# DerEchteKarsten/RayTracer3

Hardware: AMD Instinct MI355X
Metric: Mrays/s (higher is better)
Workload: dtype f32

## Files before the change

### include/rt3.h

```cpp
#ifndef RT3_H
#define RT3_H
#include <stddef.h>
#include <stdint.h>

#ifdef __cplusplus
extern "C" {
#endif

#define RT3_OK 0
#define RT3_E_INVALID (-1)
#define RT3_E_HIP (-2)
#define RT3_E_NO_DEVICE (-3)
#define RT3_E_STATE (-4)
#define RT3_E_UNSUPPORTED (-5)
#define RT3_E_DEPTH (-6)
#define RT3_E_COMM (-7)

#define RT3_INVALID_HANDLE 0xFFFFFFFFu
#define RT3_TAG_BUFFER 0u
#define RT3_TAG_IMAGE 1u
#define RT3_TAG_ACCEL 3u
#define RT3_MISS 0xFFFFFFFFu
#define RT3_BACKGROUND_DEPTH 100000.0f

#define RT3_FORMAT_R32_SFLOAT 100u
#define RT3_FORMAT_R32G32B32A32_SFLOAT 109u
#define RT3_FORMAT_R32G32B32A32_UINT 107u
#define RT3_FORMAT_R8G8B8A8_UNORM 37u
#define RT3_FORMAT_R16_UINT 74u

#define RT3_F_NEE_SKY 1u
#define RT3_F_BLUENOISE 2u
#define RT3_F_SPECULAR 4u
#define RT3_F_FACEFORWARD 8u
#define RT3_F_PROBE_RADIANCE 16u
#define RT3_F_NEE_EMISSIVE 32u

typedef struct rt3_gconst {
    float proj[16];
    float view[16];
    float proj_inverse[16];
    float view_inverse[16];
    float window_size[2];
    uint32_t frame;
    float blendfactor;
    uint32_t bounces;
    uint32_t samples;
    uint32_t proberng;
    float cell_size;
    uint32_t mouse[2];
    uint32_t pad[2];
} rt3_gconst;

typedef struct rt3_geometry_info {
    float base_color[4];
    int32_t base_color_texture_index;
    float metallic_factor;
    uint32_t index_offset;
    uint32_t vertex_offset;
    float emission[4];
    float roughness;
    uint32_t _pad[3];
} rt3_geometry_info;

typedef struct rt3_instance {
    uint32_t geometry_first, geometry_count;
    float transform[16];
} rt3_instance;

typedef struct rt3_stats {
    uint64_t extension_rays;
    uint64_t shadow_rays;
    uint64_t nodes_visited;
    uint64_t tris_tested;
    uint64_t shadow_nodes_visited;
    uint64_t shadow_tris_tested;
    uint64_t extend_launches;
    double extend_ms;
    uint64_t shadow_launches;
    double shadow_ms;
    double shade_ms;
    double other_ms;
    uint64_t trace_launches;
    double trace_ms;
    uint64_t trace_rays[2];
    uint64_t trace_nodes[2];
    uint64_t trace_tris[2];
    double gather_ms;
    uint64_t nodes_visited_lds;
    uint64_t shadow_nodes_visited_lds;
    double accel_build_ms;
    uint64_t accel_bulk_copies;
    uint64_t accel_arena_serial;
} rt3_stats;

typedef struct rt3_ctx rt3_ctx;

int rt3_create(int device, rt3_ctx **out);
void rt3_destroy(rt3_ctx *ctx);
const char *rt3_last_error(rt3_ctx *ctx);
int rt3_device_name(rt3_ctx *ctx, char *buf, size_t buf_size);

#define RT3_OPT_BATCH_SPP 1
#define RT3_OPT_PROFILE 2
#define RT3_OPT_COUNT_TRAVERSAL 3
#define RT3_OPT_EXTEND_VARIANT 4
#define RT3_OPT_LEAF_SIZE 5
#define RT3_OPT_NODE_WIDTH 6
#define RT3_OPT_NODE_QUANT 7
#define RT3_OPT_WIDE_COLLAPSE 8
#define RT3_OPT_POOL_CHUNK 9
#define RT3_OPT_SAH_TOP 11
#define RT3_OPT_TRACE_BLOCKS 12
#define RT3_OPT_INSTANCE_MODE 14
int rt3_set_option(rt3_ctx *ctx, int option, int64_t value);

int rt3_scene_set_vertices(rt3_ctx *ctx, const float *interleaved_p_n_t, uint32_t n_vertices);
int rt3_scene_set_indices(rt3_ctx *ctx, const uint32_t *indices, uint32_t n_indices);
int rt3_scene_set_geometry(rt3_ctx *ctx, const rt3_geometry_info *infos, const uint32_t *prim_counts, uint32_t n);
int rt3_scene_set_sky(rt3_ctx *ctx, const float *rgb, uint32_t width, uint32_t height);
int rt3_scene_set_bluenoise(rt3_ctx *ctx, const uint8_t *rgba, uint32_t width, uint32_t height);
int rt3_scene_set_texture(rt3_ctx *ctx, uint32_t index, const uint8_t *rgba_srgb, uint32_t width, uint32_t height);
int rt3_scene_set_alpha_cutoffs(rt3_ctx *ctx, const float *cutoffs, uint32_t n);
typedef struct rt3_material_textures {
    int32_t metallic_roughness_texture;
    int32_t normal_texture;
    int32_t emissive_texture;
    float   normal_scale;
} rt3_material_textures;
int rt3_scene_set_material_textures(rt3_ctx *ctx, const rt3_material_textures *m, uint32_t n);

int rt3_scene_set_instances(rt3_ctx *ctx, const rt3_instance *instances, uint32_t n);
int rt3_scene_set_prev_transforms(rt3_ctx *ctx, const float *transforms , uint32_t n);
int rt3_scene_snapshot_vertices(rt3_ctx *ctx);
int rt3_scene_forget_prev_vertices(rt3_ctx *ctx);
int rt3_scene_deformed_geometries(rt3_ctx *ctx, uint8_t *flags, uint32_t n);

int rt3_accel_build(rt3_ctx *ctx, uint32_t *out_handle);
int rt3_accel_info(rt3_ctx *ctx, uint32_t *n_nodes, uint32_t *n_tris, uint32_t *max_depth, uint32_t *node_bytes);
int rt3_accel_download(rt3_ctx *ctx, void *nodes, size_t nodes_bytes, void *tris, size_t tris_bytes);
int rt3_accel_levels(rt3_ctx *ctx, uint32_t *n_meshes, uint32_t *n_meshes_built, uint32_t *n_top_nodes, uint64_t *accel_bytes);
int rt3_accel_import(rt3_ctx *ctx, const void *nodes, size_t nodes_bytes, const void *tris, size_t tris_bytes);
int rt3_scene_update_vertices(rt3_ctx *ctx, const float *interleaved_p_n_t, uint32_t first, uint32_t n);
int rt3_accel_refit(rt3_ctx *ctx, uint32_t *out_handle);
int rt3_light_info(rt3_ctx *ctx, uint32_t *n_emitters, uint64_t *cdf_total);
int rt3_light_download(rt3_ctx *ctx, uint32_t *prim, float *area, uint32_t *mass );
int rt3_sky_download(rt3_ctx *ctx, uint32_t *alias, uint32_t *texels_rgb9e5, float *cdf_marg, float *pdf_uv);

int rt3_buffer_create(rt3_ctx *ctx, size_t bytes, uint32_t *out_handle);
int rt3_image_create(rt3_ctx *ctx, uint32_t width, uint32_t height, uint32_t format, uint32_t *out_handle);
int rt3_image_import(rt3_ctx *ctx, void *device_ptr, uint32_t width, uint32_t height, uint32_t format, uint32_t *out_handle);
int rt3_resource_upload(rt3_ctx *ctx, uint32_t handle, const void *src, size_t bytes);
int rt3_resource_download(rt3_ctx *ctx, uint32_t handle, void *dst, size_t bytes);
int rt3_resource_device_ptr(rt3_ctx *ctx, uint32_t handle, void **out_ptr, size_t *out_bytes);

int rt3_set_tile_partition(rt3_ctx *ctx, uint32_t width, uint32_t height, uint32_t rank, uint32_t n_ranks);
int rt3_tile_pixel_count(rt3_ctx *ctx, uint32_t rank, uint32_t n_ranks, uint32_t *out_count);
int rt3_image_pack_tiles(rt3_ctx *ctx, uint32_t image, uint32_t rank, uint32_t n_ranks, void *dst_device);
int rt3_image_unpack_tiles(rt3_ctx *ctx, uint32_t image, uint32_t rank, uint32_t n_ranks, const void *src_device);

#define RT3_COMM_ID_BYTES 128
int rt3_comm_version(int *out);
int rt3_comm_unique_id(void *id_out );
int rt3_comm_init(rt3_ctx *ctx, const void *id , uint32_t rank, uint32_t n_ranks);
int rt3_comm_destroy(rt3_ctx *ctx);
int rt3_gather_tiles(rt3_ctx *ctx, uint32_t image, uint32_t root);
int rt3_gather_layout(rt3_ctx *ctx, uint32_t image, uint32_t root, uint32_t n_ranks, uint64_t *offsets );
int rt3_gather_unpack(rt3_ctx *ctx, uint32_t image, uint32_t root, uint32_t n_ranks, const void *recv_device);

int rt3_pass_launch(rt3_ctx *ctx, const char *pass_name, const char *entry, uint32_t x, uint32_t y, uint32_t z,
                    const void *constants, size_t constants_size, const uint32_t *bindings, uint32_t n_bindings);
#define RT3_DENOISE_NO_DEMODULATION 1u
typedef struct rt3_denoise_params {
    uint32_t iterations;
    uint32_t normal_squarings;
    float sigma_z;
    float sigma_l;
    uint32_t flags;
} rt3_denoise_params;
int rt3_denoise_set_params(rt3_ctx *ctx, const rt3_denoise_params *params);
int rt3_denoise_set_variance_input(rt3_ctx *ctx, uint32_t moments_image);

#define RT3_TEMPORAL_NO_DEMODULATION 1u
typedef struct rt3_temporal_params {
    float alpha;
    float alpha_moments;
    uint32_t max_history;
    float normal_cos;
    float plane_tolerance;
    uint32_t flags;
} rt3_temporal_params;
int rt3_temporal_set_prev_view(rt3_ctx *ctx, const void *prev_gconst, size_t size);
int rt3_temporal_set_params(rt3_ctx *ctx, const rt3_temporal_params *params);
int rt3_temporal_set_motion_input(rt3_ctx *ctx, uint32_t motion_image);

int rt3_frame_wait(rt3_ctx *ctx);

int rt3_trace_rays(rt3_ctx *ctx, const float *rays, uint32_t n, int any_hit, float *t, float *u, float *v, uint32_t *prim,
                   uint32_t *n_nodes, uint32_t *n_tris, int repeat, double *kernel_ms);

int rt3_selftest_eval(rt3_ctx *ctx, int op, const void *in, uint32_t n, void *out);

int rt3_stats_reset(rt3_ctx *ctx);
int rt3_stats_get(rt3_ctx *ctx, rt3_stats *out);

void rt3_camera_gconst(const float position[3], const float direction[3], float fov_y_radians, float aspect,
                       float z_near, float z_far, float width, float height, rt3_gconst *out);

#ifdef __cplusplus
}
#endif
#endif
```

### raytracer3_amd/_lib.py

```python
from __future__ import annotations

import ctypes as C
import os
from pathlib import Path

PKG = Path(__file__).resolve().parent
LIB_PATH = Path(os.environ.get("RT3_LIBRARY", PKG / "librt3.so"))

RT3_OK = 0
E_INVALID, E_HIP, E_NO_DEVICE, E_STATE, E_UNSUPPORTED, E_DEPTH, E_COMM = -1, -2, -3, -4, -5, -6, -7
COMM_ID_BYTES = 128
TAG_BUFFER, TAG_IMAGE, TAG_ACCEL = 0, 1, 3
MISS = 0xFFFFFFFF
BACKGROUND_DEPTH = 100000.0
FORMAT_R32_SFLOAT, FORMAT_R32G32B32A32_SFLOAT, FORMAT_R32G32B32A32_UINT, FORMAT_R8G8B8A8_UNORM, FORMAT_R16_UINT = 100, 109, 107, 37, 74
F_NEE_SKY, F_BLUENOISE, F_SPECULAR, F_FACEFORWARD, F_PROBE_RADIANCE = 1, 2, 4, 8, 16
F_NEE_EMISSIVE = 32
OPT_BATCH_SPP, OPT_PROFILE, OPT_COUNT_TRAVERSAL, OPT_EXTEND_VARIANT, OPT_LEAF_SIZE, OPT_NODE_WIDTH, OPT_NODE_QUANT = 1, 2, 3, 4, 5, 6, 7
OPT_WIDE_COLLAPSE, OPT_POOL_CHUNK, OPT_SAH_TOP, OPT_TRACE_BLOCKS = 8, 9, 11, 12
OPT_FUSED_TRACE = 10
OPT_INSTANCE_MODE = 14
DENOISE_NO_DEMODULATION = 1
TEMPORAL_NO_DEMODULATION = 1
SELFTEST_EXPN = 28
SELFTEST_HIT_INFO = 29

EXPORTS = [
    "rt3_create", "rt3_destroy", "rt3_last_error", "rt3_device_name", "rt3_set_option",
    "rt3_scene_set_vertices", "rt3_scene_set_indices", "rt3_scene_set_geometry", "rt3_scene_set_sky", "rt3_scene_set_bluenoise", "rt3_scene_set_texture",
    "rt3_scene_set_alpha_cutoffs",
    "rt3_scene_set_material_textures",
    "rt3_scene_set_instances",
    "rt3_accel_build", "rt3_accel_info", "rt3_accel_levels", "rt3_accel_download", "rt3_accel_import", "rt3_sky_download",
    "rt3_scene_update_vertices", "rt3_accel_refit", "rt3_light_info", "rt3_light_download",
    "rt3_buffer_create", "rt3_image_create", "rt3_image_import", "rt3_resource_upload", "rt3_resource_download", "rt3_resource_device_ptr",
    "rt3_set_tile_partition", "rt3_tile_pixel_count", "rt3_image_pack_tiles", "rt3_image_unpack_tiles",
    "rt3_comm_version", "rt3_comm_unique_id", "rt3_comm_init", "rt3_comm_destroy", "rt3_gather_tiles", "rt3_gather_layout", "rt3_gather_unpack",
    "rt3_pass_launch", "rt3_denoise_set_params", "rt3_denoise_set_variance_input", "rt3_temporal_set_prev_view", "rt3_temporal_set_params",
    "rt3_scene_set_prev_transforms", "rt3_temporal_set_motion_input",
    "rt3_scene_snapshot_vertices", "rt3_scene_forget_prev_vertices", "rt3_scene_deformed_geometries",
    "rt3_frame_wait", "rt3_trace_rays", "rt3_selftest_eval", "rt3_stats_reset", "rt3_stats_get", "rt3_camera_gconst",
]


class GConst(C.Structure):

    _fields_ = [("proj", C.c_float * 16), ("view", C.c_float * 16), ("proj_inverse", C.c_float * 16), ("view_inverse", C.c_float * 16),
                ("window_size", C.c_float * 2), ("frame", C.c_uint32), ("blendfactor", C.c_float), ("bounces", C.c_uint32),
                ("samples", C.c_uint32), ("proberng", C.c_uint32), ("cell_size", C.c_float), ("mouse", C.c_uint32 * 2), ("pad", C.c_uint32 * 2)]


class Stats(C.Structure):
    _fields_ = [("extension_rays", C.c_uint64), ("shadow_rays", C.c_uint64), ("nodes_visited", C.c_uint64), ("tris_tested", C.c_uint64),
                ("shadow_nodes_visited", C.c_uint64), ("shadow_tris_tested", C.c_uint64),
                ("extend_launches", C.c_uint64), ("extend_ms", C.c_double), ("shadow_launches", C.c_uint64), ("shadow_ms", C.c_double),
                ("shade_ms", C.c_double), ("other_ms", C.c_double),
                ("trace_launches", C.c_uint64), ("trace_ms", C.c_double), ("trace_rays", C.c_uint64 * 2), ("trace_nodes", C.c_uint64 * 2),
                ("trace_tris", C.c_uint64 * 2), ("gather_ms", C.c_double), ("nodes_visited_lds", C.c_uint64), ("shadow_nodes_visited_lds", C.c_uint64), ("accel_build_ms", C.c_double), ("accel_bulk_copies", C.c_uint64),
                ("accel_arena_serial", C.c_uint64)]


class Instance(C.Structure):

    _fields_ = [("geometry_first", C.c_uint32), ("geometry_count", C.c_uint32), ("transform", C.c_float * 16)]


class DenoiseParams(C.Structure):

    _fields_ = [("iterations", C.c_uint32), ("normal_squarings", C.c_uint32), ("sigma_z", C.c_float), ("sigma_l", C.c_float), ("flags", C.c_uint32)]

    def __init__(self, iterations=5, normal_squarings=7, sigma_z=0.05, sigma_l=4.0, flags=0):
        super().__init__(iterations, normal_squarings, sigma_z, sigma_l, flags)


class TemporalParams(C.Structure):

    _fields_ = [("alpha", C.c_float), ("alpha_moments", C.c_float), ("max_history", C.c_uint32), ("normal_cos", C.c_float),
                ("plane_tolerance", C.c_float), ("flags", C.c_uint32)]

    def __init__(self, alpha=0.2, alpha_moments=0.2, max_history=32, normal_cos=0.9, plane_tolerance=0.01, flags=0):
        super().__init__(alpha, alpha_moments, max_history, normal_cos, plane_tolerance, flags)


assert C.sizeof(GConst) == 304


def kernel_source_hash() -> str:
    import hashlib

    h = hashlib.sha256()
    files = sorted((PKG / "csrc").glob("*.hip")) + sorted((PKG / "csrc").glob("*.hpp")) + [PKG / "csrc" / "Makefile", PKG.parent / "include" / "rt3.h"]
    for f in files:
        h.update(f.name.encode())
        h.update(f.read_bytes())
    return h.hexdigest()[:16]


class Rt3Error(RuntimeError):
    def __init__(self, code, msg):
        super().__init__(f"rt3 error {code}: {msg}")
        self.code = code


_lib = None


def load():
    global _lib
    if _lib is not None:
        return _lib
    try:
        import torch
    except ImportError:
        pass
    if not LIB_PATH.exists():
        raise ImportError(f"{LIB_PATH} is missing: build it with `make -C {PKG / 'csrc'}` (hipcc, gfx950). There is no CPU fallback.")
    L = C.CDLL(str(LIB_PATH))
    vp, u32, i32, f32, sz = C.c_void_p, C.c_uint32, C.c_int, C.c_float, C.c_size_t
    pu32 = C.POINTER(C.c_uint32)
    sig = {
        "rt3_create": (i32, [i32, C.POINTER(vp)]),
        "rt3_destroy": (None, [vp]),
        "rt3_last_error": (C.c_char_p, [vp]),
        "rt3_device_name": (i32, [vp, C.c_char_p, sz]),
        "rt3_set_option": (i32, [vp, i32, C.c_int64]),
        "rt3_scene_set_vertices": (i32, [vp, vp, u32]),
        "rt3_scene_set_indices": (i32, [vp, vp, u32]),
        "rt3_scene_set_geometry": (i32, [vp, vp, vp, u32]),
        "rt3_scene_set_sky": (i32, [vp, vp, u32, u32]),
        "rt3_scene_set_bluenoise": (i32, [vp, vp, u32, u32]),
        "rt3_scene_set_texture": (i32, [vp, u32, vp, u32, u32]),
        "rt3_scene_set_alpha_cutoffs": (i32, [vp, vp, u32]),
        "rt3_scene_set_material_textures": (i32, [vp, vp, u32]),
        "rt3_scene_set_instances": (i32, [vp, vp, u32]),
        "rt3_accel_build": (i32, [vp, pu32]),
        "rt3_accel_info": (i32, [vp, pu32, pu32, pu32, pu32]),
        "rt3_accel_levels": (i32, [vp, pu32, pu32, pu32, C.POINTER(C.c_uint64)]),
        "rt3_accel_download": (i32, [vp, vp, sz, vp, sz]),
        "rt3_accel_import": (i32, [vp, vp, sz, vp, sz]),
        "rt3_sky_download": (i32, [vp, vp, vp, vp, vp]),
        "rt3_scene_update_vertices": (i32, [vp, vp, u32, u32]),
        "rt3_accel_refit": (i32, [vp, pu32]),
        "rt3_light_info": (i32, [vp, pu32, C.POINTER(C.c_uint64)]),
        "rt3_light_download": (i32, [vp, vp, vp, vp]),
        "rt3_buffer_create": (i32, [vp, sz, pu32]),
        "rt3_image_create": (i32, [vp, u32, u32, u32, pu32]),
        "rt3_image_import": (i32, [vp, vp, u32, u32, u32, pu32]),
        "rt3_resource_upload": (i32, [vp, u32, vp, sz]),
        "rt3_resource_download": (i32, [vp, u32, vp, sz]),
        "rt3_resource_device_ptr": (i32, [vp, u32, C.POINTER(vp), C.POINTER(sz)]),
        "rt3_set_tile_partition": (i32, [vp, u32, u32, u32, u32]),
        "rt3_tile_pixel_count": (i32, [vp, u32, u32, pu32]),
        "rt3_image_pack_tiles": (i32, [vp, u32, u32, u32, vp]),
        "rt3_image_unpack_tiles": (i32, [vp, u32, u32, u32, vp]),
        "rt3_comm_version": (i32, [C.POINTER(i32)]),
        "rt3_comm_unique_id": (i32, [vp]),
        "rt3_comm_init": (i32, [vp, vp, u32, u32]),
        "rt3_comm_destroy": (i32, [vp]),
        "rt3_gather_tiles": (i32, [vp, u32, u32]),
        "rt3_gather_layout": (i32, [vp, u32, u32, u32, C.POINTER(C.c_uint64)]),
        "rt3_gather_unpack": (i32, [vp, u32, u32, u32, vp]),
        "rt3_pass_launch": (i32, [vp, C.c_char_p, C.c_char_p, u32, u32, u32, vp, sz, pu32, u32]),
        "rt3_denoise_set_params": (i32, [vp, C.POINTER(DenoiseParams)]),
        "rt3_denoise_set_variance_input": (i32, [vp, u32]),
        "rt3_temporal_set_prev_view": (i32, [vp, vp, sz]),
        "rt3_temporal_set_params": (i32, [vp, C.POINTER(TemporalParams)]),
        "rt3_scene_set_prev_transforms": (i32, [vp, vp, u32]),
        "rt3_temporal_set_motion_input": (i32, [vp, u32]),
        "rt3_scene_snapshot_vertices": (i32, [vp]),
        "rt3_scene_forget_prev_vertices": (i32, [vp]),
        "rt3_scene_deformed_geometries": (i32, [vp, vp, u32]),
        "rt3_frame_wait": (i32, [vp]),
        "rt3_trace_rays": (i32, [vp, vp, u32, i32, vp, vp, vp, vp, vp, vp, i32, C.POINTER(C.c_double)]),
        "rt3_selftest_eval": (i32, [vp, i32, vp, u32, vp]),
        "rt3_stats_reset": (i32, [vp]),
        "rt3_stats_get": (i32, [vp, C.POINTER(Stats)]),
        "rt3_camera_gconst": (None, [C.POINTER(f32), C.POINTER(f32), f32, f32, f32, f32, f32, f32, C.POINTER(GConst)]),
    }
    for name, (res, args) in sig.items():
        fn = getattr(L, name)
        fn.restype = res
        fn.argtypes = args
    _lib = L
    return L
```

### raytracer3_amd/csrc/rt3_accel.hip

```cpp
#include <hip/hip_runtime.h>

#include <cmath>
#include <cstring>
#include <algorithm>
#include <chrono>
#include <string>
#include <vector>

#include "rt3_ctx.hpp"

using namespace rt3;

namespace rt3 {

void invalidate_accel(rt3_ctx* c) { c->accel.built = false; }
void mark_accel_stale(rt3_ctx* c) {
    if (c->accel.built) c->accel.stale = true;
}
int check_accel_current(rt3_ctx* c, const char* unbuilt) {
    if (!c || !c->accel.built) return fail(c, RT3_E_STATE, unbuilt);
    if (c->accel.stale) return fail(c, RT3_E_STATE, "vertices were updated since the acceleration structure was built: rt3_accel_refit or rt3_accel_build first");
    return RT3_OK;
}
std::pair<const rt3_instance*, size_t> placements(const rt3_ctx* c, rt3_instance& whole) {
// ... 392 lines not shown
    uint32_t total = 0;
    for (size_t i = 0; i < n_inst; i++) {
        const float* m = inst[i].transform;
        double M[3][3];
        for (int r = 0; r < 3; r++)
            for (int k = 0; k < 3; k++) M[r][k] = m[4 * k + r];
        const double det = M[0][0] * (M[1][1] * M[2][2] - M[1][2] * M[2][1]) - M[0][1] * (M[1][0] * M[2][2] - M[1][2] * M[2][0]) +
                           M[0][2] * (M[1][0] * M[2][1] - M[1][1] * M[2][0]);
        TlInstance& in = ii[i];
        memcpy(in.m, m, sizeof(in.m));
        in.identity = memcmp(m, kIdentity, sizeof(kIdentity)) == 0;
        if (!(std::fabs(det) > 0.0) || !std::isfinite(1.0 / det))
            return fail(c, RT3_E_UNSUPPORTED, "instance " + std::to_string(i) + ": the upper 3 x 3 of the transform is singular (instance mode 1 needs its inverse)");
        const double id = 1.0 / det;
        in.A[0][0] = (M[1][1] * M[2][2] - M[1][2] * M[2][1]) * id;
        in.A[0][1] = (M[0][2] * M[2][1] - M[0][1] * M[2][2]) * id;
        in.A[0][2] = (M[0][1] * M[1][2] - M[0][2] * M[1][1]) * id;
        in.A[1][0] = (M[1][2] * M[2][0] - M[1][0] * M[2][2]) * id;
        in.A[1][1] = (M[0][0] * M[2][2] - M[0][2] * M[2][0]) * id;
        in.A[1][2] = (M[0][2] * M[1][0] - M[0][0] * M[1][2]) * id;
        in.A[2][0] = (M[1][0] * M[2][1] - M[1][1] * M[2][0]) * id;
        in.A[2][1] = (M[0][1] * M[2][0] - M[0][0] * M[2][1]) * id;
        in.A[2][2] = (M[0][0] * M[1][1] - M[0][1] * M[1][0]) * id;
        for (int r = 0; r < 3; r++) {
            for (int k = 0; k < 3; k++) in.A[r][k] = (double)(float)in.A[r][k];
            in.b[r] = (double)(float)-(in.A[r][0] * m[12] + in.A[r][1] * m[13] + in.A[r][2] * m[14]);
        }
        in.nA = in.nM = 0.0;
        for (int r = 0; r < 3; r++) {
            in.nA = std::fmax(in.nA, std::fabs(in.A[r][0]) + std::fabs(in.A[r][1]) + std::fabs(in.A[r][2]));
            in.nM = std::fmax(in.nM, std::fabs(M[r][0]) + std::fabs(M[r][1]) + std::fabs(M[r][2]));
        }
        if (!std::isfinite(in.nA) || in.nA * in.nM > kTlMaxCondition)
            return fail(c, RT3_E_UNSUPPORTED, "instance " + std::to_string(i) + ": the transform is too badly conditioned for instance mode 1 (||M|| ||M^-1|| > 2^20)");
        in.prim_base = total;
        uint32_t cnt = 0;
        for (; at < placed.size() && placed[at].instance == i; at++) cnt += placed[at].n_prims;
        total += cnt;
        in.mesh = ~0u;
        if (cnt == 0) continue;
        for (size_t q = 0; q < meshes.size(); q++)
            if (meshes[q].first == inst[i].geometry_first && meshes[q].count == inst[i].geometry_count) in.mesh = (uint32_t)q;
        if (in.mesh == ~0u) {
            TlMesh nm;
            memset(&nm, 0, sizeof(nm));
            nm.first = inst[i].geometry_first;
            nm.count = inst[i].geometry_count;
            nm.n_tris = cnt;
            in.mesh = (uint32_t)meshes.size();
            meshes.push_back(nm);
        }
    }
    uint32_t n_ne = 0;
    for (auto& in : ii) n_ne += in.mesh != ~0u ? 1u : 0u;
    if (n_ne >= (1u << 26)) return fail(c, RT3_E_UNSUPPORTED, "instance mode 1: too many instances");
    const uint32_t top_cap = n_ne ? n_ne : 1u;
    const uint32_t head = top_cap + 2u * n_ne;

    bool same = tl.valid && tl.gen == c->scene.content_gen && tl.head == head && tl.meshes.size() == meshes.size();
    for (size_t q = 0; same && q < meshes.size(); q++) same = tl.meshes[q].first == meshes[q].first && tl.meshes[q].count == meshes[q].count;
    tl.n_built = 0;
    if (same) {
        meshes = tl.meshes;
    } else {
        const bool reuse = tl.valid && tl.gen == c->scene.content_gen;
        std::vector<LbvhResult> built(meshes.size());
        std::vector<int> from(meshes.size(), -1);
        int rc = RT3_OK;
        for (size_t q = 0; q < meshes.size() && rc == RT3_OK; q++) {
            for (size_t o = 0; reuse && o < tl.meshes.size(); o++)
                if (tl.meshes[o].first == meshes[q].first && tl.meshes[o].count == meshes[q].count) from[q] = (int)o;
            if (from[q] >= 0) {
                const TlMesh& om = tl.meshes[from[q]];
                meshes[q].n_nodes = om.n_nodes;
                meshes[q].depth = om.depth;
                memcpy(meshes[q].box, om.box, sizeof(om.box));
            } else {
                rc = tl_build_mesh(c, meshes[q], &built[q]);
                tl.n_built++;
            }
        }
        uint64_t nodes_total = head, tris_total = 0;
        for (auto& m : meshes) {
            m.node_off = (uint32_t)nodes_total;
            m.tri_off = (uint32_t)tris_total;
            nodes_total += m.n_nodes;
            tris_total += m.n_tris;
        }
        if (rc == RT3_OK && (nodes_total >= (1ull << 29) || tris_total > (1ull << 28)))
            rc = fail(c, RT3_E_UNSUPPORTED, "instance mode 1: the bottom trees exceed the 28-bit references");
        LbvhResult fresh;
        hipError_t e = hipSuccess;
        if (rc == RT3_OK) {
            e = fresh.alloc_arena((size_t)nodes_total * 64, (size_t)tris_total, c->stream);
            if (fresh.arena_need > kArenaMaxBytes) rc = fail_arena(c, "two-level: bottom trees", fresh.arena_need);
        }
        if (rc == RT3_OK) {
            for (size_t q = 0; e == hipSuccess && q < meshes.size(); q++) {
                const TlMesh& m = meshes[q];
                if (from[q] >= 0) {
                    const TlMesh& om = tl.meshes[from[q]];
                    tlas_rebase_nodes(c->stream, c->accel.bvh.nodes.get() + 4 * (size_t)om.node_off, fresh.nodes.get() + 4 * (size_t)m.node_off, m.n_nodes, om.node_off,
                                      m.node_off, om.tri_off, m.tri_off);
                    e = hipMemcpyAsync(fresh.tris.get() + 3 * (size_t)m.tri_off, c->accel.bvh.tris.get() + 3 * (size_t)om.tri_off, (size_t)m.n_tris * 48, hipMemcpyDeviceToDevice,
                                       c->stream);
                } else {
                    tlas_rebase_nodes(c->stream, built[q].nodes.get(), fresh.nodes.get() + 4 * (size_t)m.node_off, m.n_nodes, 0u, m.node_off, 0u, m.tri_off);
                    e = hipMemcpyAsync(fresh.tris.get() + 3 * (size_t)m.tri_off, built[q].tris.get(), (size_t)m.n_tris * 48, hipMemcpyDeviceToDevice, c->stream);
                }
            }
            if (e == hipSuccess) e = hipGetLastError();
            if (e == hipSuccess) e = hipStreamSynchronize(c->stream);
            if (e != hipSuccess) rc = fail(c, RT3_E_HIP, std::string("two-level: bottom trees: ") + hipGetErrorString(e));
        }
        if (rc != RT3_OK) {
            free_accel(c);
            return rc;
        }
        c->accel.bvh.take_arena(fresh);
        tl.meshes = meshes;
        tl.head = head;
        tl.gen = c->scene.content_gen;
        tl.n_alloc_nodes = (uint32_t)nodes_total;
        tl.valid = true;
    }
    tl.inst = std::move(ii);
    tl.n_placed = n_ne;
    tl.top_cap = top_cap;
    return tl_records_and_top(c);
}

static int make_alpha_tables(rt3_ctx* c) {
    c->accel.masked = false;
    if (!any_cutoff(c)) return RT3_OK;
    if (c->opt.node_width != 4 || c->opt.node_quant != 1)
        return fail(c, RT3_E_UNSUPPORTED, "alpha-masked geometry needs the default node layout (RT3_OPT_NODE_WIDTH 4, RT3_OPT_NODE_QUANT 1)");
    std::vector<uint2> mask(c->scene.n_geoms, make_uint2(0u, 0u)), table;
    for (uint32_t g = 0; g < c->scene.n_geoms; g++) {
        if (!(c->scene.h_cutoffs[g] > 0.0f)) continue;
        uint32_t cb, ab;
        memcpy(&cb, &c->scene.h_cutoffs[g], 4);
        memcpy(&ab, &c->scene.h_geoms[g].base_color[3], 4);
        mask[g] = make_uint2(cb, (uint32_t)table.size());
        table.push_back(make_uint2((uint32_t)c->scene.h_geoms[g].base_color_texture_index, ab));
    }
    for (const Placed& p : c->accel.placed)
        if (mask[p.geom].x != 0u && p.n_prims > 0) c->accel.masked = true;
    if (int r = dev_alloc(c, c->accel.d_geom_mask, mask.size())) return r;
    if (int r = dev_alloc(c, c->accel.d_alpha, table.size())) return r;
    HIPC(c, hipMemcpy(c->accel.d_geom_mask.get(), mask.data(), mask.size() * sizeof(uint2), hipMemcpyHostToDevice));
    HIPC(c, hipMemcpy(c->accel.d_alpha.get(), table.data(), table.size() * sizeof(uint2), hipMemcpyHostToDevice));
    return RT3_OK;
}
static void bump_stamp(rt3_ctx* c) { c->accel.stamp++; }
static int accel_finish(rt3_ctx* c, uint32_t* out_handle) {
    if (int r = make_shade_records(c)) return r;
    HIPC(c, hipStreamSynchronize(c->stream));
    c->prof.stats.accel_bulk_copies += c->accel.bulk_copies;
    c->accel.bulk_copies = 0;
    c->accel.built = true;
    c->accel.stale = false;
    bump_stamp(c);
    c->accel.topo_gen = c->scene.topo_gen;
    if (out_handle) *out_handle = (RT3_TAG_ACCEL << 30) | 0u;
    return RT3_OK;
}
int rt3_accel_build(rt3_ctx* c, uint32_t* out_handle) {
    if (!c) return RT3_E_INVALID;
    HIPC(c, hipSetDevice(c->device));
    if (c->scene.n_prims && (!c->scene.d_verts || !c->scene.d_indices)) return fail(c, RT3_E_STATE, "set vertices, indices and geometry before rt3_accel_build");
    if (int r = revalidate_geometry(c)) return r;
    HIPC(c, hipStreamSynchronize(c->stream));
    const auto t_build0 = std::chrono::steady_clock::now();
    invalidate_accel(c);
    c->accel.refit_planned = false;
    if (int r = flatten_world(c)) return r;
    if (int r = make_alpha_tables(c)) return r;
    if (c->opt.instance_mode == 1) {
        if (int r = build_two_level(c)) return r;
    } else {
        free_accel(c);
        hipError_t e = lbvh_build(c->stream, world_tables(c), c->accel.n_flat_prims, c->opt.leaf_size, c->opt.node_width, c->opt.node_quant, c->opt.collapse,
                                  c->opt.sah_top, c->accel.build_scratch, &c->accel.bvh, c->accel.masked ? c->accel.d_geom_mask.get() : nullptr);
        if (c->accel.build_scratch.capacity_bytes() > ((size_t)1 << 30)) c->accel.build_scratch.reset();
        if (e != hipSuccess) {
            const uint64_t need = c->accel.bvh.arena_need;
            free_accel(c);
            if (need > kArenaMaxBytes) return fail_arena(c, "lbvh_build", need);
            return fail(c, RT3_E_HIP, std::string("lbvh_build: ") + hipGetErrorString(e));
        }
        const uint32_t stack_need = stack_entries(c->opt.node_width, c->accel.bvh.max_depth);
        if (stack_need > kMaxStack) {
            const int rc = fail(c, RT3_E_DEPTH, "LBVH with " + std::to_string(c->accel.bvh.max_depth) + " levels needs " + std::to_string(stack_need) +
                                                    " stack entries, the traversal kernels hold " + std::to_string(kMaxStack));
            free_accel(c);
            return rc;
        }
    }
    if (int r = accel_finish(c, out_handle)) return r;
    c->prof.stats.accel_build_ms = std::chrono::duration<double, std::milli>(std::chrono::steady_clock::now() - t_build0).count();
    return RT3_OK;
}
int rt3_accel_info(rt3_ctx* c, uint32_t* n_nodes, uint32_t* n_tris, uint32_t* max_depth, uint32_t* node_bytes) {
    if (!c || !c->accel.built) return fail(c, RT3_E_STATE, "no acceleration structure built");
    if (n_nodes) *n_nodes = c->accel.bvh.n_nodes;
    if (n_tris) *n_tris = c->accel.bvh.n_tris;
    if (max_depth) *max_depth = c->accel.bvh.max_depth;
    if (node_bytes) *node_bytes = c->accel.bvh.node_bytes;
    return RT3_OK;
}
int rt3_accel_levels(rt3_ctx* c, uint32_t* n_meshes, uint32_t* n_meshes_built, uint32_t* n_top_nodes, uint64_t* accel_bytes) {
    if (!c || !c->accel.built) return fail(c, RT3_E_STATE, "no acceleration structure built");
    const bool two = c->accel.bvh.layout == kLayoutTwoLevel;
    if (n_meshes) *n_meshes = two ? c->accel.tl.n_meshes : 0u;
    if (n_meshes_built) *n_meshes_built = two ? c->accel.tl.n_built : 0u;
    if (n_top_nodes) *n_top_nodes = two ? c->accel.tl.n_top : 0u;
    if (accel_bytes) {
        const uint64_t nodes = !c->accel.bvh.nodes ? 0u : (two ? (uint64_t)c->accel.tl.n_alloc_nodes * 64u : (uint64_t)c->accel.bvh.n_nodes * c->accel.bvh.node_bytes);
        *accel_bytes = nodes + (!c->accel.bvh.tris ? 0u : (uint64_t)c->accel.bvh.n_tris * 48u) + (uint64_t)c->accel.bvh.n_top * 64u;
    }
    return RT3_OK;
}
int rt3_accel_download(rt3_ctx* c, void* nodes, size_t nodes_bytes, void* tris, size_t tris_bytes) {
    if (int r = check_accel_current(c, "no acceleration structure built")) return r;
    if (c->accel.bvh.layout == kLayoutTwoLevel) return fail(c, RT3_E_UNSUPPORTED, "accel_download: not for the two-level structure (RT3_OPT_INSTANCE_MODE 1)");
    if (nodes) {
        if (nodes_bytes != (size_t)c->accel.bvh.n_nodes * c->accel.bvh.node_bytes) return fail(c, RT3_E_INVALID, "nodes_bytes mismatch");
        if (nodes_bytes) HIPC(c, hipMemcpy(nodes, c->accel.bvh.nodes.get(), nodes_bytes, hipMemcpyDeviceToHost));
    }
    if (tris) {
        if (tris_bytes != (size_t)c->accel.bvh.n_tris * 48) return fail(c, RT3_E_INVALID, "tris_bytes mismatch");
        if (tris_bytes) HIPC(c, hipMemcpy(tris, c->accel.bvh.tris.get(), tris_bytes, hipMemcpyDeviceToHost));
    }
    return RT3_OK;
}
int rt3_accel_import(rt3_ctx* c, const void* nodes, size_t nodes_bytes, const void* tris, size_t tris_bytes) {
    if (!c || !nodes || !tris) return fail(c, RT3_E_INVALID, "accel_import: NULL argument");
    if (!c->accel.built) return fail(c, RT3_E_STATE, "accel_import: build the scene's own structure first (rt3_accel_build makes the shading records)");
    if (c->accel.bvh.layout == kLayoutTwoLevel) return fail(c, RT3_E_UNSUPPORTED, "accel_import: not for the two-level structure (RT3_OPT_INSTANCE_MODE 1)");
    if (c->accel.bvh.layout != kLayoutWide64Q) return fail(c, RT3_E_UNSUPPORTED, "accel_import: default node layout only");
    if (any_cutoff(c)) return fail(c, RT3_E_UNSUPPORTED, "accel_import: not for a scene with alpha-masked geometry (rt3_scene_set_alpha_cutoffs)");
    if (nodes_bytes == 0 || nodes_bytes % 64 || tris_bytes % 48 || nodes_bytes / 64 > 0x3FFFFFFFull) return fail(c, RT3_E_INVALID, "accel_import: sizes must be multiples of 64 / 48 bytes");
    const uint32_t nn = (uint32_t)(nodes_bytes / 64), nt = (uint32_t)(tris_bytes / 48);
    const uint32_t* w = static_cast<const uint32_t*>(nodes);
    const uint32_t* tw = static_cast<const uint32_t*>(tris);
    for (uint32_t k = 0; k < nt; k++)
        if (tw[12 * (size_t)k + 9] >= c->accel.n_flat_prims) return fail(c, RT3_E_INVALID, "accel_import: triangle record " + std::to_string(k) + " names a primitive the scene does not have");
    std::vector<uint8_t> seen(nn, 0);
    std::vector<std::pair<uint32_t, uint32_t>> st;
    st.emplace_back(0u, 1u);
    seen[0] = 1;
    uint32_t max_level = 1;
    while (!st.empty()) {
        const auto [node, level] = st.back();
        st.pop_back();
        max_level = level > max_level ? level : max_level;
        for (int k = 0; k < 4; k++) {
            const uint32_t ref = w[16 * (size_t)node + 10 + k];
            if (ref == 0xFFFFFFFFu) continue;
            if (ref & 0x80000000u) {
                const uint64_t first = ref & 0x0FFFFFFFu, cnt = ((ref >> 28) & 7u) + 1u;
                if (first + cnt > nt) return fail(c, RT3_E_INVALID, "accel_import: node " + std::to_string(node) + " references triangles beyond the array");
            } else {
                if (ref >= nn || seen[ref]) return fail(c, RT3_E_INVALID, "accel_import: node " + std::to_string(node) + " references a node out of range or reachable twice");
                seen[ref] = 1;
                st.emplace_back(ref, level + 1);
            }
        }
    }
    const uint32_t depth = max_level + 1;
    if (stack_entries(4, depth) > kMaxStack) return fail(c, RT3_E_DEPTH, "accel_import: the tree is deeper than the traversal stack supports");
    HIPC(c, hipSetDevice(c->device));
    HIPC(c, hipStreamSynchronize(c->stream));
    LbvhResult fresh;
    hipError_t e = fresh.alloc_arena(nodes_bytes, nt, c->stream);
    if (fresh.arena_need > kArenaMaxBytes) return fail_arena(c, "accel_import", fresh.arena_need);
    if (e == hipSuccess) e = hipStreamSynchronize(c->stream);
    if (e == hipSuccess) e = hipMemcpy(fresh.nodes.get(), nodes, nodes_bytes, hipMemcpyHostToDevice);
    if (e == hipSuccess && tris_bytes) e = hipMemcpy(fresh.tris.get(), tris, tris_bytes, hipMemcpyHostToDevice);
    if (e != hipSuccess) return fail(c, RT3_E_HIP, std::string("accel_import: ") + hipGetErrorString(e));
    c->accel.bvh.take_arena(fresh);
    c->accel.bvh.n_nodes = nn;
    c->accel.bvh.n_tris = nt;
    c->accel.bvh.max_depth = depth;
    c->accel.refit_planned = false;
    bump_stamp(c);
    e = lbvh_make_top(c->stream, c->accel.bvh.nodes.get(), nn, c->accel.bvh.top, &c->accel.bvh.n_top);
    if (e != hipSuccess) {
        invalidate_accel(c);
        return fail(c, RT3_E_HIP, std::string("accel_import: top-of-tree copy: ") + hipGetErrorString(e));
    }
    return RT3_OK;
}

struct RefitScratch {
    uint32_t* bounds;
    float *nbox, *tbox;
};
static int refit_scratch(rt3_ctx* c, size_t n_nodes, size_t n_tris, RefitScratch* s) {
    BufLayout plan;
    plan.add(&s->bounds, 6).add(&s->nbox, 6 * n_nodes).add(&s->tbox, 6 * n_tris);
    HIPC(c, c->accel.refit_scratch.grow_bytes(plan.bytes()));
    HIPC(c, plan.carve(c->accel.refit_scratch));
    return RT3_OK;
}
static int refit_flat(rt3_ctx* c) {
    LbvhResult& b = c->accel.bvh;
    if (!b.n_nodes) return RT3_OK;
    if (!c->accel.refit_planned) {
        c->accel.refit_trees.clear();
        c->accel.refit_trees.resize(1);
        const hipError_t e = refit_plan(c->stream, b.nodes.get(), 0u, b.n_nodes, b.max_depth, &c->accel.refit_trees[0]);
        if (e != hipSuccess) return fail(c, RT3_E_HIP, std::string("accel_refit: plan: ") + hipGetErrorString(e));
        c->accel.refit_planned = true;
    }
    RefitScratch s;
    if (int r = refit_scratch(c, b.n_nodes, b.n_tris, &s)) return r;
    hipError_t e = refit_tree(c->stream, c->accel.refit_trees[0], world_tables(c), c->accel.n_flat_prims, 0u, b.n_tris, b.nodes.get(), b.tris.get(), s.bounds, s.nbox,
                              s.tbox);
    if (e == hipSuccess) e = lbvh_make_top(c->stream, b.nodes.get(), b.n_nodes, b.top, &b.n_top);
    if (e != hipSuccess) return fail(c, RT3_E_HIP, std::string("accel_refit: ") + hipGetErrorString(e));
    return RT3_OK;
}
static int refit_two_level(rt3_ctx* c) {
    TwoLevelState& tl = c->accel.tl;
    tl.n_built = 0;
    if (!tl.valid) return RT3_OK;
    const std::vector<TlMesh>& meshes = tl.meshes;
    const size_t nm = meshes.size();
    if (!c->accel.refit_planned) {
        c->accel.refit_trees.clear();
        c->accel.refit_trees.resize(nm);
        c->accel.refit_tables.clear();
        c->accel.refit_tables.resize(nm);
        for (size_t q = 0; q < nm; q++) {
            const TlMesh& m = meshes[q];
            hipError_t e = make_mesh_tables(c, m, &c->accel.refit_tables[q]);
            if (e == hipSuccess && m.count * sizeof(FlatGeomDev) > (64u << 10)) c->accel.bulk_copies += 1;
            if (e == hipSuccess) e = refit_plan(c->stream, c->accel.bvh.nodes.get(), m.node_off, m.n_nodes, m.depth, &c->accel.refit_trees[q]);
            if (e != hipSuccess) return fail(c, RT3_E_HIP, std::string("accel_refit: plan: ") + hipGetErrorString(e));
        }
        c->accel.refit_planned = true;
    }
    RefitScratch s;
    if (int r = refit_scratch(c, tl.n_alloc_nodes, c->accel.bvh.n_tris, &s)) return r;
    std::vector<uint32_t> roots(16 * nm);
    hipError_t e = hipSuccess;
    for (size_t q = 0; e == hipSuccess && q < nm; q++) {
        const TlMesh& m = meshes[q];
        e = refit_tree(c->stream, c->accel.refit_trees[q], mesh_tables(c, c->accel.refit_tables[q]), m.n_tris, m.tri_off, m.n_tris, c->accel.bvh.nodes.get(), c->accel.bvh.tris.get(),
                       s.bounds, s.nbox, s.tbox);
        if (e == hipSuccess) e = hipMemcpyAsync(&roots[16 * q], c->accel.bvh.nodes.get() + 4 * (size_t)m.node_off, 64, hipMemcpyDeviceToHost, c->stream);
    }
    if (e == hipSuccess) e = hipStreamSynchronize(c->stream);
    if (e != hipSuccess) return fail(c, RT3_E_HIP, std::string("accel_refit: bottom trees: ") + hipGetErrorString(e));
    for (size_t q = 0; q < nm; q++) quantised_node_box(&roots[16 * q], tl.meshes[q].box);
    tl.gen = c->scene.content_gen;
    return tl_records_and_top(c);
}
int rt3_accel_refit(rt3_ctx* c, uint32_t* out_handle) {
    if (!c) return RT3_E_INVALID;
    if (c->opt.node_width != 4 || c->opt.node_quant != 1)
        return fail(c, RT3_E_UNSUPPORTED, "accel_refit: default node layout only (RT3_OPT_NODE_WIDTH 4, RT3_OPT_NODE_QUANT 1)");
    if (!c->accel.built || c->accel.topo_gen != c->scene.topo_gen)
        return fail(c, RT3_E_STATE, "accel_refit: no acceleration structure for the current scene (only rt3_scene_update_vertices may come between rt3_accel_build and a refit)");
    const bool two = c->accel.bvh.layout == kLayoutTwoLevel;
    if (!two && c->accel.bvh.layout != kLayoutWide64Q) return fail(c, RT3_E_UNSUPPORTED, "accel_refit: default node layout only");
    HIPC(c, hipSetDevice(c->device));
    HIPC(c, hipStreamSynchronize(c->stream));
    invalidate_accel(c);
    if (int r = two ? refit_two_level(c) : refit_flat(c)) return r;
    return accel_finish(c, out_handle);
}

int rt3_light_info(rt3_ctx* c, uint32_t* n_emitters, uint64_t* cdf_total) {
    if (!c) return RT3_E_INVALID;
    if (int r = ensure_lights(c)) return r;
    if (n_emitters) *n_emitters = c->accel.lights.n;
    if (cdf_total) *cdf_total = c->accel.lights.total;
    return RT3_OK;
}
int rt3_light_download(rt3_ctx* c, uint32_t* prim, float* area, uint32_t* mass) {
    if (!c) return RT3_E_INVALID;
    if (int r = ensure_lights(c)) return r;
    const LightTable& t = c->accel.lights;
    if (!t.n) return RT3_OK;
    if (prim) HIPC(c, hipMemcpy(prim, t.prim.get(), (size_t)t.n * 4, hipMemcpyDeviceToHost));
    if (area) HIPC(c, hipMemcpy(area, t.area.get(), (size_t)t.n * 4, hipMemcpyDeviceToHost));
    if (mass) {
        HIPC(c, hipMemcpy(mass, t.cdf.get(), (size_t)t.n * 4, hipMemcpyDeviceToHost));
        for (uint32_t k = t.n - 1; k > 0; k--) mass[k] -= mass[k - 1];
    }
    return RT3_OK;
}

}
```

### raytracer3_amd/csrc/rt3_api.hip

```cpp
#include <hip/hip_runtime.h>

#include <cmath>
#include <cstdio>
#include <cstring>
#include <string>
#include <vector>

#include "rt3_ctx.hpp"

using namespace rt3;

static_assert(sizeof(rt3_gconst) == 304 && sizeof(GConstDev) == 304, "GConst is 304 bytes (renderer/mod.rs:47-63)");
static_assert(sizeof(rt3_geometry_info) == 64, "geometry info is 64 bytes");
static_assert(RT3_F_NEE_SKY == RT3_FLAG_NEE_SKY && RT3_F_BLUENOISE == RT3_FLAG_BLUENOISE && RT3_F_FACEFORWARD == RT3_FLAG_FACEFORWARD && RT3_F_SPECULAR == RT3_FLAG_SPECULAR && RT3_F_PROBE_RADIANCE == RT3_FLAG_PROBE_RADIANCE && RT3_F_NEE_EMISSIVE == RT3_FLAG_NEE_EMISSIVE, "flags");

static thread_local std::string g_create_error;

namespace rt3 {

int fail(rt3_ctx* c, int code, const std::string& msg) {
    if (c) c->err = msg;
    else g_create_error = msg;
    return code;
}
// ... 5 lines not shown
    return r->tag == want_tag && r->ptr ? r : nullptr;
}
size_t format_bytes(uint32_t f) {
    switch (f) {
        case RT3_FORMAT_R32_SFLOAT: return 4;
        case RT3_FORMAT_R32G32B32A32_SFLOAT: return 16;
        case RT3_FORMAT_R32G32B32A32_UINT: return 16;
        case RT3_FORMAT_R8G8B8A8_UNORM: return 4;
        case RT3_FORMAT_R16_UINT: return 2;
        default: return 0;
    }
}

int harvest(rt3_ctx* c) {
    if (!c->work.pending_counters.empty()) {
        std::vector<uint32_t> h(c->work.counters_next);
        HIPC(c, hipMemcpy(h.data(), c->work.d_counters.get(), (size_t)c->work.counters_next * 4, hipMemcpyDeviceToHost));
        for (auto& b : c->work.pending_counters) {
            for (uint32_t k = 0; k < b.n_pairs; k++) {
                c->prof.stats.extension_rays += h[b.first + 2 * k];
                c->prof.stats.shadow_rays += h[b.first + 2 * k + 1];
            }
            for (uint32_t k = 0; k < b.n_emit; k++) c->prof.stats.shadow_rays += h[b.emit_first + k];
        }
        c->work.pending_counters.clear();
    }
    c->work.counters_next = 0;
    c->prof.stats.extension_rays += c->work.primary_rays_pending;
    c->work.primary_rays_pending = 0;
    if (c->opt.count) {
        unsigned long long t[kTotWords] = {};
        HIPC(c, hipMemcpy(t, c->work.d_totals.get(), sizeof(t), hipMemcpyDeviceToHost));
        c->prof.stats.nodes_visited += t[kTotExtendNodes];
        c->prof.stats.tris_tested += t[kTotExtendTris];
        c->prof.stats.shadow_nodes_visited += t[kTotShadowNodes];
        c->prof.stats.shadow_tris_tested += t[kTotShadowTris];
        c->prof.stats.nodes_visited_lds += t[kTotExtendLds];
        c->prof.stats.shadow_nodes_visited_lds += t[kTotShadowLds];
        HIPC(c, hipMemset(c->work.d_totals.get(), 0, sizeof(t)));
    }
    for (auto& t : c->prof.pending_events) {
        float ms = 0.0f;
        HIPC(c, hipEventElapsedTime(&ms, t.a, t.b));
        switch (t.cat) {
            case CAT_EXTEND: c->prof.stats.extend_ms += ms; c->prof.stats.extend_launches++; break;
            case CAT_SHADOW: c->prof.stats.shadow_ms += ms; c->prof.stats.shadow_launches++; break;
            case CAT_SHADE: c->prof.stats.shade_ms += ms; break;
            case CAT_GATHER: c->prof.stats.gather_ms += ms; break;
            default: c->prof.stats.other_ms += ms; break;
        }
        c->prof.free_events.push_back(t);
    }
    c->prof.pending_events.clear();
    return RT3_OK;
}

}

extern "C" {

int rt3_create(int device, rt3_ctx** out) {
    if (!out) return fail(nullptr, RT3_E_INVALID, "out is NULL");
    *out = nullptr;
    int n = 0;
    if (hipGetDeviceCount(&n) != hipSuccess || n <= 0) return fail(nullptr, RT3_E_NO_DEVICE, "no HIP device visible (librt3 has no CPU fallback)");
    if (device < 0 || device >= n) return fail(nullptr, RT3_E_INVALID, "device index out of range");
    hipDeviceProp_t prop;
    if (hipSetDevice(device) != hipSuccess || hipGetDeviceProperties(&prop, device) != hipSuccess) return fail(nullptr, RT3_E_HIP, "hipSetDevice failed");
    if (std::string(prop.gcnArchName).rfind("gfx950", 0) != 0)
        return fail(nullptr, RT3_E_NO_DEVICE, std::string("device is ") + prop.gcnArchName + ", librt3 is built for gfx950 only");
    rt3_ctx* c = new rt3_ctx();
    c->device = device;
    snprintf(c->name, sizeof(c->name), "%s (%s)", prop.name, prop.gcnArchName);
    memset(&c->prof.stats, 0, sizeof(c->prof.stats));
    if (hipStreamCreateWithFlags(&c->stream, hipStreamNonBlocking) != hipSuccess || c->work.d_counters.alloc_bytes((size_t)c->work.counters_cap * 4) != hipSuccess ||
        c->work.d_totals.alloc_bytes(kTotWords * 8) != hipSuccess || hipMemset(c->work.d_totals.get(), 0, kTotWords * 8) != hipSuccess) {
        rt3_destroy(c);
        return fail(nullptr, RT3_E_HIP, "stream / counter allocation failed");
    }
    *out = c;
    return RT3_OK;
}

void rt3_destroy(rt3_ctx* c) {
    if (!c) return;
    (void)hipSetDevice(c->device);
    if (c->stream) (void)hipStreamSynchronize(c->stream);
    comm_release(c);
    for (auto& t : c->prof.pending_events) { (void)hipEventDestroy(t.a); (void)hipEventDestroy(t.b); }
    for (auto& t : c->prof.free_events) { (void)hipEventDestroy(t.a); (void)hipEventDestroy(t.b); }
    hipStream_t stream = c->stream;
    delete c;
    if (stream) (void)hipStreamDestroy(stream);
}

const char* rt3_last_error(rt3_ctx* c) { return c ? c->err.c_str() : g_create_error.c_str(); }

int rt3_device_name(rt3_ctx* c, char* buf, size_t n) {
    if (!c || !buf || !n) return RT3_E_INVALID;
    snprintf(buf, n, "%s", c->name);
    return RT3_OK;
}

int rt3_set_option(rt3_ctx* c, int option, int64_t value) {
    if (!c) return RT3_E_INVALID;
    switch (option) {
        case RT3_OPT_BATCH_SPP: c->opt.batch_spp = value; return RT3_OK;
        case RT3_OPT_PROFILE: c->opt.profile = value != 0; return RT3_OK;
        case RT3_OPT_COUNT_TRAVERSAL: c->opt.count = value != 0; return RT3_OK;
        case RT3_OPT_EXTEND_VARIANT:
            c->opt.variant = (int)value;
            HIPC(c, hipSetDevice(c->device));
            set_refill_lanes((uint32_t)value);
            return RT3_OK;
        case RT3_OPT_LEAF_SIZE:
            if (value < 1 || value > 8) return fail(c, RT3_E_INVALID, "leaf size must be 1..8");
            c->opt.leaf_size = (uint32_t)value;
            invalidate_topology(c);
            return RT3_OK;
        case RT3_OPT_NODE_QUANT:
            if (value < 0 || value > 2) return fail(c, RT3_E_INVALID, "node quantisation must be 0 (fp32), 1 (64 B) or 2 (compact 48 B)");
            c->opt.node_quant = (uint32_t)value;
            invalidate_topology(c);
            return RT3_OK;
        case RT3_OPT_SAH_TOP:
            if (value < 0 || value > 65536) return fail(c, RT3_E_INVALID, "SAH-top cluster size must be 0 (off) .. 65536");
            c->opt.sah_top = (uint32_t)value;
            invalidate_topology(c);
            return RT3_OK;
        case RT3_OPT_POOL_CHUNK:
            if (value < 64 || value > 65536 || (value & 63)) return fail(c, RT3_E_INVALID, "pool chunk must be a multiple of 64 in [64, 65536]");
            HIPC(c, hipSetDevice(c->device));
            set_pool_chunk((uint32_t)value);
            return RT3_OK;
        case RT3_OPT_TRACE_BLOCKS:
            if (value < 1 || value > 65535) return fail(c, RT3_E_INVALID, "trace blocks must be in [1, 65535]");
            set_trace_blocks((uint32_t)value);
            return RT3_OK;
        case RT3_OPT_WIDE_COLLAPSE:
            if (value < 0 || value > 2) return fail(c, RT3_E_INVALID, "wide collapse must be 0 (even depth), 1 (surface area) or 2 (cost-driven)");
            c->opt.collapse = (uint32_t)value;
            invalidate_topology(c);
            return RT3_OK;
        case RT3_OPT_NODE_WIDTH:
            if (value != 2 && value != 4) return fail(c, RT3_E_INVALID, "node width must be 2 or 4");
            c->opt.node_width = (uint32_t)value;
            invalidate_topology(c);
            return RT3_OK;
        case RT3_OPT_INSTANCE_MODE:
            if (value != 0 && value != 1) return fail(c, RT3_E_INVALID, "instance mode must be 0 (flatten) or 1 (two-level)");
            c->opt.instance_mode = (int)value;
            invalidate_accel(c);
            return RT3_OK;
        default: return fail(c, RT3_E_INVALID, "unknown option");
    }
}

int rt3_buffer_create(rt3_ctx* c, size_t bytes, uint32_t* out) {
    if (!c || !out || !bytes) return fail(c, RT3_E_INVALID, "bad buffer size");
    HIPC(c, hipSetDevice(c->device));
    Resource r;
    r.tag = RT3_TAG_BUFFER;
    r.bytes = bytes;
    HIPC(c, r.mem.alloc_bytes(bytes));
    r.ptr = r.mem.get();
    HIPC(c, hipMemset(r.ptr, 0, bytes));
    c->resources.push_back(std::move(r));
    *out = (RT3_TAG_BUFFER << 30) | (uint32_t)(c->resources.size() - 1);
    return RT3_OK;
}
int rt3_image_create(rt3_ctx* c, uint32_t w, uint32_t h, uint32_t format, uint32_t* out) {
    size_t px = format_bytes(format);
    if (!c || !out || !w || !h || !px) return fail(c, RT3_E_INVALID, "bad image size / format");
    HIPC(c, hipSetDevice(c->device));
    Resource r;
    r.tag = RT3_TAG_IMAGE;
    r.w = w; r.h = h; r.format = format;
    r.bytes = (size_t)w * h * px;
    HIPC(c, r.mem.alloc_bytes(r.bytes));
    r.ptr = r.mem.get();
    HIPC(c, hipMemset(r.ptr, 0, r.bytes));
    c->resources.push_back(std::move(r));
    *out = (RT3_TAG_IMAGE << 30) | (uint32_t)(c->resources.size() - 1);
    return RT3_OK;
}
int rt3_image_import(rt3_ctx* c, void* device_ptr, uint32_t w, uint32_t h, uint32_t format, uint32_t* out) {
    size_t px = format_bytes(format);
    if (!c || !out || !device_ptr || !w || !h || !px) return fail(c, RT3_E_INVALID, "bad import");
    Resource r;
    r.tag = RT3_TAG_IMAGE;
    r.w = w; r.h = h; r.format = format;
    r.bytes = (size_t)w * h * px;
    r.ptr = device_ptr;
    c->resources.push_back(std::move(r));
    *out = (RT3_TAG_IMAGE << 30) | (uint32_t)(c->resources.size() - 1);
    return RT3_OK;
}
static Resource* any_res(rt3_ctx* c, uint32_t handle) {
    Resource* r = get_res(c, handle, RT3_TAG_IMAGE);
    return r ? r : get_res(c, handle, RT3_TAG_BUFFER);
}
int rt3_resource_upload(rt3_ctx* c, uint32_t handle, const void* src, size_t bytes) {
    if (!c || !src) return RT3_E_INVALID;
    Resource* r = any_res(c, handle);
    if (!r || bytes != r->bytes) return fail(c, RT3_E_INVALID, "upload: bad handle or size");
    HIPC(c, hipSetDevice(c->device));
    HIPC(c, hipStreamSynchronize(c->stream));
    HIPC(c, hipMemcpy(r->ptr, src, bytes, hipMemcpyHostToDevice));
    return RT3_OK;
}
int rt3_resource_download(rt3_ctx* c, uint32_t handle, void* dst, size_t bytes) {
    if (!c || !dst) return RT3_E_INVALID;
    Resource* r = any_res(c, handle);
    if (!r || bytes != r->bytes) return fail(c, RT3_E_INVALID, "download: bad handle or size");
    HIPC(c, hipSetDevice(c->device));
    HIPC(c, hipStreamSynchronize(c->stream));
    HIPC(c, hipMemcpy(dst, r->ptr, bytes, hipMemcpyDeviceToHost));
    return RT3_OK;
}
int rt3_resource_device_ptr(rt3_ctx* c, uint32_t handle, void** out_ptr, size_t* out_bytes) {
    if (!c || !out_ptr) return RT3_E_INVALID;
    Resource* r = any_res(c, handle);
    if (!r) return fail(c, RT3_E_INVALID, "bad handle");
    *out_ptr = r->ptr;
    if (out_bytes) *out_bytes = r->bytes;
    return RT3_OK;
}

int rt3_frame_wait(rt3_ctx* c) {
    if (!c) return RT3_E_INVALID;
    HIPC(c, hipSetDevice(c->device));
    HIPC(c, hipStreamSynchronize(c->stream));
    return RT3_OK;
}

int rt3_trace_rays(rt3_ctx* c, const float* rays, uint32_t n, int any_hit, float* t, float* u, float* v, uint32_t* prim, uint32_t* n_nodes,
                   uint32_t* n_tris, int repeat, double* kernel_ms) {
    if (!c || !rays || !prim || (!any_hit && (!t || !u || !v))) return fail(c, RT3_E_INVALID, "trace_rays: NULL argument");
    if (int r = check_accel_current(c)) return r;
    if (n == 0) return RT3_OK;
    HIPC(c, hipSetDevice(c->device));
    DevBuf<float> d_rays, d_hits;
    DevBuf<uint32_t> d_cn, d_ct, d_occ, d_cur;
    const bool count = n_nodes || n_tris;
    struct Events {
        hipEvent_t e0 = nullptr, e1 = nullptr;
        ~Events() {
            if (e0) (void)hipEventDestroy(e0);
            if (e1) (void)hipEventDestroy(e1);
        }
    } ev;
    HIPC(c, d_rays.alloc_bytes((size_t)n * 32));
    HIPC(c, d_hits.alloc_bytes((size_t)n * 16));
    HIPC(c, d_occ.alloc_bytes((size_t)n * 4));
    HIPC(c, d_cur.alloc_bytes(4));
    if (count) {
        HIPC(c, d_cn.alloc_bytes((size_t)n * 4));
        HIPC(c, d_ct.alloc_bytes((size_t)n * 4));
    }
    {
        std::vector<float> rec((size_t)n * 8);
        for (uint32_t i = 0; i < n; i++) {
            float* a = &rec[4 * (size_t)i];
            float* b = &rec[4 * ((size_t)n + i)];
            a[0] = rays[i]; a[1] = rays[(size_t)n + i]; a[2] = rays[2 * (size_t)n + i]; a[3] = rays[6 * (size_t)n + i];
            b[0] = rays[3 * (size_t)n + i]; b[1] = rays[4 * (size_t)n + i]; b[2] = rays[5 * (size_t)n + i]; b[3] = rays[7 * (size_t)n + i];
        }
        HIPC(c, hipMemcpy(d_rays.get(), rec.data(), (size_t)n * 32, hipMemcpyHostToDevice));
    }
    HIPC(c, hipEventCreate(&ev.e0));
    HIPC(c, hipEventCreate(&ev.e1));
    if (repeat < 1) repeat = 1;
    TraceLaunch L;
    L.rays = d_rays.get(); L.stride = n; L.n = n; L.work_counter = d_cur.get();
    L.hits = d_hits.get(); L.occluded = d_occ.get();
    L.count = count; L.cnt_nodes = d_cn.get(); L.cnt_tris = d_ct.get();
    if (c->accel.masked) {
        if (int r = sync_textures(c)) return r;
        L.alpha = alpha_dev(c);
    }
    auto launch = [&]() {
        (void)hipMemsetAsync(d_cur.get(), 0, 4, c->stream);
        if (any_hit) launch_shadow(c->stream, c->accel.bvh, L);
        else launch_extend(c->stream, c->accel.bvh, L);
    };
    launch();
    HIPC(c, hipEventRecord(ev.e0, c->stream));
    for (int k = 0; k < repeat; k++) launch();
    HIPC(c, hipEventRecord(ev.e1, c->stream));
    HIPC(c, hipGetLastError());
    HIPC(c, hipStreamSynchronize(c->stream));
    float ms = 0.0f;
    HIPC(c, hipEventElapsedTime(&ms, ev.e0, ev.e1));
    if (kernel_ms) *kernel_ms = (double)ms / repeat;
    if (any_hit) {
        HIPC(c, hipMemcpy(prim, d_occ.get(), (size_t)n * 4, hipMemcpyDeviceToHost));
    } else {
        std::vector<float> rec((size_t)n * 4);
        HIPC(c, hipMemcpy(rec.data(), d_hits.get(), (size_t)n * 16, hipMemcpyDeviceToHost));
        for (uint32_t i = 0; i < n; i++) {
            t[i] = rec[4 * (size_t)i];
            u[i] = rec[4 * (size_t)i + 1];
            v[i] = rec[4 * (size_t)i + 2];
            memcpy(&prim[i], &rec[4 * (size_t)i + 3], 4);
        }
    }
// ... 110 lines not shown
```

### raytracer3_amd/csrc/rt3_ctx.hpp

```cpp
#pragma once
#include <hip/hip_runtime.h>

#include <cstring>
#include <string>
#include <utility>
#include <vector>

#include "../../include/rt3.h"
#include "rt3_internal.hpp"

struct ncclComm;

namespace rt3 {

inline const rt3_denoise_params kDenoiseDefaults = {5u, 7u, 0.05f, 4.0f, 0u};
inline const rt3_temporal_params kTemporalDefaults = {0.2f, 0.2f, 32u, 0.9f, 0.01f, 0u};
inline constexpr float kIdentity[16] = {1, 0, 0, 0, 0, 1, 0, 0, 0, 0, 1, 0, 0, 0, 0, 1};
inline void pack3x4(const float* m16, float* m12) {
    for (int col = 0; col < 4; col++)
        for (int row = 0; row < 3; row++) m12[3 * col + row] = m16[4 * col + row];
}

struct Resource {
    uint32_t tag = 0;
    void* ptr = nullptr;
    DevBuf<char> mem;
    size_t bytes = 0;
    uint32_t w = 0, h = 0, format = 0;
};
struct PixelList {
    uint32_t w, h, rank, n_ranks, count;
    DevBuf<uint32_t> dev;
    DevBuf<uint2> dev_bn;
    uint64_t bn_stamp = ~0ull;
};
struct GatherLayout {
    uint32_t w, h, root, n_ranks;
    std::vector<uint64_t> off;
    DevBuf<uint32_t> dev;
};
enum Cat { CAT_EXTEND = 0, CAT_SHADOW = 1, CAT_SHADE = 2, CAT_OTHER = 3, CAT_GATHER = 4 };
struct Timed {
    hipEvent_t a, b;
    int cat;
};
struct CounterBlock {
    uint32_t first, n_pairs;
    uint32_t emit_first = 0, n_emit = 0;
};

struct TlMesh {
    uint32_t first, count;
    uint32_t node_off, tri_off;
    uint32_t n_nodes, n_tris, depth;
    double box[6];
};
struct TlInstance {
    double A[3][3], b[3];
    double nA, nM;
    float m[16];
    uint32_t mesh, prim_base;
    bool identity;
};
struct TwoLevelState {
    bool valid = false;
    uint64_t gen = 0;
    uint32_t head = 0;
    uint32_t n_alloc_nodes = 0;
    std::vector<TlMesh> meshes;
    std::vector<TlInstance> inst;
    uint32_t n_placed = 0, top_cap = 0;
    uint32_t n_meshes = 0, n_built = 0, n_top = 0;
    DevBuf<char> scratch;
};
struct MeshTables {
    DevBuf<char> mem;
    FlatGeomDev* geoms = nullptr;
    uint32_t *first_prim = nullptr, *prim_geom = nullptr;
};
struct ShadeRecords {
    DevBuf<uint4> rec;
    DevBuf<float2> uv;
    DevBuf<uint32_t> tan;
    bool has_tan = false;
    uint32_t n = 0;
    std::vector<uint64_t> key;
};
struct Placed {
    uint32_t instance, geom;
    uint32_t first_prim, n_prims;
    bool identity;
};

}

struct rt3_ctx {
    int device = 0;
    hipStream_t stream = nullptr;
    std::string err;
    char name[256] = {0};
    std::vector<rt3::Resource> resources;

    struct Scene {
        rt3::DevBuf<float> d_verts;
        uint32_t n_verts = 0;
        rt3::DevBuf<uint32_t> d_indices;
        uint32_t n_indices = 0;
        uint32_t n_geoms = 0, n_prims = 0;
        std::vector<uint32_t> h_indices;
        std::vector<rt3_geometry_info> h_geoms;
        std::vector<uint32_t> h_prim_counts;
        std::vector<std::pair<uint32_t, uint32_t>> h_geom_span;
        int64_t max_tex_index = -1;
        std::vector<float> h_cutoffs;
        std::vector<rt3_material_textures> h_mat_tex;
        std::vector<rt3_instance> h_instances;
        std::vector<float> prev_transforms;
        rt3::DevBuf<uint2> d_sky;
        rt3::DevBuf<float> d_cdf_marg;
        rt3::DevBuf<uint32_t> d_sky_alias, d_guide_marg;
        uint32_t sky_w = 0, sky_h = 0, sky_wt = 0;
        rt3::DevBuf<uint8_t> d_bn;
        uint32_t bn_w = 0, bn_h = 0;
        uint64_t bn_stamp = 0;
        std::vector<std::vector<uint8_t>> h_tex;
        std::vector<uint32_t> tex_w, tex_h;
        rt3::DevBuf<uint8_t> d_tex_pixels;
        rt3::DevBuf<uint4> d_tex_table;
        rt3::DevBuf<float> d_srgb_lut;
        bool tex_dirty = false;
        uint64_t topo_gen = 1, content_gen = 1;
    } scene;

    struct Accel {
        rt3::DevBuf<rt3::FlatGeomDev> d_geoms;
        rt3::DevBuf<rt3::ShadeGeomDev> d_shade_geoms;
        rt3::DevBuf<rt3::MatTexDev> d_mat_tex;
        bool has_mat_tex = false, has_normal_tex = false;
        rt3::DevBuf<uint32_t> d_prim_geom, d_first_prim;
        uint32_t n_flat_geoms = 0, n_flat_prims = 0;
        std::vector<rt3::Placed> placed;
        uint64_t bulk_copies = 0;
        rt3::DevBuf<uint2> d_geom_mask, d_alpha;
        bool masked = false;
        rt3::LbvhResult bvh;
        rt3::ShadeRecords shade;
        rt3::DevBuf<char> build_scratch;
        bool built = false;
        bool stale = false;
        uint64_t topo_gen = 0;
        uint64_t stamp = 0;
        rt3::LightTable lights;
        bool refit_planned = false;
        std::vector<rt3::RefitTree> refit_trees;
        std::vector<rt3::MeshTables> refit_tables;
        rt3::DevBuf<char> refit_scratch;
        rt3::TwoLevelState tl;
    } accel;

    struct Work {
        size_t cap = 0, cap_pix = 0;
        rt3::DevBuf<float> rays[2], hits, T[2];
        rt3::DevBuf<float> sh_rays, sh_contrib, lacc, radsum;
        rt3::DevBuf<float> sh2_rays, sh2_contrib, sh2_tmax;
        size_t cap_emit = 0;
        rt3::DevBuf<uint32_t> d_counters;
        uint32_t counters_cap = 1 << 16, counters_next = 0;
        rt3::DevBuf<unsigned long long> d_totals;
        std::vector<rt3::CounterBlock> pending_counters;
        uint64_t primary_rays_pending = 0;
    } work;

    struct Tiles {
        std::vector<rt3::PixelList> pixlists;
        std::vector<rt3::GatherLayout> gather_layouts;
        uint32_t rank = 0, n_ranks = 1, part_w = 0, part_h = 0;
        ncclComm* comm = nullptr;
        uint32_t comm_rank = 0, comm_size = 0;
        rt3::DevBuf<char> gather_buf;
    } tiles;

    struct Denoise {
        rt3_denoise_params params = rt3::kDenoiseDefaults;
        rt3::DevBuf<char> scratch;
        uint32_t variance_image = 0;
    } denoise;
    struct Temporal {
        rt3_temporal_params params = rt3::kTemporalDefaults;
        rt3_gconst prev;
        bool has_prev = false;
        uint32_t motion_image = 0;
    } temporal;
    struct Motion {
        bool dirty = false, any_moved = false, any_deformed = false;
        uint64_t stamp = 0;
        rt3::DevBuf<rt3::MotionPrevDev> d_prev;
        rt3::DevBuf<uint32_t> d_slot;
    } motion;
    struct Deform {
        rt3::DevBuf<float4> d_prev_pos;
        bool snapshot = false, dirty = false;
        std::vector<std::pair<uint32_t, uint32_t>> ranges;
        std::vector<uint32_t> h_deformed;
        rt3::DevBuf<uint32_t> d_deformed;
        rt3::DevBuf<uint4> d_chunks;
    } deform;

    struct Opt {
        int64_t batch_spp = 0;
        bool profile = false, count = false;
        int variant = 0;
        uint32_t leaf_size = 2, node_width = 4, node_quant = 1, collapse = 2, sah_top = 1;
        int instance_mode = 0;
    } opt;
    struct Prof {
        rt3_stats stats;
        std::vector<rt3::Timed> pending_events;
        std::vector<rt3::Timed> free_events;
    } prof;
};

namespace rt3 {

int fail(rt3_ctx* c, int code, const std::string& msg);
#define HIPC(ctx, call)                                                                                              \
    do {                                                                                                             \
        hipError_t e_ = (call);                                                                                      \
        if (e_ != hipSuccess) return fail(ctx, RT3_E_HIP, std::string(#call) + ": " + hipGetErrorString(e_));        \
    } while (0)

template <typename T>
int dev_alloc(rt3_ctx* c, DevBuf<T>& b, size_t count) {
    HIPC(c, b.alloc_bytes((count ? count : 1) * sizeof(T)));
    return RT3_OK;
}
struct ScopedTimer {
    rt3_ctx* c;
    Timed t;
    bool on;
    ScopedTimer(rt3_ctx* ctx, int cat) : c(ctx), on(ctx->opt.profile) {
        if (!on) return;
        if (!c->prof.free_events.empty()) {
            t = c->prof.free_events.back();
            c->prof.free_events.pop_back();
        } else if (hipEventCreate(&t.a) != hipSuccess || hipEventCreate(&t.b) != hipSuccess) {
            on = false;
            return;
        }
        t.cat = cat;
        (void)hipEventRecord(t.a, c->stream);
    }
    ~ScopedTimer() {
        if (!on) return;
        (void)hipEventRecord(t.b, c->stream);
        c->prof.pending_events.push_back(t);
    }
};
Resource* get_res(rt3_ctx* c, uint32_t handle, uint32_t want_tag);
size_t format_bytes(uint32_t f);
int harvest(rt3_ctx* c);

void invalidate_topology(rt3_ctx* c);
int sync_textures(rt3_ctx* c);
int revalidate_geometry(rt3_ctx* c);
int deform_flags(rt3_ctx* c);
inline bool any_cutoff(const rt3_ctx* c) { return !c->scene.h_cutoffs.empty(); }
inline bool any_mat_tex(const rt3_ctx* c) { return !c->scene.h_mat_tex.empty(); }

void invalidate_accel(rt3_ctx* c);
void mark_accel_stale(rt3_ctx* c);
int check_accel_current(rt3_ctx* c, const char* unbuilt = "rt3_accel_build has not been called for the current scene");
std::pair<const rt3_instance*, size_t> placements(const rt3_ctx* c, rt3_instance& whole);
SceneDev scene_dev(const rt3_ctx* c);
GeomTables world_tables(const rt3_ctx* c);
AlphaDev alpha_dev(const rt3_ctx* c);
int ensure_lights(rt3_ctx* c);

void motion_tables_stale(rt3_ctx* c);

int get_pixlist(rt3_ctx* c, uint32_t w, uint32_t h, uint32_t rank, uint32_t n_ranks, PixelList** out);
int pixlist_bluenoise(rt3_ctx* c, PixelList* pl);
void comm_release(rt3_ctx* c);

}
```

### raytracer3_amd/csrc/rt3_internal.hpp

```cpp
#pragma once
#include <hip/hip_runtime.h>
#include <stddef.h>
#include <stdint.h>

#include <utility>
#include <vector>

#include "rt3_camera.hpp"
#include "rt3_math.hpp"
#include "rt3_surface.hpp"

#define RT3_FLAG_NEE_SKY 1u
#define RT3_FLAG_BLUENOISE 2u
#define RT3_FLAG_SPECULAR 4u
#define RT3_FLAG_FACEFORWARD 8u
#define RT3_FLAG_PROBE_RADIANCE 16u
#define RT3_FLAG_NEE_EMISSIVE 32u

namespace rt3 {

constexpr int kExtendBlock = 256;
constexpr unsigned kExtendMaxBlocks = 2048;
constexpr int kLayoutBinary64 = 0;
constexpr int kLayoutWide128 = 1;
// ... 31 lines not shown
    uint32_t n_first;
    float* out_rays;
    float* out_T;
    uint32_t* out_count;
    float* sh_rays;
    float* sh_contrib;
    uint32_t* sh_count;
    float* lacc;
    size_t stride;
    LightsDev lights;
    float* sh2_rays;
    float* sh2_contrib;
    float* sh2_tmax;
    uint32_t* sh2_count;
};
struct GeomTables {
    const float* verts;
    const uint32_t* indices;
    const FlatGeomDev* geoms;
    const uint32_t *prim_geom, *first_prim;
};

inline unsigned grid_for(uint64_t n, unsigned block, unsigned max_blocks) {
    uint64_t b = (n + block - 1) / block;
    if (b < 1) b = 1;
    return (unsigned)(b > max_blocks ? max_blocks : b);
}

void launch_raygen(hipStream_t st, const GConstDev& g, const uint32_t* pixels, uint32_t npix, float* rays, size_t stride);
void launch_gbuffer(hipStream_t st, const SceneDev& sc, const uint32_t* pixels, uint32_t npix, uint32_t width, const float* hits,
                    size_t stride, void* gbuffer, float* depth);
void launch_shade(hipStream_t st, bool first, ShadeLaunch L);
void launch_pixbn(hipStream_t st, const uint32_t* pixels, uint32_t npix, const uint8_t* bluenoise, uint32_t bn_w, uint32_t bn_h, uint2* out);
void launch_accumulate(hipStream_t st, const GConstDev& g, const uint32_t* pixels, uint32_t npix, uint32_t width, const float* depth,
                       const float* lacc, size_t stride, uint32_t sb, int first_batch, int last_batch, float* radsum, void* light,
                       const void* prev);
void launch_postprocess(hipStream_t st, const GConstDev& g, const SceneDev& sc, const uint32_t* pixels, uint32_t npix, uint32_t width,
                        const float* depth, const void* in, void* out);
void launch_pack_tiles(hipStream_t st, const uint32_t* pixels, uint32_t npix, uint32_t width, const void* img, void* dst);
void launch_unpack_tiles(hipStream_t st, const uint32_t* pixels, uint32_t npix, uint32_t width, const void* src, void* img);

void launch_sis(hipStream_t st, uint32_t W, uint32_t probes_x, uint32_t probes_y, const void* gbuffer, void* out, float* debug);
void launch_probe_raygen(hipStream_t st, const GConstDev& g, uint32_t W, uint32_t probes_x, uint32_t probes_y, const float* depth, const void* directions,
                         void* atlas, float* rays, size_t stride, void* d2);
void launch_probe_store(hipStream_t st, const SceneDev& sc, uint32_t flags, float blend, uint32_t probes_x, uint32_t probes_y, const float* hits,
                        const void* d2, const void* prev, void* atlas);
void launch_sh_conversion(hipStream_t st, uint32_t probes_x, uint32_t probes_y, const void* atlas, void* out);
void launch_interpolate(hipStream_t st, const GConstDev& g, uint32_t W, uint32_t H, const void* gbuffer, const float* depth, const void* sh, void* light);
void launch_selftest_probes(hipStream_t st, int op, const uint32_t* in, uint32_t n, uint32_t* out);

void launch_prim_geom(hipStream_t st, const uint32_t* first_prim, uint32_t n_geoms, uint32_t n, uint32_t* prim_geom);
void set_refill_lanes(uint32_t v);
void set_pool_chunk(uint32_t v);
void set_trace_blocks(uint32_t v);
bool selftest_widths(int op, uint32_t* in_w, uint32_t* out_w);
void launch_selftest(hipStream_t st, int op, const SceneDev& sc, const uint32_t* in, uint32_t n, uint32_t* out);

#define RT3_TRY(x)                           \
    do {                                     \
        const hipError_t e_ = (x);           \
        if (e_ != hipSuccess) return e_;     \
    } while (0)

template <typename T>
class DevBuf {
public:
    DevBuf() = default;
    DevBuf(const DevBuf&) = delete;
    DevBuf& operator=(const DevBuf&) = delete;
    DevBuf(DevBuf&& o) noexcept : p_(o.p_), cap_(o.cap_) {
        o.p_ = nullptr;
        o.cap_ = 0;
    }
    DevBuf& operator=(DevBuf&& o) noexcept {
        if (this != &o) {
            reset();
            p_ = o.p_;
            cap_ = o.cap_;
            o.p_ = nullptr;
            o.cap_ = 0;
        }
        return *this;
    }
    ~DevBuf() { reset(); }
    T* get() const { return p_; }
    size_t capacity_bytes() const { return cap_; }
    explicit operator bool() const { return p_ != nullptr; }
    void reset() {
        if (p_) (void)hipFree(p_);
        p_ = nullptr;
        cap_ = 0;
    }
    hipError_t alloc_bytes(size_t bytes) {
        reset();
        void* p = nullptr;
        const hipError_t e = hipMalloc(&p, bytes);
        if (e == hipSuccess) {
            p_ = static_cast<T*>(p);
            cap_ = bytes;
        }
        return e;
    }
    hipError_t grow_bytes(size_t bytes) { return bytes <= cap_ ? hipSuccess : alloc_bytes(bytes); }

private:
    T* p_ = nullptr;
    size_t cap_ = 0;
};

class BufLayout {
public:
    template <typename T>
    BufLayout& add(T** dst, size_t count) {
        const size_t at = (end_ + 255) & ~(size_t)255;
        pieces_.push_back({dst, at, &set_ptr<T>});
        end_ = at + count * sizeof(T);
        return *this;
    }
    size_t bytes() const { return end_; }
    hipError_t carve(const DevBuf<char>& buf) const {
        if (buf.capacity_bytes() < end_) return hipErrorOutOfMemory;
        for (const Piece& p : pieces_) p.set(p.dst, buf.get() + p.at);
        return hipSuccess;
    }

private:
    struct Piece {
        void* dst;
        size_t at;
        void (*set)(void* dst, char* p);
    };
    template <typename T>
    static void set_ptr(void* dst, char* p) { *static_cast<T**>(dst) = reinterpret_cast<T*>(p); }
    std::vector<Piece> pieces_;
    size_t end_ = 0;
};

template <typename T>
class DevView {
public:
    DevView() = default;
    explicit DevView(T* p) : p_(p) {}
    T* get() const { return p_; }
    explicit operator bool() const { return p_ != nullptr; }

private:
    T* p_ = nullptr;
};

constexpr uint64_t kArenaMaxBytes = (4ull << 30) - 128;
uint64_t next_arena_serial();
constexpr size_t kArenaSlack = 128;

struct LbvhResult {
    DevBuf<float4> arena;
    DevView<float4> nodes;
    uint32_t node_bytes = 128;
    int layout = kLayoutWide128;
    DevView<float4> tris;
    uint32_t tri_off = 0;
    uint64_t arena_need = 0;
    uint64_t arena_serial = 0;
    DevBuf<float4> top;
    uint32_t n_top = 0;
    uint32_t n_nodes = 0, n_tris = 0, max_depth = 0;

    hipError_t alloc_arena(size_t nodes_bytes, size_t n_records, hipStream_t st) {
        free_arena();
        const size_t off = (nodes_bytes + 127) & ~(size_t)127, rec_end = off + n_records * 48;
        arena_need = rec_end + kArenaSlack;
        if (arena_need > kArenaMaxBytes) return hipErrorInvalidValue;
        RT3_TRY(arena.alloc_bytes(rec_end + kArenaSlack));
        arena_serial = next_arena_serial();
        tri_off = (uint32_t)off;
        nodes = DevView<float4>(arena.get());
        tris = DevView<float4>(reinterpret_cast<float4*>(reinterpret_cast<char*>(arena.get()) + off));
        return hipMemsetAsync(reinterpret_cast<char*>(arena.get()) + rec_end, 0, kArenaSlack, st);
    }
    void free_arena() {
        arena.reset();
        nodes = tris = DevView<float4>();
        tri_off = 0;
        arena_serial = 0;
    }
    void take_arena(LbvhResult& from) {
        arena = std::move(from.arena);
        nodes = from.nodes;
        tris = from.tris;
        tri_off = from.tri_off;
        arena_serial = from.arena_serial;
        from.nodes = from.tris = DevView<float4>();
        from.tri_off = 0;
        from.arena_serial = 0;
    }
};
struct TraceLaunch {
    const float* rays = nullptr;
    size_t stride = 0;
    const uint32_t* count_ptr = nullptr;
    uint32_t n = 0;
    uint32_t* work_counter = nullptr;
    float* hits = nullptr;
    bool payload = false;
    const float* contrib = nullptr;
    float* lacc = nullptr;
    const float* tmax = nullptr;
    uint32_t* occluded = nullptr;
    bool count = false;
    uint32_t *cnt_nodes = nullptr, *cnt_tris = nullptr;
    unsigned long long* totals = nullptr;
    AlphaDev alpha = {};
};
void launch_extend(hipStream_t st, const LbvhResult& bvh, const TraceLaunch& L);
void launch_shadow(hipStream_t st, const LbvhResult& bvh, const TraceLaunch& L);
hipError_t lbvh_build(hipStream_t st, GeomTables t, uint32_t n_prims, uint32_t leaf_max, uint32_t node_width, uint32_t node_quant, uint32_t collapse_mode,
                      uint32_t sah_top, DevBuf<char>& scratch, LbvhResult* out, const uint2* geom_mask = nullptr);
struct SahTopScratch {
    uint32_t *top, *ncl, *pool_pos, *cl_pos, *pool, *cl_ref, *cl_cnt, *idx, *tmp, *counters, *tile_left, *tile_woff, *tile_roff;
    float *cl_mn, *cl_mx;
    char *seg_a, *seg_b, *seg_small, *huge, *tiles;
    char* scan_tmp;
    size_t scan_bytes;
};
hipError_t sah_top_plan(hipStream_t st, uint32_t n, BufLayout& plan, SahTopScratch* s);
hipError_t sah_top_relink_gpu(hipStream_t st, uint32_t nn, uint32_t* left, uint32_t* right, uint32_t* rcnt, uint32_t* pint, uint32_t* pleaf,
                              const float* lmin, const float* lmax, float* nbox, uint32_t T, const SahTopScratch& s, bool* relinked);

void launch_tri_shade(hipStream_t st, GeomTables t, uint32_t n, uint4* tri_shade, float2* tri_uv);
void launch_tri_tangent(hipStream_t st, GeomTables t, uint32_t n, uint32_t* tri_tan);

void tlas_rebase_nodes(hipStream_t st, const float4* src, float4* dst, uint32_t n, uint32_t node_from, uint32_t node_to, uint32_t tri_from, uint32_t tri_to);
void tlas_box_tris(hipStream_t st, const float* boxes, uint32_t n, float* verts, uint32_t* indices);
void tlas_emit_top(hipStream_t st, const float4* top_nodes, uint32_t n_nodes, const float4* top_tris, uint32_t rec_base, float4* dst);

struct RefitTree {
    DevBuf<uint32_t> order;
    std::vector<uint32_t> level_count;
};
hipError_t refit_plan(hipStream_t st, const float4* nodes, uint32_t root, uint32_t n_nodes, uint32_t max_depth, RefitTree* plan);
hipError_t refit_tree(hipStream_t st, const RefitTree& plan, GeomTables t, uint32_t n_prims, uint32_t tri_first, uint32_t n_tris, float4* nodes,
                      float4* tris, uint32_t* bounds, float* nbox, float* tbox);

struct LightTable {
    DevBuf<float4> rec;
    DevBuf<uint32_t> cdf, guide, prim, geom_base;
    DevBuf<float> area;
    DevBuf<char> scratch;
    uint32_t n = 0, n_guide = 0, guide_shift = 0, total = 0;
    uint64_t stamp = 0;
    LightsDev dev() const {
        LightsDev d;
        d.rec = rec.get(); d.cdf = cdf.get(); d.guide = guide.get(); d.geom_base = geom_base.get();
        d.n = total ? n : 0u; d.guide_shift = guide_shift;
        return d;
    }
};
hipError_t lights_build(hipStream_t st, GeomTables t, const std::vector<uint32_t>& geom_base, const std::vector<uint32_t>& eg_geom,
                        const std::vector<uint32_t>& eg_first, uint32_t n, LightTable* out);

struct DenoiseScratch {
    float4 *gP, *gN;
    float4* sig[2];
};
struct DenoiseLaunch {
    GConstDev g;
    uint32_t W, H, squarings, flags;
    float sigma_z, sigma_l;
    const void* gbuffer;
    const float* depth;
    const void* in;
    void* out;
    const void* moments = nullptr;
    DenoiseScratch s;
};
void denoise_plan(uint32_t W, uint32_t H, BufLayout& plan, DenoiseScratch* s);
void launch_denoise_prepare(hipStream_t st, const DenoiseLaunch& L);
void launch_denoise_variance(hipStream_t st, const DenoiseLaunch& L);
void launch_denoise_atrous(hipStream_t st, const DenoiseLaunch& L, uint32_t iteration);
void launch_denoise_finish(hipStream_t st, const DenoiseLaunch& L, uint32_t iterations);
void launch_selftest_denoise(hipStream_t st, const uint32_t* in, uint32_t n, uint32_t* out);

struct TemporalLaunch {
    GConstDev g, prev;
    uint32_t W, H, flags;
    float alpha, alpha_moments, max_history, normal_cos, plane_tolerance;
    const void *gbuffer, *in, *prev_gbuffer, *prev_history, *prev_moments;
    const float *depth, *prev_depth;
    void *out, *history, *moments;
    const void* motion = nullptr;
};
void launch_temporal(hipStream_t st, const TemporalLaunch& L);

constexpr uint32_t kMotionUnmoved = 0xFFFFFFFFu;
constexpr uint32_t kMotionDeformed = 0x80000000u;
struct MotionPrevDev {
    float m[12];
    uint32_t identity;
    uint32_t pad[3];
};
static_assert(sizeof(MotionPrevDev) == 64, "MotionPrev layout");
struct MotionDev {
    const float* verts;
    const uint32_t *indices, *prim_geom, *first_prim, *geom_slot;
    const FlatGeomDev* geoms;
    const MotionPrevDev* prev;
};
struct MotionLaunch {
    GConstDev g;
    MotionDev m;
    const uint32_t* pixels;
    uint32_t npix, width;
    const float* hits;
    void* out;
    const float4* prev_pos = nullptr;
};
void launch_motion(hipStream_t st, const MotionLaunch& L);
void launch_snapshot_positions(hipStream_t st, const float* verts, uint32_t first, uint32_t n, float4* prev_pos);
constexpr uint32_t kDeformChunk = 1024;
void launch_compare_positions(hipStream_t st, const float* verts, const float4* prev_pos, const uint4* chunks, uint32_t n_chunks, uint32_t* flags);

hipError_t lbvh_make_top(hipStream_t st, const float4* nodes, uint32_t n_nodes, DevBuf<float4>& top, uint32_t* n_top);

}
```

### raytracer3_amd/csrc/rt3_lbvh.hip

```cpp
#include <hip/hip_runtime.h>
#include <hipcub/hipcub.hpp>

#include <atomic>
#include <chrono>
#include <cstdio>
#include <cstdlib>
#include <vector>

#include "rt3_bvh_device.hpp"
#include "rt3_internal.hpp"
#include "rt3_math.hpp"
#include "rt3_surface.hpp"

namespace rt3 {

__global__ void k_prim_geom(const uint32_t* first_prim, uint32_t n_geoms, uint32_t n, uint32_t* prim_geom) {
    for (uint32_t p = blockIdx.x * blockDim.x + threadIdx.x; p < n; p += gridDim.x * blockDim.x) {
        uint32_t lo = 0, hi = n_geoms;
        while (hi - lo > 1u) {
            uint32_t mid = (lo + hi) >> 1;
            if (first_prim[mid] <= p) lo = mid;
            else hi = mid;
        }
        prim_geom[p] = lo;
// ... 548 lines not shown
                        meta[k] = 8u | (cnt - 1u);
                        for (uint32_t t = 0; t < 3u * cnt; t++) tris_out[3 * (size_t)tcur + t] = tris_morton[3 * (size_t)first + t];
                        tcur += cnt;
                    } else {
                        meta[k] = 0u;
                    }
                }
                compact_node(qmn, qmx, meta, ns, 1u + cbase[i], tbase[i], nodes + kC48Stride * (size_t)o);
            } else {
                quantize_node(qmn, qmx, qref, ns, nodes + 4 * (size_t)o);
            }
        } else if (wide) {
            const float inf = INFINITY;
            const uint32_t sl[4] = {s0, s1, s2, s3};
            const bool vl[4] = {true, true, v2, v3};
#pragma unroll
            for (int k = 0; k < 4; k++) {
                if (vl[k]) {
                    slot_of(sl[k], lmin, lmax, nbox, range_lo, range_cnt, newidx, live, mn, mx, ref);
                } else {
                    mn[0] = mn[1] = mn[2] = inf;
                    mx[0] = mx[1] = mx[2] = -inf;
                    ref = 0xFFFFFFFFu;
                }
                nodes[8 * (size_t)o + 2 * k] = make_float4(mn[0], mn[1], mn[2], mx[0]);
                nodes[8 * (size_t)o + 2 * k + 1] = make_float4(mx[1], mx[2], __uint_as_float(ref), 0.0f);
            }
        } else {
            float mn1[3], mx1[3];
            uint32_t ref1;
            slot_of(s0, lmin, lmax, nbox, range_lo, range_cnt, newidx, live, mn, mx, ref);
            slot_of(s1, lmin, lmax, nbox, range_lo, range_cnt, newidx, live, mn1, mx1, ref1);
            nodes[4 * (size_t)o + 0] = make_float4(mn[0], mn[1], mn[2], mx[0]);
            nodes[4 * (size_t)o + 1] = make_float4(mx[1], mx[2], mn1[0], mn1[1]);
            nodes[4 * (size_t)o + 2] = make_float4(mn1[2], mx1[0], mx1[1], mx1[2]);
            nodes[4 * (size_t)o + 3] = make_float4(__uint_as_float(ref), __uint_as_float(ref1), 0.0f, 0.0f);
        }
    }
}

__global__ void k_top_cache(const float4* __restrict__ nodes, uint32_t n_nodes, uint32_t* __restrict__ top_words , uint32_t* __restrict__ n_top_out) {
    if (blockIdx.x != 0 || threadIdx.x != 0) return;
    uint32_t queue[kTopCacheNodes];
    uint32_t head = 0, tail = 0;
    if (n_nodes) queue[tail++] = 0u;
    while (head < tail) {
        const uint32_t node = queue[head];
        const uint32_t* src = reinterpret_cast<const uint32_t*>(nodes + 4 * (size_t)node);
        uint32_t* dst = top_words + 16 * (size_t)head;
        for (int k = 0; k < 16; k++) dst[k] = src[k];
        for (int k = 0; k < 4; k++) {
            const uint32_t ref = src[10 + k];
            if (ref == 0xFFFFFFFFu || (ref & 0x80000000u)) continue;
            if (tail < kTopCacheNodes) {
                dst[10 + k] = 0x40000000u | tail;
                queue[tail++] = ref;
            }
        }
        head++;
    }
    *n_top_out = tail;
}

hipError_t lbvh_make_top(hipStream_t st, const float4* nodes, uint32_t n_nodes, DevBuf<float4>& top, uint32_t* n_top) {
    *n_top = 0;
    if (!top) {
        hipError_t e = top.alloc_bytes((size_t)kTopCacheNodes * 64);
        if (e != hipSuccess) return e;
    }
    DevBuf<uint32_t> d_ntop;
    hipError_t e = d_ntop.alloc_bytes(4);
    if (e != hipSuccess) return e;
    hipLaunchKernelGGL(k_top_cache, dim3(1), dim3(1), 0, st, nodes, n_nodes, (uint32_t*)top.get(), d_ntop.get());
    e = hipMemcpyAsync(n_top, d_ntop.get(), 4, hipMemcpyDeviceToHost, st);
    if (e == hipSuccess) e = hipStreamSynchronize(st);
    return e;
}

__global__ void k_single(const float* lmin, const float* lmax, int wide, int quant, float4* nodes) {
    const float inf = INFINITY;
    if (wide && quant) {
        float qmn[4][3], qmx[4][3];
        uint32_t qref[4] = {0x80000000u, 0, 0, 0};
        for (int j = 0; j < 3; j++) {
            qmn[0][j] = lmin[j];
            qmx[0][j] = lmax[j];
        }
        const uint32_t qmeta[4] = {8u, 7u, 7u, 7u};
        if (quant == 2) compact_node(qmn, qmx, qmeta, 1, 1u, 0u, nodes);
        else quantize_node(qmn, qmx, qref, 1, nodes);
    } else if (wide) {
        nodes[0] = make_float4(lmin[0], lmin[1], lmin[2], lmax[0]);
        nodes[1] = make_float4(lmax[1], lmax[2], __uint_as_float(0x80000000u), 0.0f);
        for (int k = 1; k < 4; k++) {
            nodes[2 * k] = make_float4(inf, inf, inf, -inf);
            nodes[2 * k + 1] = make_float4(-inf, -inf, __uint_as_float(0xFFFFFFFFu), 0.0f);
        }
    } else {
        nodes[0] = make_float4(lmin[0], lmin[1], lmin[2], lmax[0]);
        nodes[1] = make_float4(lmax[1], lmax[2], inf, inf);
        nodes[2] = make_float4(inf, -inf, -inf, -inf);
        nodes[3] = make_float4(__uint_as_float(0x80000000u), __uint_as_float(0xFFFFFFFFu), 0.0f, 0.0f);
    }
}

namespace {
struct LbvhScratch {
    float *bmin, *bmax, *lmin, *lmax, *nbox;
    uint32_t *bounds, *vals_in, *vals_out, *left, *right, *pint, *pleaf, *arrive, *rlo, *rcnt, *keep, *newidx, *levels, *live;
    uint64_t *keys_in, *keys_out;
    char *sort_tmp, *scan_tmp;
    size_t sort_bytes, scan_bytes;
    uint32_t *dk, *newpos;
    float *dc, *lmin2, *lmax2;
    float4* tris_dp;
    float4* tris_morton;
    uint32_t *n_int, *n_ltri, *cbase, *tbase;
    float4* tris_stage;
    SahTopScratch sah;
    uint32_t *fr_a, *fr_b, *fr_n;
    uint32_t* n_top;
};
hipError_t plan_scratch(hipStream_t st, uint32_t n, int quant, int collapse, bool sah_top, bool top_cache, BufLayout& plan, LbvhScratch* s) {
    const size_t nn = n > 1 ? n - 1 : 1;
    plan.add(&s->bmin, 3 * (size_t)n).add(&s->bmax, 3 * (size_t)n).add(&s->lmin, 3 * (size_t)n).add(&s->lmax, 3 * (size_t)n).add(&s->nbox, 6 * nn);
    plan.add(&s->bounds, 12).add(&s->keys_in, n).add(&s->keys_out, n).add(&s->vals_in, n).add(&s->vals_out, n);
    plan.add(&s->left, nn).add(&s->right, nn).add(&s->pint, nn).add(&s->pleaf, n).add(&s->arrive, nn).add(&s->rlo, nn).add(&s->rcnt, nn);
    plan.add(&s->keep, nn).add(&s->newidx, nn).add(&s->levels, 1).add(&s->live, nn);
    if (collapse == 2 && n > 1) {
        plan.add(&s->dk, nn).add(&s->dc, 3 * nn).add(&s->newpos, n).add(&s->lmin2, 3 * (size_t)n).add(&s->lmax2, 3 * (size_t)n);
        plan.add(&s->tris_dp, 3 * (size_t)n);
    }
    if (quant != 2 || n == 1) plan.add(&s->tris_stage, 3 * (size_t)n);
    if (quant == 2 && n > 1)
        plan.add(&s->tris_morton, 3 * (size_t)n).add(&s->n_int, nn).add(&s->n_ltri, nn).add(&s->cbase, nn).add(&s->tbase, nn);
    RT3_TRY(hipcub::DeviceRadixSort::SortPairs(nullptr, s->sort_bytes, s->keys_in, s->keys_out, s->vals_in, s->vals_out, (int)n, 0, 63, st));
    plan.add(&s->sort_tmp, s->sort_bytes);
    if (n == 1) return hipSuccess;
    if (sah_top) RT3_TRY(sah_top_plan(st, n, plan, &s->sah));
    if (collapse) plan.add(&s->fr_a, nn).add(&s->fr_b, nn).add(&s->fr_n, nn + 18);
    RT3_TRY(hipcub::DeviceScan::ExclusiveSum(nullptr, s->scan_bytes, s->keep, s->newidx, (int)nn, st));
    plan.add(&s->scan_tmp, s->scan_bytes);
    if (top_cache) plan.add(&s->n_top, 1);
    return hipSuccess;
}
}

uint64_t next_arena_serial() {
    static std::atomic<uint64_t> serial{0};
    return ++serial;
}

hipError_t lbvh_build(hipStream_t st, GeomTables t, uint32_t n, uint32_t leaf_max, uint32_t node_width, uint32_t node_quant, uint32_t collapse_mode,
                      uint32_t sah_top, DevBuf<char>& scratch, LbvhResult* out, const uint2* geom_mask) {
    *out = LbvhResult{};
    out->n_tris = n;
    const int wide = node_width == 4, quant = wide ? (node_quant > 2 ? 2 : (int)node_quant) : 0, collapse = wide ? (collapse_mode > 2 ? 2 : (int)collapse_mode) : 0;
    const bool dp = collapse == 2;
    out->node_bytes = (wide && !quant) ? 128u : (quant == 2 ? 16u * kC48Stride : 64u);
    out->layout = !wide ? kLayoutBinary64 : (quant == 2 ? kLayoutWide48Q : (quant ? kLayoutWide64Q : kLayoutWide128));
    if (n == 0) return hipSuccess;
    const uint32_t nn = n > 1 ? n - 1 : 1;
    LbvhScratch s = {};
    {
        BufLayout plan;
        RT3_TRY(plan_scratch(st, n, quant, collapse, sah_top != 0, wide && quant == 1, plan, &s));
        RT3_TRY(scratch.grow_bytes(plan.bytes()));
        RT3_TRY(plan.carve(scratch));
        if (getenv("RT3_TRACE_BUILD"))
            fprintf(stderr, "rt3 build: %u triangles, scratch %zu bytes (radix sort %zu, scan %zu)\n", n, plan.bytes(), s.sort_bytes, s.scan_bytes);
    }
    const unsigned grid = (unsigned)(((uint64_t)n + 255) / 256 > 4096 ? 4096 : ((uint64_t)n + 255) / 256);
    uint32_t init_bounds[12];
    uint32_t tail[2] = {0, 0};
    for (int k = 0; k < 3; k++) {
        init_bounds[k] = 0xFFFFFFFFu;
        init_bounds[3 + k] = 0u;
        init_bounds[6 + k] = 0xFFFFFFFFu;
        init_bounds[9 + k] = 0u;
    }
    RT3_TRY(hipMemcpyAsync(s.bounds, init_bounds, sizeof(init_bounds), hipMemcpyHostToDevice, st));
    RT3_TRY(hipMemsetAsync(s.arrive, 0, (size_t)nn * 4, st));
    RT3_TRY(hipMemsetAsync(s.levels, 0, 4, st));
    hipLaunchKernelGGL(k_prim_bounds, dim3(grid > 512 ? 512 : grid), dim3(256), 0, st, t.verts, t.indices, t.geoms, t.prim_geom, t.first_prim, n, s.bmin, s.bmax, s.bounds);
    hipLaunchKernelGGL(k_morton, dim3(grid), dim3(256), 0, st, s.bmin, s.bmax, s.bounds, n, s.keys_in, s.vals_in);
    RT3_TRY(hipcub::DeviceRadixSort::SortPairs(s.sort_tmp, s.sort_bytes, s.keys_in, s.keys_out, s.vals_in, s.vals_out, (int)n, 0, 63, st));
    hipLaunchKernelGGL(k_leaves, dim3(grid), dim3(256), 0, st, t.verts, t.indices, t.geoms, t.prim_geom, t.first_prim, s.vals_out, s.bmin, s.bmax, s.bounds, n,
                       s.tris_dp ? s.tris_dp : (s.tris_morton ? s.tris_morton : s.tris_stage), s.lmin, s.lmax, geom_mask);
    if (n == 1) {
        RT3_TRY(out->alloc_arena(out->node_bytes, 1, st));
        hipLaunchKernelGGL(k_single, dim3(1), dim3(1), 0, st, s.lmin, s.lmax, wide, quant, out->nodes.get());
        RT3_TRY(hipMemcpyAsync(out->tris.get(), s.tris_stage, 48, hipMemcpyDeviceToDevice, st));
        out->n_nodes = 1;
        out->max_depth = 2;
        RT3_TRY(hipGetLastError());
        RT3_TRY(hipStreamSynchronize(st));
    } else {
        hipLaunchKernelGGL(k_hierarchy, dim3(grid), dim3(256), 0, st, s.keys_out, (int)n, s.left, s.right, s.pint, s.pleaf, s.rlo, s.rcnt);
        const uint32_t T_sah = dp ? sah_top : (sah_top > leaf_max ? sah_top : leaf_max);
        const bool lite = sah_top && T_sah <= 64;
        if (lite) hipLaunchKernelGGL(k_refit_clusters, dim3(grid), dim3(256), 0, st, s.rlo, s.rcnt, s.lmin, s.lmax, nn, T_sah, s.nbox);
        else hipLaunchKernelGGL(k_refit, dim3(grid), dim3(256), 0, st, s.left, s.right, s.pint, s.pleaf, s.lmin, s.lmax, n, s.nbox, s.arrive);
        if (sah_top) {
            bool relinked = false;
            const auto t0 = std::chrono::steady_clock::now();
            RT3_TRY(sah_top_relink_gpu(st, nn, s.left, s.right, s.rcnt, s.pint, s.pleaf, s.lmin, s.lmax, s.nbox, T_sah, s.sah, &relinked));
            if (!relinked && lite) {
                RT3_TRY(hipMemsetAsync(s.arrive, 0, (size_t)nn * 4, st));
                hipLaunchKernelGGL(k_refit, dim3(grid), dim3(256), 0, st, s.left, s.right, s.pint, s.pleaf, s.lmin, s.lmax, n, s.nbox, s.arrive);
            }
            if (getenv("RT3_TRACE_BUILD")) {
                RT3_TRY(hipStreamSynchronize(st));
                fprintf(stderr, "rt3 build: device SAH top (incl. GPU LBVH drain) %.2f ms\n",
                        std::chrono::duration<double, std::milli>(std::chrono::steady_clock::now() - t0).count());
            }
        }
        const auto t3 = std::chrono::steady_clock::now();
        if (dp) {
            RT3_TRY(hipMemsetAsync(s.arrive, 0, (size_t)nn * 4, st));
            hipLaunchKernelGGL(k_dp_up, dim3(grid), dim3(256), 0, st, s.left, s.right, s.pint, s.pleaf, s.lmin, s.lmax, s.nbox, n, leaf_max, s.rcnt, s.dc, s.dk,
                               s.live, s.arrive);
            const unsigned g3 = (unsigned)(((uint64_t)n + nn + 255) / 256 > 4096 ? 4096 : ((uint64_t)n + nn + 255) / 256);
            hipLaunchKernelGGL(k_tree_order, dim3(g3), dim3(256), 0, st, s.left, s.right, s.pint, s.pleaf, s.rcnt, n, nn, s.newpos, s.rlo);
            float4* tris_to = quant == 2 ? s.tris_morton : s.tris_stage;
            hipLaunchKernelGGL(k_tree_reorder, dim3(g3), dim3(256), 0, st, s.newpos, n, nn, s.tris_dp, tris_to, s.lmin, s.lmax, s.lmin2, s.lmax2, s.left, s.right);
            s.lmin = s.lmin2;
            s.lmax = s.lmax2;
        } else {
            hipLaunchKernelGGL(k_live_flags, dim3(grid), dim3(256), 0, st, s.rcnt, nn, leaf_max, s.live);
        }
        if (collapse) {
            const uint32_t root = 0, one = 1;
            const size_t n_cnt = (size_t)nn + 18;
            RT3_TRY(hipMemsetAsync(s.keep, 0, (size_t)nn * 4, st));
            RT3_TRY(hipMemsetAsync(s.fr_n, 0, n_cnt * 4, st));
            RT3_TRY(hipMemcpyAsync(s.fr_a, &root, 4, hipMemcpyHostToDevice, st));
            RT3_TRY(hipMemcpyAsync(s.fr_n, &one, 4, hipMemcpyHostToDevice, st));
            const unsigned g2 = (unsigned)((nn + 255) / 256 > 1024 ? 1024 : (nn + 255) / 256);
            uint32_t level = 0, last = 1, wide_levels = 0;
            while (last > 0 && level + 16 < n_cnt) {
                for (int burst = 0; burst < 16; burst++, level++) {
                    hipLaunchKernelGGL(k_wide_level, dim3(g2), dim3(256), 0, st, s.left, s.right, s.live, s.nbox, s.dk, collapse, s.fr_a, s.fr_n + level, s.keep,
                                       s.fr_b, s.fr_n + level + 1);
                    std::swap(s.fr_a, s.fr_b);
                }
                RT3_TRY(hipMemcpyAsync(&last, s.fr_n + level, 4, hipMemcpyDeviceToHost, st));
                RT3_TRY(hipStreamSynchronize(st));
            }
            std::vector<uint32_t> h_cnt(level + 1);
            RT3_TRY(hipMemcpyAsync(h_cnt.data(), s.fr_n, (size_t)(level + 1) * 4, hipMemcpyDeviceToHost, st));
            RT3_TRY(hipStreamSynchronize(st));
            while (wide_levels <= level && h_cnt[wide_levels] > 0) wide_levels++;
            const uint32_t lv = wide_levels + 1;
            RT3_TRY(hipMemcpyAsync(s.levels, &lv, 4, hipMemcpyHostToDevice, st));
            RT3_TRY(hipStreamSynchronize(st));
        } else {
            hipLaunchKernelGGL(k_keep_flags, dim3(grid), dim3(256), 0, st, s.pint, s.live, nn, wide, s.keep, s.levels);
        }
        RT3_TRY(hipcub::DeviceScan::ExclusiveSum(s.scan_tmp, s.scan_bytes, s.keep, s.newidx, (int)nn, st));
        RT3_TRY(hipMemcpyAsync(&tail[0], s.newidx + (nn - 1), 4, hipMemcpyDeviceToHost, st));
        RT3_TRY(hipMemcpyAsync(&tail[1], s.keep + (nn - 1), 4, hipMemcpyDeviceToHost, st));
        RT3_TRY(hipMemcpyAsync(&out->max_depth, s.levels, 4, hipMemcpyDeviceToHost, st));
        RT3_TRY(hipStreamSynchronize(st));
        out->n_nodes = tail[0] + tail[1];
        RT3_TRY(out->alloc_arena((size_t)out->n_nodes * out->node_bytes, n, st));
        if (quant != 2) RT3_TRY(hipMemcpyAsync(out->tris.get(), s.tris_stage, (size_t)n * 48, hipMemcpyDeviceToDevice, st));
        if (quant == 2) {
            hipLaunchKernelGGL(k_child_counts, dim3(grid), dim3(256), 0, st, s.left, s.right, s.rcnt, s.nbox, s.keep, nn, s.live, s.dk, collapse, s.n_int, s.n_ltri);
            RT3_TRY(hipcub::DeviceScan::ExclusiveSum(s.scan_tmp, s.scan_bytes, s.n_int, s.cbase, (int)nn, st));
            RT3_TRY(hipcub::DeviceScan::ExclusiveSum(s.scan_tmp, s.scan_bytes, s.n_ltri, s.tbase, (int)nn, st));
            hipLaunchKernelGGL(k_assign_index, dim3(grid), dim3(256), 0, st, s.left, s.right, s.live, s.nbox, s.keep, nn, s.dk, collapse, s.cbase, s.newidx);
        }
        hipLaunchKernelGGL(k_emit_nodes, dim3(grid), dim3(256), 0, st, s.left, s.right, s.rlo, s.rcnt, s.keep, s.newidx, s.lmin, s.lmax, s.nbox, nn, s.live, s.dk,
                           wide, quant, collapse, out->nodes.get(), s.cbase, s.tbase, s.tris_morton, out->tris.get());
        if (wide && quant == 1) {
            RT3_TRY(out->top.alloc_bytes((size_t)kTopCacheNodes * 64));
            hipLaunchKernelGGL(k_top_cache, dim3(1), dim3(1), 0, st, out->nodes.get(), out->n_nodes, (uint32_t*)out->top.get(), s.n_top);
            RT3_TRY(hipMemcpyAsync(&out->n_top, s.n_top, 4, hipMemcpyDeviceToHost, st));
            RT3_TRY(hipStreamSynchronize(st));
        }
        RT3_TRY(hipGetLastError());
        RT3_TRY(hipStreamSynchronize(st));
        if (getenv("RT3_TRACE_BUILD"))
            fprintf(stderr, "rt3 build: collapse + emit %.2f ms\n", std::chrono::duration<double, std::milli>(std::chrono::steady_clock::now() - t3).count());
    }
    return hipSuccess;
}

}
```

### raytracer3_amd/csrc/rt3_scene.hip

```cpp
#include <hip/hip_runtime.h>

#include <cmath>
#include <cstring>
#include <algorithm>
#include <string>
#include <vector>

#include "rt3_ctx.hpp"

using namespace rt3;

static int validate_geometry(rt3_ctx* c, const rt3_geometry_info* g, const uint32_t* prim_counts, uint32_t n,
                             std::vector<std::pair<uint32_t, uint32_t>>* spans = nullptr) {
    for (uint32_t i = 0; i < n; i++) {
        if ((uint64_t)g[i].index_offset + 3ull * prim_counts[i] > c->scene.n_indices)
            return fail(c, RT3_E_INVALID, "geometry " + std::to_string(i) + ": index range exceeds the index buffer");
        uint32_t mx = 0, mn = 0xFFFFFFFFu;
        for (uint64_t k = 0; k < 3ull * prim_counts[i]; k++) {
            uint32_t v = c->scene.h_indices[g[i].index_offset + k];
            mx = v > mx ? v : mx;
            mn = v < mn ? v : mn;
        }
        if (prim_counts[i] && (uint64_t)g[i].vertex_offset + mx >= (uint64_t)c->scene.n_verts)
            return fail(c, RT3_E_INVALID, "geometry " + std::to_string(i) + ": vertex range exceeds the vertex buffer (set vertices and indices before geometry)");
// ... 204 lines not shown
    forget_snapshot(c);
    return RT3_OK;
}
int rt3_scene_set_alpha_cutoffs(rt3_ctx* c, const float* cutoffs, uint32_t n) {
    if (!c || (!cutoffs && n)) return fail(c, RT3_E_INVALID, "alpha cutoffs NULL");
    if (n != 0 && n != c->scene.n_geoms)
        return fail(c, RT3_E_INVALID, "alpha cutoffs: n must be 0 or the geometry count of rt3_scene_set_geometry (" + std::to_string(c->scene.n_geoms) + ")");
    for (uint32_t i = 0; i < n; i++)
        if (!(cutoffs[i] >= 0.0f && cutoffs[i] <= 1.0f)) return fail(c, RT3_E_INVALID, "alpha cutoff " + std::to_string(i) + " is not in [0, 1]");
    c->scene.h_cutoffs.clear();
    if (std::any_of(cutoffs, cutoffs + n, [](float v) { return v > 0.0f; })) c->scene.h_cutoffs.assign(cutoffs, cutoffs + n);
    invalidate_topology(c);
    return RT3_OK;
}
int rt3_scene_set_material_textures(rt3_ctx* c, const rt3_material_textures* m, uint32_t n) {
    if (!c || (!m && n)) return fail(c, RT3_E_INVALID, "material textures NULL");
    if (n != 0 && n != c->scene.n_geoms)
        return fail(c, RT3_E_INVALID, "material textures: n must be 0 or the geometry count of rt3_scene_set_geometry (" + std::to_string(c->scene.n_geoms) + ")");
    for (uint32_t i = 0; i < n; i++) {
        if (m[i].metallic_roughness_texture < -1 || m[i].normal_texture < -1 || m[i].emissive_texture < -1)
            return fail(c, RT3_E_INVALID, "material textures: entry " + std::to_string(i) + " has a texture index below -1");
        if (!(std::fabs(m[i].normal_scale) <= kFloatMax)) return fail(c, RT3_E_INVALID, "material textures: normal_scale " + std::to_string(i) + " is not finite");
    }
    c->scene.h_mat_tex.clear();
    if (std::any_of(m, m + n, [](const rt3_material_textures& e) { return e.metallic_roughness_texture >= 0 || e.normal_texture >= 0 || e.emissive_texture >= 0; }))
        c->scene.h_mat_tex.assign(m, m + n);
    invalidate_topology(c);
    return RT3_OK;
}
static uint32_t host_rgb9e5(const float* c) {
    auto bits = [](float f) { uint32_t u; memcpy(&u, &f, 4); return u; };
    auto from_bits = [](uint32_t u) { float f; memcpy(&f, &u, 4); return f; };
    const float mx = (511.0f / 512.0f) * 65536.0f;
    auto clampf = [&](float v) { v = v > 0.0f ? v : 0.0f; return v < mx ? v : mx; };
    const float rc = clampf(c[0]), gc = clampf(c[1]), bc = clampf(c[2]);
    const float m1 = gc > bc ? gc : bc, maxrgb = rc > m1 ? rc : m1;
    const int fl2 = (int)((bits(maxrgb) & 0x7F800000u) >> 23) - 127;
    int exp_shared = (fl2 > -16 ? fl2 : -16) + 1 + 15;
    float denom = from_bits((uint32_t)(exp_shared - 15 - 9 + 127) << 23);
    const int maxm = (int)std::floor(maxrgb / denom + 0.5f);
    if (maxm == 512) {
        denom *= 2.0f;
        exp_shared += 1;
    }
    const int rm = (int)std::floor(rc / denom + 0.5f), gm = (int)std::floor(gc / denom + 0.5f), bm = (int)std::floor(bc / denom + 0.5f);
    return ((uint32_t)rm << 23) | ((uint32_t)gm << 14) | ((uint32_t)bm << 5) | (uint32_t)exp_shared;
}
static void host_rgb9e5_decode(uint32_t v, float* c) {
    const uint32_t sb = (uint32_t)((int)(v & 31u) - 24 + 127) << 23;
    float scale;
    memcpy(&scale, &sb, 4);
    c[0] = (float)((v >> 23) & 511u) * scale;
    c[1] = (float)((v >> 14) & 511u) * scale;
    c[2] = (float)((v >> 5) & 511u) * scale;
}
int rt3_scene_set_sky(rt3_ctx* c, const float* rgb, uint32_t w, uint32_t h) {
    if (!c || !rgb || !w || !h) return fail(c, RT3_E_INVALID, "sky NULL / empty");
    if (w > 65535 || h > 65535) return fail(c, RT3_E_INVALID, "sky larger than 65535 texels per side");
    HIPC(c, hipSetDevice(c->device));
    const size_t n = (size_t)w * h;
    for (size_t i = 0; i < 3 * n; i++)
        if (!(rgb[i] >= 0.0f && rgb[i] <= kFloatMax))
            return fail(c, RT3_E_INVALID, "sky texel " + std::to_string(i / 3) + " is negative or not finite (clamp the image before uploading it)");
    std::vector<uint32_t> texq(n), alias(n);
    std::vector<float> pdf(n), marg(h);
    std::vector<double> rows(h), f(w), sc(w), real(w);
    std::vector<uint32_t> small(w), large(w);
    double total = 0.0;
    for (uint32_t y = 0; y < h; y++) {
        const double st = std::sin(3.14159265358979323846 * ((double)y + 0.5) / (double)h);
        double acc = 0.0;
        for (uint32_t x = 0; x < w; x++) {
            const size_t i = (size_t)y * w + x;
            texq[i] = host_rgb9e5(rgb + 3 * i);
            float p[3];
            host_rgb9e5_decode(texq[i], p);
            const float lum = p[0] * 0.299f + p[1] * 0.587f + p[2] * 0.114f;
            f[x] = ((double)lum + 1e-6) * st;
            acc += f[x];
        }
        rows[y] = acc;
        total += acc;
        uint32_t ns = 0, nl = 0;
        uint32_t* al = alias.data() + (size_t)y * w;
        for (uint32_t x = 0; x < w; x++) {
            sc[x] = f[x] * (double)w / acc;
            if (sc[x] < 1.0) small[ns++] = x;
            else large[nl++] = x;
        }
        for (uint32_t x = 0; x < w; x++) al[x] = 65535u | (x << 16);
        while (ns && nl) {
            const uint32_t a = small[--ns], g = large[--nl];
            const double q = sc[a] * 65536.0;
            int64_t q16 = (int64_t)std::floor(q + 0.5) - 1;
            q16 = q16 < 0 ? 0 : (q16 > 65535 ? 65535 : q16);
            al[a] = (uint32_t)q16 | (g << 16);
            sc[g] = (sc[g] + sc[a]) - 1.0;
            if (sc[g] < 1.0) small[ns++] = g;
            else large[nl++] = g;
        }
        for (uint32_t x = 0; x < w; x++) real[x] = 0.0;
        for (uint32_t x = 0; x < w; x++) {
            const double Q = (double)((al[x] & 0xFFFFu) + 1u) / 65536.0;
            real[x] += Q;
            real[al[x] >> 16] += 1.0 - Q;
        }
        for (uint32_t x = 0; x < w; x++) pdf[(size_t)y * w + x] = (float)real[x];
    }
    double run = 0.0;
    for (uint32_t y = 0; y < h; y++) {
        run += rows[y];
        marg[y] = (float)(run / total);
        const double rowp = rows[y] / total * (double)h;
        for (uint32_t x = 0; x < w; x++) pdf[(size_t)y * w + x] = (float)((double)pdf[(size_t)y * w + x] * rowp);
    }
    marg[h - 1] = 1.0f;
    std::vector<uint32_t> gmarg(h);
    {
        std::vector<uint32_t> g(h + 1);
        uint32_t i = 0;
        for (uint32_t k = 0; k <= h; k++) {
            const float thr = (float)k / (float)h;
            while (i < h - 1 && !(marg[i] > thr)) i++;
            g[k] = i;
        }
        for (uint32_t k = 0; k < h; k++) {
            const uint32_t lo = g[k > 0 ? k - 1 : 0], hi = g[k + 1] > h - 1 ? h - 1 : g[k + 1];
            gmarg[k] = lo | (hi << 16);
        }
    }
    std::vector<float> margp((size_t)h + 4);
    margp[0] = 0.0f;
    std::memcpy(margp.data() + 1, marg.data(), (size_t)h * 4);
    margp[h + 1] = margp[h + 2] = margp[h + 3] = 2.0f;
    const uint32_t wt = (w + 3) / 4, ht = (h + 3) / 4;
    std::vector<uint2> tiled((size_t)wt * ht * 16, make_uint2(0u, 0u));
    for (uint32_t y = 0; y < h; y++)
        for (uint32_t x = 0; x < w; x++) {
            uint32_t pb;
            memcpy(&pb, &pdf[(size_t)y * w + x], 4);
            tiled[((size_t)(y >> 2) * wt + (x >> 2)) * 16 + (((y & 3u) << 2) | (x & 3u))] = make_uint2(texq[(size_t)y * w + x], pb);
        }
    if (int r = dev_alloc(c, c->scene.d_guide_marg, gmarg.size())) return r;
    if (int r = dev_alloc(c, c->scene.d_sky_alias, alias.size())) return r;
    if (int r = dev_alloc(c, c->scene.d_sky, tiled.size())) return r;
    if (int r = dev_alloc(c, c->scene.d_cdf_marg, margp.size())) return r;
    HIPC(c, hipMemcpy(c->scene.d_guide_marg.get(), gmarg.data(), gmarg.size() * 4, hipMemcpyHostToDevice));
    HIPC(c, hipMemcpy(c->scene.d_sky_alias.get(), alias.data(), alias.size() * 4, hipMemcpyHostToDevice));
    HIPC(c, hipMemcpy(c->scene.d_sky.get(), tiled.data(), tiled.size() * 8, hipMemcpyHostToDevice));
    HIPC(c, hipMemcpy(c->scene.d_cdf_marg.get(), margp.data(), margp.size() * 4, hipMemcpyHostToDevice));
    c->scene.sky_w = w;
    c->scene.sky_h = h;
    c->scene.sky_wt = wt;
    return RT3_OK;
}
int rt3_scene_set_bluenoise(rt3_ctx* c, const uint8_t* rgba, uint32_t w, uint32_t h) {
    if (!c || !rgba || !w || !h) return fail(c, RT3_E_INVALID, "bluenoise NULL / empty");
    HIPC(c, hipSetDevice(c->device));
    if (int r = dev_alloc(c, c->scene.d_bn, (size_t)w * h * 4)) return r;
    HIPC(c, hipMemcpy(c->scene.d_bn.get(), rgba, (size_t)w * h * 4, hipMemcpyHostToDevice));
    c->scene.bn_w = w;
    c->scene.bn_h = h;
    c->scene.bn_stamp++;
    return RT3_OK;
}
int rt3_scene_set_texture(rt3_ctx* c, uint32_t index, const uint8_t* rgba, uint32_t w, uint32_t h) {
    if (!c || !rgba || !w || !h || w > 16384 || h > 16384 || index > 4096) return fail(c, RT3_E_INVALID, "texture: NULL / bad size / index");
    if (index >= c->scene.h_tex.size()) {
        c->scene.h_tex.resize(index + 1);
        c->scene.tex_w.resize(index + 1, 0);
        c->scene.tex_h.resize(index + 1, 0);
    }
    c->scene.h_tex[index].assign(rgba, rgba + (size_t)w * h * 4);
    c->scene.tex_w[index] = w;
    c->scene.tex_h[index] = h;
    c->scene.tex_dirty = true;
    return RT3_OK;
}
int rt3_sky_download(rt3_ctx* c, uint32_t* alias, uint32_t* texels, float* marg, float* pdf) {
    if (!c || !c->scene.d_sky) return fail(c, RT3_E_STATE, "no sky set");
    const uint32_t w = c->scene.sky_w, h = c->scene.sky_h, wt = c->scene.sky_wt, ht = (h + 3) / 4;
    if (alias) HIPC(c, hipMemcpy(alias, c->scene.d_sky_alias.get(), (size_t)w * h * 4, hipMemcpyDeviceToHost));
    if (marg) HIPC(c, hipMemcpy(marg, c->scene.d_cdf_marg.get() + 1, (size_t)h * 4, hipMemcpyDeviceToHost));
    if (texels || pdf) {
        std::vector<uint2> tiled((size_t)wt * ht * 16);
        HIPC(c, hipMemcpy(tiled.data(), c->scene.d_sky.get(), tiled.size() * 8, hipMemcpyDeviceToHost));
        for (uint32_t y = 0; y < h; y++)
            for (uint32_t x = 0; x < w; x++) {
                const uint2 t = tiled[((size_t)(y >> 2) * wt + (x >> 2)) * 16 + (((y & 3u) << 2) | (x & 3u))];
                if (texels) texels[(size_t)y * w + x] = t.x;
                if (pdf) memcpy(&pdf[(size_t)y * w + x], &t.y, 4);
            }
    }
    return RT3_OK;
}

static int check_matrix(rt3_ctx* c, const float* m, uint32_t i, const char* what, const char* not_finite, const char* bad_row) {
    for (int k = 0; k < 16; k++)
        if (!(std::fabs(m[k]) <= 1.0e18f)) return fail(c, RT3_E_INVALID, what + std::to_string(i) + not_finite);
    if (m[3] != 0.0f || m[7] != 0.0f || m[11] != 0.0f || m[15] != 1.0f) return fail(c, RT3_E_INVALID, what + std::to_string(i) + bad_row);
    return RT3_OK;
}
int rt3_scene_set_instances(rt3_ctx* c, const rt3_instance* inst, uint32_t n) {
    if (!c || (!inst && n)) return fail(c, RT3_E_INVALID, "instances NULL");
    for (uint32_t i = 0; i < n; i++)
        if (int r = check_matrix(c, inst[i].transform, i, "instance ", ": transform is not finite (or beyond 1e18)",
                                 ": the last row of the transform must be (0, 0, 0, 1) (VkTransformMatrixKHR is 3 x 4 too)"))
            return r;
    c->scene.h_instances.assign(inst, inst + n);
    invalidate_accel(c);
    return RT3_OK;
}
int rt3_scene_set_prev_transforms(rt3_ctx* c, const float* transforms, uint32_t n) {
    if (!c || (!transforms && n)) return fail(c, RT3_E_INVALID, "previous transforms NULL");
    for (uint32_t i = 0; i < n; i++)
        if (int r = check_matrix(c, transforms + 16 * (size_t)i, i, "previous transform ", " is not finite (or beyond 1e18)",
                                 ": the last row must be (0, 0, 0, 1), as for an instance's matrix"))
            return r;
    c->scene.prev_transforms.assign(transforms, transforms + 16 * (size_t)n);
    motion_tables_stale(c);
    return RT3_OK;
}

}
```

### raytracer3_amd/csrc/rt3_trace.hip

```cpp
#include <hip/hip_fp16.h>
#include <hip/hip_runtime.h>

#include <type_traits>

#include "rt3_hit.hpp"
#include "rt3_internal.hpp"
#include "rt3_math.hpp"
#include "rt3_surface.hpp"

namespace rt3 {

constexpr int kLdsStack = 12;
constexpr uint32_t kTopFlag = 0x40000000u;
constexpr int kSpill = 64 - kLdsStack;
constexpr uint32_t kMaxSteps = 1u << 20;

constexpr uint32_t kEmptySlot = 0xFFFFFFFFu;
constexpr float kTopPadRel = 2.44140625e-4f;

struct Cand {
    float tn;
    uint32_t ref;
};
__device__ __forceinline__ void cswap(Cand& a, Cand& b) {
    bool sw = b.tn < a.tn;
    float ta = a.tn;
    uint32_t ra = a.ref;
    a.tn = sw ? b.tn : a.tn;
    a.ref = sw ? b.ref : a.ref;
    b.tn = sw ? ta : b.tn;
    b.ref = sw ? ra : b.ref;
}
__device__ __forceinline__ void pin(float4& q) { asm volatile("" : "+v"(q.x), "+v"(q.y), "+v"(q.z), "+v"(q.w)); }
__device__ __forceinline__ V3 cross_exact(V3 a, V3 b) { return V3{(a.y * b.z) - (a.z * b.y), (a.z * b.x) - (a.x * b.z), (a.x * b.y) - (a.y * b.x)}; }
template <bool MASK = false>
__device__ __forceinline__ void tri_test_nb(float4 q0, float4 q1, float4 q2, V3 o, V3 d, float inv_dd, float tmin, Hit& best, const AlphaDev& alpha = AlphaDev{}) {
    const V3 A = v3(q0.x, q0.y, q0.z) - o, B = v3(q0.w, q1.x, q1.y) - o, C = v3(q1.z, q1.w, q2.x) - o;
    const float U = dot_fma(d, cross_exact(B, C)), V = dot_fma(d, cross_exact(C, A)), W = dot_fma(d, cross_exact(A, B));
    const float det = U + (V + W);
    const float inv = 1.0f / det;
    const float w = U * inv, u = V * inv, v = W * inv;
    const float T = __builtin_fmaf(U, dot_fma(A, d), __builtin_fmaf(V, dot_fma(B, d), W * dot_fma(C, d)));
    const float t = (T * inv) * inv_dd;
    const uint32_t prim = __float_as_uint(q2.y);
    constexpr float kEdgeEps = 9.5367431640625e-07f;
    const bool inside = (w >= -kEdgeEps) & (u >= -kEdgeEps) & (v >= -kEdgeEps);
    bool ok = (det != 0.0f) & inside & (t > tmin) & ((t < best.t) | ((t == best.t) & (prim < best.prim)));
    if (MASK && ok && q2.z != 0.0f) ok = alpha_counts(alpha, __float_as_uint(q2.w), q2.z, prim, u, v);
    best.t = ok ? t : best.t;
    best.u = ok ? u : best.u;
    best.v = ok ? v : best.v;
    best.prim = ok ? prim : best.prim;
}

__constant__ uint32_t g_pool_chunk = 256;
__constant__ uint32_t g_refill_lanes = 12;
void set_refill_lanes(uint32_t v) { (void)hipMemcpyToSymbol(HIP_SYMBOL(g_refill_lanes), &v, 4); }
void set_pool_chunk(uint32_t v) { (void)hipMemcpyToSymbol(HIP_SYMBOL(g_pool_chunk), &v, 4); }
static unsigned g_trace_max_blocks = kExtendMaxBlocks;
void set_trace_blocks(uint32_t v) { g_trace_max_blocks = v; }

constexpr uint32_t kTopNodes = kTopCacheNodes;
__device__ __forceinline__ bool load_top(float4* s_top, const float4* __restrict__ top, uint32_t n_top) {
    if (top == nullptr || n_top == 0u) return false;
    n_top = n_top < kTopNodes ? n_top : kTopNodes;
    for (uint32_t i = threadIdx.x; i < 4u * n_top; i += kExtendBlock) s_top[i] = top[i];
    __syncthreads();
    return true;
}

__device__ __forceinline__ bool slab_test_sorted(uint32_t p, uint32_t q, V3 A, V3 B, float tmin, float tbest, float& tn_out) {
    const float nx = __builtin_fmaf((float)(p & 0xFFu), A.x, B.x), ny = __builtin_fmaf((float)((p >> 8) & 0xFFu), A.y, B.y),
                nz = __builtin_fmaf((float)((p >> 16) & 0xFFu), A.z, B.z), fx = __builtin_fmaf((float)(p >> 24), A.x, B.x),
                fy = __builtin_fmaf((float)(q & 0xFFu), A.y, B.y), fz = __builtin_fmaf((float)((q >> 8) & 0xFFu), A.z, B.z);
    const float tn = __builtin_fmaxf(__builtin_fmaxf(nx, ny), __builtin_fmaxf(nz, tmin));
    const float tf = __builtin_fminf(__builtin_fminf(fx, fy), __builtin_fminf(fz, tbest));
    tn_out = tn;
    return tn <= tf;
}

__device__ __forceinline__ bool slab_test_sorted_pad(uint32_t p, uint32_t q, V3 A, V3 B, V3 pad, float tmin, float tbest, float& tn_out) {
    const float nx = __builtin_fmaf((float)(p & 0xFFu), A.x, B.x) - pad.x, ny = __builtin_fmaf((float)((p >> 8) & 0xFFu), A.y, B.y) - pad.y,
                nz = __builtin_fmaf((float)((p >> 16) & 0xFFu), A.z, B.z) - pad.z, fx = __builtin_fmaf((float)(p >> 24), A.x, B.x) + pad.x,
                fy = __builtin_fmaf((float)(q & 0xFFu), A.y, B.y) + pad.y, fz = __builtin_fmaf((float)((q >> 8) & 0xFFu), A.z, B.z) + pad.z;
    const float tn = __builtin_fmaxf(__builtin_fmaxf(nx, ny), __builtin_fmaxf(nz, tmin));
    const float tf = __builtin_fminf(__builtin_fminf(fx, fy), __builtin_fminf(fz, tbest));
    tn_out = tn;
    return tn <= tf;
}

struct LaneRay {
    V3 o, d, inv;
    float tmin, inv_dd;
    Hit best;
    uint32_t cur, leaf_k, index, steps, cn, ct, cl;
    int sp;
    float pay0, pay1;
    float pay2, pay3;
    uint32_t sel_p0, sel_q0, sel_p1, sel_q1;
};

template <int MODE, bool COUNT, int LAYOUT, bool TWO = false, bool RANGE = false, bool MASK = false, typename Finish>
__device__ __forceinline__ void trace_stream(const float4* __restrict__ nodes, uint32_t tri_off,
                                             const float* __restrict__ rays, size_t stride, uint32_t n, uint32_t* __restrict__ work_counter,
                                             uint32_t* __restrict__ lds, Finish finish, bool any_payload = false, bool ext_payload = false, const float4* top_lds = nullptr, bool use_top = false,
                                             const float2* __restrict__ any_contrib = nullptr, const float* __restrict__ any_tmax = nullptr,
                                             const AlphaDev& alpha = AlphaDev{}) {
    constexpr bool ANY = MODE == 1;
    constexpr bool WIDE = LAYOUT == kLayoutWide128;
    constexpr bool WIDEQ = LAYOUT == kLayoutWide64Q || LAYOUT == kLayoutWide48Q;
    constexpr bool C48 = LAYOUT == kLayoutWide48Q;
    uint32_t pool_next = 0, pool_end = 0;
    bool queue_empty = false;
    const uint32_t lane = __lane_id();
    const unsigned long long lanes_below = (1ull << lane) - 1ull;
    const uint32_t n_waves = gridDim.x * (blockDim.x >> 6);
    const uint32_t kRefillLanes = g_refill_lanes,
                   kPoolChunk = (n < 2u * n_waves * g_pool_chunk && g_pool_chunk >= 128u) ? ((g_pool_chunk >> 1) & ~63u) : g_pool_chunk;
    const uint32_t wave_id = blockIdx.x * (blockDim.x >> 6) + (uint32_t)__builtin_amdgcn_readfirstlane((int)(threadIdx.x >> 6));
    bool first_chunk = true;
    uint32_t spill[kSpill];
    LaneRay r;
    r.o = r.d = r.inv = v3(0.0f, 0.0f, 0.0f);
    r.tmin = 0.0f;
    r.inv_dd = 1.0f;
    r.best = Hit{0.0f, 0.0f, 0.0f, kMiss};
    r.cur = r.leaf_k = r.index = r.steps = r.cn = r.ct = r.cl = 0u;
    r.sp = 0;
    r.pay0 = r.pay1 = r.pay2 = r.pay3 = 0.0f;
    r.sel_p0 = r.sel_q0 = r.sel_p1 = r.sel_q1 = 0u;
    bool busy = false;
    V3 tl_o = v3(0.0f, 0.0f, 0.0f), tl_pad = v3(0.0f, 0.0f, 0.0f);
    uint32_t tl_mark = 0u, tl_rec = 0u, tl_base = 0u;
    bool tl_bottom = false;
    auto tl_world = [&]() {
        r.inv = v3(guarded_inverse(r.d.x), guarded_inverse(r.d.y), guarded_inverse(r.d.z));
        tl_o = r.o;
        const float pw = kTopPadRel * __builtin_fmaxf(__builtin_fmaxf(fabsf(r.o.x), fabsf(r.o.y)), fabsf(r.o.z));
        tl_pad = v3(pw * fabsf(r.inv.x), pw * fabsf(r.inv.y), pw * fabsf(r.inv.z));
        tl_bottom = false;
    };
    auto tl_sels = [&]() {
        const uint32_t sx = r.inv.x < 0.0f ? 1u : 0u, sy = r.inv.y < 0.0f ? 1u : 0u, sz = r.inv.z < 0.0f ? 1u : 0u;
        const uint32_t nx = 3u * sx, ny = 1u + 3u * sy, nz = 2u + 3u * sz, fx = 3u - 3u * sx, fy = 4u - 3u * sy, fz = 5u - 3u * sz;
        r.sel_p0 = nx | (ny << 8) | (nz << 16) | (fx << 24);
        r.sel_q0 = fy | (fz << 8);
        r.sel_p1 = r.sel_p0 + 0x02020202u;
        r.sel_q1 = r.sel_q0 + 0x00000202u;
    };
    for (;;) {
        const unsigned long long m_idle = __ballot(!busy);
        if (pool_next >= pool_end && !queue_empty && m_idle != 0ull) {
            uint32_t base = 0;
            if (first_chunk) {
                base = wave_id * kPoolChunk;
                first_chunk = false;
            } else {
                if (lane == 0) base = atomicAdd(work_counter, kPoolChunk);
                base = __builtin_amdgcn_readfirstlane(base);
                const unsigned long long b64 = (unsigned long long)n_waves * kPoolChunk + base;
                base = b64 > 0xFFFFFFFFull ? 0xFFFFFFFFu : (uint32_t)b64;
            }
            queue_empty = base >= n;
            pool_next = base < n ? base : n;
            pool_end = (n - pool_next) > kPoolChunk ? pool_next + kPoolChunk : n;
        }
        if (m_idle != 0ull && pool_next < pool_end && ((uint32_t)__popcll(m_idle) >= kRefillLanes || m_idle == ~0ull)) {
            const uint32_t idx = pool_next + (uint32_t)__popcll(m_idle & lanes_below);
            if (!busy && idx < pool_end) {
                const float4 ro = reinterpret_cast<const float4*>(rays)[idx], rd = reinterpret_cast<const float4*>(rays)[stride + idx];
                r.o = v3(ro.x, ro.y, ro.z);
                r.d = v3(rd.x, rd.y, rd.z);
                const bool payload = ANY ? any_payload : ext_payload;
                r.tmin = payload ? kRayTMin : ro.w;
                r.best = Hit{payload ? kBackgroundDepth : rd.w, 0.0f, 0.0f, kMiss};
                if (RANGE) r.best.t = any_tmax[idx];
                r.pay0 = ro.w;
                r.pay1 = rd.w;
                if (ANY && any_contrib != nullptr) {
                    const float2 c2 = any_contrib[idx];
                    r.pay2 = c2.x;
                    r.pay3 = c2.y;
                }
                r.inv = v3(guarded_inverse(r.d.x), guarded_inverse(r.d.y), guarded_inverse(r.d.z));
                r.inv_dd = 1.0f / dot_fma(r.d, r.d);
                if (LAYOUT == kLayoutWide64Q) {
                    const uint32_t sx = r.inv.x < 0.0f ? 1u : 0u, sy = r.inv.y < 0.0f ? 1u : 0u, sz = r.inv.z < 0.0f ? 1u : 0u;
                    const uint32_t nx = 3u * sx, ny = 1u + 3u * sy, nz = 2u + 3u * sz, fx = 3u - 3u * sx, fy = 4u - 3u * sy, fz = 5u - 3u * sz;
                    r.sel_p0 = nx | (ny << 8) | (nz << 16) | (fx << 24);
                    r.sel_q0 = fy | (fz << 8);
                    r.sel_p1 = r.sel_p0 + 0x02020202u;
                    r.sel_q1 = r.sel_q0 + 0x00000202u;
                }
                r.cur = (LAYOUT == kLayoutWide64Q && use_top) ? kTopFlag : 0u;
                if (TWO) tl_world();
                r.leaf_k = 0u;
                r.sp = 0;
                r.index = idx;
                r.steps = 0u;
                r.cn = r.ct = r.cl = 0u;
                busy = true;
                const bool finite_ray = fabsf(r.o.x) <= kFloatMax && fabsf(r.o.y) <= kFloatMax && fabsf(r.o.z) <= kFloatMax && fabsf(r.d.x) <= kFloatMax &&
                                        fabsf(r.d.y) <= kFloatMax && fabsf(r.d.z) <= kFloatMax;
                if (nodes == nullptr || !finite_ray) {
                    finish(r.index, r.best, 0u, 0u, 0u, r.pay0, r.pay1, r.pay2, r.pay3);
                    busy = false;
                }
            }
            const uint32_t taken = (uint32_t)__popcll(m_idle);
            pool_next = pool_next + taken < pool_end ? pool_next + taken : pool_end;
        }
        if (__ballot(busy) == 0ull && pool_next >= pool_end && queue_empty) break;
        if (busy) {
        const bool is_leaf = (r.cur & 0x80000000u) != 0u;
        const uint32_t first = r.cur & 0x0FFFFFFFu, cnt = ((r.cur >> 28) & 7u) + 1u;
        const bool cached = LAYOUT == kLayoutWide64Q && !is_leaf && (r.cur & kTopFlag) != 0u;
        const bool is_inst = TWO && is_leaf && !tl_bottom;
        const bool is_tri = is_leaf && !is_inst;
        constexpr uint32_t kNodeBytes = 16u * (WIDE ? 8 : (C48 ? kC48Stride : 4));
        uint32_t off_tri = tri_off + 48u * (first + r.leaf_k), off_node = kNodeBytes * (cached ? 0u : (is_inst ? first : r.cur));
        asm volatile("" : "+v"(off_tri), "+v"(off_node));
        const uint32_t off = is_tri ? off_tri : off_node;
        const float4* p = reinterpret_cast<const float4*>(reinterpret_cast<const char*>(nodes) + off);
        float4 q0, q1, q2, q3, q4, q5, q6, q7;
        if (TWO && is_tri) {
            const float4* pm = reinterpret_cast<const float4*>(reinterpret_cast<const char*>(nodes) + 64u * (tl_rec + 1u));
            q4 = pm[0];
            q5 = pm[1];
            q6 = pm[2];
        }
        if (LAYOUT == kLayoutWide64Q && cached) {
            const float4* t = top_lds + 4 * (r.cur & 0xFFFFu);
            q0 = t[0];
            q1 = t[1];
            q2 = t[2];
            q3 = t[3];
        } else {
            q0 = p[0];
            q1 = p[1];
            q2 = p[2];
            q3 = C48 ? make_float4(0.0f, 0.0f, 0.0f, 0.0f) : p[3];
        }
        if (WIDE) {
            q4 = p[4];
            q5 = p[5];
            q6 = p[6];
            q7 = p[7];
        }
        if (TWO && is_tri) { pin(q4); pin(q5); pin(q6); }
        pin(q0); pin(q1); pin(q2);
        if (!C48) pin(q3);
        if (WIDE) { pin(q4); pin(q5); pin(q6); pin(q7); }
        bool pop = false, done = false;
        const V3 o = r.o, d = r.d, inv = r.inv;
        const float tmin = r.tmin;
        if (TWO && is_inst) {
            if (COUNT) r.cn++;
            const float mi[12] = {q0.x, q0.y, q0.z, q0.w, q1.x, q1.y, q1.z, q1.w, q2.x, q2.y, q2.z, q2.w};
            const V3 oo = transform_point(mi, o), dd = transform_vector(mi, d);
            r.inv = v3(guarded_inverse(dd.x), guarded_inverse(dd.y), guarded_inverse(dd.z));
            tl_sels();
            const float om = __builtin_fmaxf(__builtin_fmaxf(__builtin_fmaxf(fabsf(o.x), fabsf(o.y)), __builtin_fmaxf(fabsf(o.z), fabsf(oo.x))),
                                             __builtin_fmaxf(fabsf(oo.y), fabsf(oo.z)));
            const float pb = __builtin_fmaf(q3.w, om, q3.z);
            tl_pad = v3(pb * fabsf(r.inv.x), pb * fabsf(r.inv.y), pb * fabsf(r.inv.z));
            tl_o = oo;
            tl_mark = (uint32_t)r.sp;
            tl_rec = first;
            tl_base = __float_as_uint(q3.y);
            tl_bottom = true;
            r.cur = __float_as_uint(q3.x);
        } else if (is_leaf) {
            if (COUNT) r.ct++;
            if (TWO) {
                const float fm[12] = {q4.x, q4.y, q4.z, q4.w, q5.x, q5.y, q5.z, q5.w, q6.x, q6.y, q6.z, q6.w};
                V3 a = v3(q0.x, q0.y, q0.z), b = v3(q0.w, q1.x, q1.y), c = v3(q1.z, q1.w, q2.x);
                if ((tl_base >> 31) == 0u) {
                    a = transform_point(fm, a);
                    b = transform_point(fm, b);
                    c = transform_point(fm, c);
                }
                const uint32_t gp = __float_as_uint(q2.y) + (tl_base & 0x7FFFFFFFu);
                tri_test_nb<MASK>(make_float4(a.x, a.y, a.z, b.x), make_float4(b.y, b.z, c.x, c.y),
                                  make_float4(c.z, __uint_as_float(gp), MASK ? q2.z : 0.0f, MASK ? q2.w : 0.0f), o, d, r.inv_dd, tmin, r.best, alpha);
            } else {
                tri_test_nb<MASK>(q0, q1, q2, o, d, r.inv_dd, tmin, r.best, alpha);
            }
            r.leaf_k++;
            if (WIDE) {
                if (r.leaf_k < cnt && !(ANY && r.best.prim != kMiss)) {
                    if (COUNT) r.ct++;
                    tri_test_nb(q3, q4, q5, o, d, r.inv_dd, tmin, r.best);
                    r.leaf_k++;
                }
            }
            if (ANY && r.best.prim != kMiss) done = true;
            if (r.leaf_k >= cnt) {
                r.leaf_k = 0;
                pop = true;
            }
        } else {
            if (COUNT) {
                r.cn++;
                r.cl += cached ? 1u : 0u;
            }
            if (WIDE || WIDEQ) {
                const float kInf = __builtin_huge_valf();
                float t0, t1, t2, t3;
                uint32_t r0, r1, r2, r3;
                bool h0, h1, h2, h3;
                if (WIDEQ) {
                    const uint32_t ex = __float_as_uint(q0.w);
                    const V3 A = C48 ? v3(__uint_as_float((ex & 0xFFu) << 23) * inv.x, __uint_as_float(((ex >> 8) & 0xFFu) << 23) * inv.y,
                                          __uint_as_float(((ex >> 16) & 0xFFu) << 23) * inv.z)
                                     : v3(q0.w * inv.x, q3.z * inv.y, q3.w * inv.z);
                    const V3 ob = TWO ? tl_o : o;
                    const V3 B = v3((q0.x - ob.x) * inv.x, (q0.y - ob.y) * inv.y, (q0.z - ob.z) * inv.z);
                    const uint32_t w0 = __float_as_uint(q1.x), w1 = __float_as_uint(q1.y), w2 = __float_as_uint(q1.z), w3 = __float_as_uint(q1.w),
                                   w4 = __float_as_uint(q2.x), w5 = __float_as_uint(q2.y);
                    if (C48) {
                        const uint32_t wa = __float_as_uint(q2.z), wb = __float_as_uint(q2.w);
                        const uint32_t m0 = (ex >> 24) & 15u, m1 = ex >> 28, m2 = wa >> 28, m3 = wb >> 28;
                        uint32_t nb = wa & 0x0FFFFFFFu, tb = wb & 0x0FFFFFFFu;
#define RT3_REF48(m, out)                                                         \
    {                                                                             \
        const bool in_ = (m) == 0u, lf_ = ((m)&8u) != 0u;                         \
        out = in_ ? nb : (lf_ ? (0x80000000u | (((m)&7u) << 28) | tb) : kEmptySlot); \
        nb += in_ ? 1u : 0u;                                                      \
        tb += lf_ ? ((m)&7u) + 1u : 0u;                                           \
    }
                        RT3_REF48(m0, r0)
                        RT3_REF48(m1, r1)
                        RT3_REF48(m2, r2)
                        RT3_REF48(m3, r3)
#undef RT3_REF48
                    } else {
                        r0 = __float_as_uint(q2.z);
                        r1 = __float_as_uint(q2.w);
                        r2 = __float_as_uint(q3.x);
                        r3 = __float_as_uint(q3.y);
                    }
#define RT3_Q(w, b) ((float)(((w) >> (8 * (b))) & 0xFFu))
#define RT3_SLABQ(lx, ly, lz, hx, hy, hz, tn) \
    slab_test_q(__builtin_fmaf(lx, A.x, B.x), __builtin_fmaf(hx, A.x, B.x), __builtin_fmaf(ly, A.y, B.y), __builtin_fmaf(hy, A.y, B.y), \
                __builtin_fmaf(lz, A.z, B.z), __builtin_fmaf(hz, A.z, B.z), tmin, r.best.t, tn)
                    if (LAYOUT == kLayoutWide64Q) {
#define RT3_SLABS(wlo, whi, selp, selq, tn)                                                                                                    \
    (TWO ? slab_test_sorted_pad(__builtin_amdgcn_perm(whi, wlo, selp), __builtin_amdgcn_perm(whi, wlo, selq), A, B, tl_pad, tmin, r.best.t, tn) \
         : slab_test_sorted(__builtin_amdgcn_perm(whi, wlo, selp), __builtin_amdgcn_perm(whi, wlo, selq), A, B, tmin, r.best.t, tn))
                        h0 = RT3_SLABS(w0, w1, r.sel_p0, r.sel_q0, t0) & (r0 != kEmptySlot);
                        h1 = RT3_SLABS(w1, w2, r.sel_p1, r.sel_q1, t1) & (r1 != kEmptySlot);
                        h2 = RT3_SLABS(w3, w4, r.sel_p0, r.sel_q0, t2) & (r2 != kEmptySlot);
                        h3 = RT3_SLABS(w4, w5, r.sel_p1, r.sel_q1, t3) & (r3 != kEmptySlot);
#undef RT3_SLABS
                    } else {
                    h0 = RT3_SLABQ(RT3_Q(w0, 0), RT3_Q(w0, 1), RT3_Q(w0, 2), RT3_Q(w0, 3), RT3_Q(w1, 0), RT3_Q(w1, 1), t0) & (r0 != kEmptySlot);
                    h1 = RT3_SLABQ(RT3_Q(w1, 2), RT3_Q(w1, 3), RT3_Q(w2, 0), RT3_Q(w2, 1), RT3_Q(w2, 2), RT3_Q(w2, 3), t1) & (r1 != kEmptySlot);
                    h2 = RT3_SLABQ(RT3_Q(w3, 0), RT3_Q(w3, 1), RT3_Q(w3, 2), RT3_Q(w3, 3), RT3_Q(w4, 0), RT3_Q(w4, 1), t2) & (r2 != kEmptySlot);
                    h3 = RT3_SLABQ(RT3_Q(w4, 2), RT3_Q(w4, 3), RT3_Q(w5, 0), RT3_Q(w5, 1), RT3_Q(w5, 2), RT3_Q(w5, 3), t3) & (r3 != kEmptySlot);
                    }
#undef RT3_Q
#undef RT3_SLABQ
                } else {
                    r0 = __float_as_uint(q1.z);
                    r1 = __float_as_uint(q3.z);
                    r2 = __float_as_uint(q5.z);
                    r3 = __float_as_uint(q7.z);
                    h0 = slab_test_hw(v3(q0.x, q0.y, q0.z), v3(q0.w, q1.x, q1.y), o, inv, tmin, r.best.t, t0) & (r0 != kEmptySlot);
                    h1 = slab_test_hw(v3(q2.x, q2.y, q2.z), v3(q2.w, q3.x, q3.y), o, inv, tmin, r.best.t, t1) & (r1 != kEmptySlot);
                    h2 = slab_test_hw(v3(q4.x, q4.y, q4.z), v3(q4.w, q5.x, q5.y), o, inv, tmin, r.best.t, t2) & (r2 != kEmptySlot);
                    h3 = slab_test_hw(v3(q6.x, q6.y, q6.z), v3(q6.w, q7.x, q7.y), o, inv, tmin, r.best.t, t3) & (r3 != kEmptySlot);
                }
                Cand c0{h0 ? (ANY ? -t0 : t0) : kInf, r0}, c1{h1 ? (ANY ? -t1 : t1) : kInf, r1};
                Cand c2{h2 ? (ANY ? -t2 : t2) : kInf, r2}, c3{h3 ? (ANY ? -t3 : t3) : kInf, r3};
                const uint32_t nh = (uint32_t)h0 + (uint32_t)h1 + (uint32_t)h2 + (uint32_t)h3;
                cswap(c0, c1);
                cswap(c2, c3);
                cswap(c0, c2);
                cswap(c1, c3);
                cswap(c1, c2);
                if (nh > 3) {
                    if (r.sp < kLdsStack) lds[r.sp * kExtendBlock] = c3.ref;
                    else spill[r.sp - kLdsStack] = c3.ref;
                    ++r.sp;
                }
                if (nh > 2) {
                    if (r.sp < kLdsStack) lds[r.sp * kExtendBlock] = c2.ref;
                    else spill[r.sp - kLdsStack] = c2.ref;
                    ++r.sp;
                }
                if (nh > 1) {
                    if (r.sp < kLdsStack) lds[r.sp * kExtendBlock] = c1.ref;
                    else spill[r.sp - kLdsStack] = c1.ref;
                    ++r.sp;
                }
                r.cur = c0.ref;
                pop = nh == 0;
            } else {
                float tn0, tn1;
                uint32_t r0 = __float_as_uint(q3.x), r1 = __float_as_uint(q3.y);
                bool h0 = slab_test_hw(v3(q0.x, q0.y, q0.z), v3(q0.w, q1.x, q1.y), o, inv, tmin, r.best.t, tn0) & (r0 != kEmptySlot);
                bool h1 = slab_test_hw(v3(q1.z, q1.w, q2.x), v3(q2.y, q2.z, q2.w), o, inv, tmin, r.best.t, tn1) & (r1 != kEmptySlot);
                bool near1 = tn1 < tn0;
                if (h0 & h1) {
                    uint32_t far = near1 ? r0 : r1;
                    if (r.sp < kLdsStack) lds[r.sp * kExtendBlock] = far;
                    else spill[r.sp - kLdsStack] = far;
                    ++r.sp;
                }
                r.cur = (h0 & h1) ? (near1 ? r1 : r0) : (h0 ? r0 : r1);
                pop = !(h0 | h1);
            }
        }
        if (pop && !done) {
            if (TWO && tl_bottom && (uint32_t)r.sp == tl_mark) {
                tl_world();
                tl_sels();
            }
            if (r.sp == 0) {
                done = true;
            } else {
                --r.sp;
                if (r.sp < kLdsStack) {
                    r.cur = lds[r.sp * kExtendBlock];
                } else {
                    r.cur = spill[r.sp - kLdsStack];
                    __builtin_amdgcn_sched_barrier(0);
                }
            }
        }
        if (++r.steps >= kMaxSteps) done = true;
        if (done) {
            finish(r.index, r.best, r.cn, r.ct, r.cl, r.pay0, r.pay1, r.pay2, r.pay3);
            busy = false;
        }
        }
    }
}

template <bool COUNT>
struct TraceCounts {
    uint32_t *cnt_nodes, *cnt_tris;
    unsigned long long nodes = 0, tris = 0, lds = 0;
    __device__ __forceinline__ void ray(uint32_t i, uint32_t cn, uint32_t ct, uint32_t cl) {
        if (!COUNT) return;
        if (cnt_nodes) cnt_nodes[i] = cn;
        if (cnt_tris) cnt_tris[i] = ct;
        nodes += cn;
        tris += ct;
        lds += cl;
    }
    __device__ __forceinline__ void add_totals(unsigned long long* totals, unsigned long long* lds_total) {
        if (!COUNT || !totals) return;
        atomicAdd(&totals[0], nodes);
        atomicAdd(&totals[1], tris);
        if (lds_total) atomicAdd(lds_total, lds);
    }
};

template <bool MASK>
struct AlphaArg {
    AlphaDev a;
    __device__ __forceinline__ AlphaDev get() const { return a; }
};
template <>
struct AlphaArg<false> {
    __device__ __forceinline__ AlphaDev get() const { return AlphaDev{}; }
};

template <bool COUNT, int LAYOUT, bool MASK = false>
__global__ __launch_bounds__(kExtendBlock) void k_extend(const float4* __restrict__ nodes, uint32_t tri_off, const float4* __restrict__ top, uint32_t n_top,
                                                         const float* __restrict__ rays, size_t stride,
                                                         const uint32_t* __restrict__ count_ptr, uint32_t count_imm,
                                                         float* __restrict__ hits, uint32_t* __restrict__ cnt_nodes,
                                                         uint32_t* __restrict__ cnt_tris, unsigned long long* __restrict__ totals,
                                                         uint32_t* __restrict__ work_counter, int payload, AlphaArg<MASK> alpha,
                                                         unsigned long long* __restrict__ lds_total) {
    __shared__ uint32_t stack[kLdsStack * kExtendBlock];
    __shared__ float4 s_top[4 * kTopNodes];
    const bool use_top = load_top(s_top, top, n_top);
    const uint32_t n = count_ptr ? *count_ptr : count_imm;
    TraceCounts<COUNT> counts{cnt_nodes, cnt_tris};
    auto finish = [&](uint32_t i, const Hit& h, uint32_t cn, uint32_t ct, uint32_t cl, float, float, float, float) {
        reinterpret_cast<float4*>(hits)[i] = make_float4(h.t, h.u, h.v, __uint_as_float(h.prim));
        counts.ray(i, cn, ct, cl);
    };
    trace_stream<0, COUNT, LAYOUT == kLayoutTwoLevel ? kLayoutWide64Q : LAYOUT, LAYOUT == kLayoutTwoLevel, false, MASK>(
        nodes, tri_off, rays, stride, n, work_counter, stack + threadIdx.x, finish, false, payload != 0, s_top, use_top, nullptr, nullptr, alpha.get());
    counts.add_totals(totals, lds_total);
}

template <bool COUNT, int LAYOUT, bool RANGE = false, bool MASK = false>
__global__ __launch_bounds__(kExtendBlock) void k_shadow(const float4* __restrict__ nodes, uint32_t tri_off, const float4* __restrict__ top, uint32_t n_top,
                                                         const float* __restrict__ rays, size_t stride,
                                                         const uint32_t* __restrict__ count_ptr, uint32_t count_imm, AlphaArg<MASK> alpha,
                                                         const float* __restrict__ contrib, float* __restrict__ lacc,
                                                         uint32_t* __restrict__ occluded_out, uint32_t* __restrict__ cnt_nodes,
                                                         uint32_t* __restrict__ cnt_tris, unsigned long long* __restrict__ totals,
                                                         uint32_t* __restrict__ work_counter, unsigned long long* __restrict__ lds_total,
                                                         const float* __restrict__ tmax) {
    __shared__ uint32_t stack[kLdsStack * kExtendBlock];
    __shared__ float4 s_top[4 * kTopNodes];
    const bool use_top = load_top(s_top, top, n_top);
    const uint32_t n = count_ptr ? *count_ptr : count_imm;
    TraceCounts<COUNT> counts{cnt_nodes, cnt_tris};
    trace_stream<1, COUNT, LAYOUT == kLayoutTwoLevel ? kLayoutWide64Q : LAYOUT, LAYOUT == kLayoutTwoLevel, RANGE, MASK>(
        nodes, tri_off, rays, stride, n, work_counter, stack + threadIdx.x,
        [&](uint32_t i, const Hit& h, uint32_t cn, uint32_t ct, uint32_t cl, float c_r, float c_g, float c_b, float c_pid) {
            if (occluded_out) {
                occluded_out[i] = h.prim != kMiss ? 1u : 0u;
            } else if (h.prim == kMiss) {
                float4* L = reinterpret_cast<float4*>(lacc) + __float_as_uint(c_pid);
                float4 v = *L;
                *L = make_float4(v.x + c_r, v.y + c_g, v.z + c_b, 0.0f);
            }
            counts.ray(i, cn, ct, cl);
        },
        occluded_out == nullptr, false, s_top, use_top, occluded_out == nullptr ? reinterpret_cast<const float2*>(contrib) : nullptr, tmax,
        alpha.get());
    counts.add_totals(totals, lds_total);
}

template <typename Launch>
static void dispatch_traversal(bool count, int layout, bool masked, Launch launch) {
    auto by_mask = [&](auto c, auto l) {
        if (masked) launch(c, l, std::true_type{});
        else launch(c, l, std::false_type{});
    };
    auto by_layout = [&](auto c) {
        if (layout == kLayoutTwoLevel) by_mask(c, std::integral_constant<int, kLayoutTwoLevel>{});
        else if (layout == kLayoutWide48Q) launch(c, std::integral_constant<int, kLayoutWide48Q>{}, std::false_type{});
        else if (layout == kLayoutWide64Q) by_mask(c, std::integral_constant<int, kLayoutWide64Q>{});
        else if (layout == kLayoutWide128) launch(c, std::integral_constant<int, kLayoutWide128>{}, std::false_type{});
        else launch(c, std::integral_constant<int, kLayoutBinary64>{}, std::false_type{});
    };
    if (count) by_layout(std::true_type{});
    else by_layout(std::false_type{});
}
template <bool MASK>
static AlphaArg<MASK> alpha_arg(const TraceLaunch& L) {
    if constexpr (MASK) return AlphaArg<true>{L.alpha};
    else return AlphaArg<false>{};
}
void launch_extend(hipStream_t st, const LbvhResult& bvh, const TraceLaunch& L) {
    const unsigned grid = grid_for(L.n, kExtendBlock, g_trace_max_blocks);
    unsigned long long* const tot = L.totals ? L.totals + kTotExtendNodes : nullptr;
    unsigned long long* const lds_tot = L.totals ? L.totals + kTotExtendLds : nullptr;
    dispatch_traversal(L.count, bvh.layout, L.alpha.table != nullptr, [&](auto c, auto l, auto m) {
        hipLaunchKernelGGL((k_extend<decltype(c)::value, decltype(l)::value, decltype(m)::value>), dim3(grid), dim3(kExtendBlock), 0, st, bvh.nodes.get(),
                           bvh.tri_off, bvh.top.get(), bvh.n_top, L.rays, L.stride, L.count_ptr, L.n, L.hits, L.cnt_nodes, L.cnt_tris, tot, L.work_counter,
                           L.payload ? 1 : 0, alpha_arg<decltype(m)::value>(L), lds_tot);
    });
}
void launch_shadow(hipStream_t st, const LbvhResult& bvh, const TraceLaunch& L) {
    const unsigned grid = grid_for(L.n, kExtendBlock, g_trace_max_blocks);
    unsigned long long* const tot = L.totals ? L.totals + kTotShadowNodes : nullptr;
    unsigned long long* const lds_tot = L.totals ? L.totals + kTotShadowLds : nullptr;
    dispatch_traversal(L.count, bvh.layout, L.alpha.table != nullptr, [&](auto c, auto l, auto m) {
        auto launch = [&](auto range) {
            hipLaunchKernelGGL((k_shadow<decltype(c)::value, decltype(l)::value, decltype(range)::value, decltype(m)::value>), dim3(grid), dim3(kExtendBlock), 0,
                               st, bvh.nodes.get(), bvh.tri_off, bvh.top.get(), bvh.n_top, L.rays, L.stride, L.count_ptr, L.n,
                               alpha_arg<decltype(m)::value>(L), L.contrib, L.lacc, L.occluded, L.cnt_nodes, L.cnt_tris, tot, L.work_counter, lds_tot, L.tmax);
        };
        if (L.tmax) launch(std::true_type{});
        else launch(std::false_type{});
    });
}

}
```

### raytracer3_amd/render_graph.py

```python
from __future__ import annotations

import ctypes as C
from dataclasses import dataclass, field

import numpy as np

from . import _lib as L

IMPORTED = 0xFFFFFFFFFFFFFFFF


class ImageSize:

    def __init__(self, kind, a=0, b=0):
        self.kind, self.a, self.b = kind, a, b

    FullScreen = None

    @staticmethod
    def FractionalFullScreen(dx, dy):
        return ImageSize("frac", dx, dy)

    @staticmethod
    def XY(x, y):
# ... 68 lines not shown


@dataclass
class NodeEdge:
    origin: int | None
    edge_type: str
    resource: int


@dataclass
class Node:
    name: str
    kind: str
    path: str
    entry: str
    size: object
    constants: object
    edges: list = field(default_factory=list)


class Context:

    def __init__(self, device: int = 0):
        self.lib = L.load()
        h = C.c_void_p()
        rc = self.lib.rt3_create(device, C.byref(h))
        if rc != 0:
            raise L.Rt3Error(rc, self.lib.rt3_last_error(None).decode())
        self.h = h

    def check(self, rc):
        if rc != 0:
            raise L.Rt3Error(rc, self.lib.rt3_last_error(self.h).decode())

    def close(self):
        if getattr(self, "h", None):
            self.lib.rt3_destroy(self.h)
            self.h = None

    def __del__(self):
        try:
            self.close()
        except Exception:
            pass

    @property
    def device_name(self):
        buf = C.create_string_buffer(256)
        self.check(self.lib.rt3_device_name(self.h, buf, 256))
        return buf.value.decode()

    def set_option(self, opt, value):
        self.check(self.lib.rt3_set_option(self.h, opt, int(value)))

    def upload_mesh(self, mesh):
        v = np.ascontiguousarray(mesh.vertices, np.float32)
        i = np.ascontiguousarray(mesh.indices, np.uint32)
        g = np.ascontiguousarray(mesh.geometries)
        pc = np.ascontiguousarray(mesh.prim_counts, np.uint32)
        self.check(self.lib.rt3_scene_set_vertices(self.h, v.ctypes.data, len(v)))
        self.check(self.lib.rt3_scene_set_indices(self.h, i.ctypes.data, len(i)))
        self.check(self.lib.rt3_scene_set_geometry(self.h, g.ctypes.data, pc.ctypes.data, len(g)))
        cut = getattr(mesh, "alpha_cutoffs", None)
        if cut is not None and np.any(np.asarray(cut) != 0):
            self.set_alpha_cutoffs(cut)
        mt = getattr(mesh, "material_textures", None)
        if mt is not None and len(mt) and any(np.any(mt[k] >= 0) for k in ("metallic_roughness_texture", "normal_texture", "emissive_texture")):
            self.set_material_textures(mt)
        for i, t in enumerate(getattr(mesh, "textures", None) or []):
            t = np.ascontiguousarray(t, np.uint8)
            self.check(self.lib.rt3_scene_set_texture(self.h, i, t.ctypes.data, t.shape[1], t.shape[0]))

    def set_alpha_cutoffs(self, cutoffs):
        c = np.ascontiguousarray(cutoffs, np.float32).reshape(-1)
        self.check(self.lib.rt3_scene_set_alpha_cutoffs(self.h, c.ctypes.data, len(c)))

    def set_material_textures(self, table):
        from .assets import MATERIAL_TEXTURES_DTYPE

        t = np.ascontiguousarray(table, MATERIAL_TEXTURES_DTYPE).reshape(-1)
        self.check(self.lib.rt3_scene_set_material_textures(self.h, t.ctypes.data if len(t) else None, len(t)))

    def set_instances(self, instances):
        arr = (L.Instance * max(1, len(instances)))()
        for k, (first, count, m) in enumerate(instances):
            arr[k].geometry_first, arr[k].geometry_count = int(first), int(count)
            arr[k].transform[:] = [float(x) for x in np.asarray(m, np.float32).T.ravel()]
        self.check(self.lib.rt3_scene_set_instances(self.h, C.byref(arr), len(instances)))

    def set_prev_transforms(self, transforms=None):
        n = 0 if transforms is None else len(transforms)
        arr = np.ascontiguousarray([np.asarray(m, np.float32).T.ravel() for m in transforms], np.float32).reshape(n, 16) if n else None
        self.check(self.lib.rt3_scene_set_prev_transforms(self.h, arr.ctypes.data if n else None, n))

    def snapshot_vertices(self):
        self.check(self.lib.rt3_scene_snapshot_vertices(self.h))

    def forget_prev_vertices(self):
        self.check(self.lib.rt3_scene_forget_prev_vertices(self.h))

    def deformed_geometries(self, n):
        flags = np.zeros(int(n), np.uint8)
        self.check(self.lib.rt3_scene_deformed_geometries(self.h, flags.ctypes.data, len(flags)))
        return flags.astype(bool)

    def set_sky(self, rgb):
        s = np.ascontiguousarray(rgb, np.float32)
        self.check(self.lib.rt3_scene_set_sky(self.h, s.ctypes.data, s.shape[1], s.shape[0]))

    def set_bluenoise(self, rgba):
        b = np.ascontiguousarray(rgba, np.uint8)
        self.check(self.lib.rt3_scene_set_bluenoise(self.h, b.ctypes.data, b.shape[1], b.shape[0]))

    def build_accel(self) -> int:
        out = C.c_uint32()
        self.check(self.lib.rt3_accel_build(self.h, C.byref(out)))
        return out.value

    def update_vertices(self, vertices, first=0):
        v = np.ascontiguousarray(vertices, np.float32).reshape(-1, 8)
        self.check(self.lib.rt3_scene_update_vertices(self.h, v.ctypes.data, int(first), len(v)))

    def refit_accel(self) -> int:
        out = C.c_uint32()
        self.check(self.lib.rt3_accel_refit(self.h, C.byref(out)))
        return out.value

    def light_info(self):
        n, t = C.c_uint32(), C.c_uint64()
        self.check(self.lib.rt3_light_info(self.h, C.byref(n), C.byref(t)))
        return n.value, t.value

    def light_download(self):
        n, _ = self.light_info()
        prim, area, mass = np.zeros(n, np.uint32), np.zeros(n, np.float32), np.zeros(n, np.uint32)
        self.check(self.lib.rt3_light_download(self.h, prim.ctypes.data, area.ctypes.data, mass.ctypes.data))
        return prim, area, mass

    def accel_import(self, nodes, tris):
        n = np.ascontiguousarray(nodes)
        t = np.ascontiguousarray(tris)
        self.check(self.lib.rt3_accel_import(self.h, n.ctypes.data, n.nbytes, t.ctypes.data, t.nbytes))

    def accel_info(self):
        a, b, c, d = C.c_uint32(), C.c_uint32(), C.c_uint32(), C.c_uint32()
        self.check(self.lib.rt3_accel_info(self.h, C.byref(a), C.byref(b), C.byref(c), C.byref(d)))
        return a.value, b.value, c.value, d.value

    def accel_levels(self):
        a, b, c, d = C.c_uint32(), C.c_uint32(), C.c_uint32(), C.c_uint64()
        self.check(self.lib.rt3_accel_levels(self.h, C.byref(a), C.byref(b), C.byref(c), C.byref(d)))
        return a.value, b.value, c.value, d.value

    def accel_download(self):
        nn, nt, _, nb = self.accel_info()
        nodes = np.empty((nn, nb // 4), np.uint32)
        tris = np.empty((nt, 12), np.uint32)
        self.check(self.lib.rt3_accel_download(self.h, nodes.ctypes.data, nodes.nbytes, tris.ctypes.data, tris.nbytes))
        return nodes, tris

    def sky_download(self, w, h):
        al, tx, cm, pu = np.empty((h, w), np.uint32), np.empty((h, w), np.uint32), np.empty(h, np.float32), np.empty((h, w), np.float32)
        self.check(self.lib.rt3_sky_download(self.h, al.ctypes.data, tx.ctypes.data, cm.ctypes.data, pu.ctypes.data))
        return al, tx, cm, pu

    def trace_rays(self, rays, any_hit=False, counts=False, repeat=1):
        rays = np.ascontiguousarray(rays, np.float32)
        n = rays.shape[1]
        t, u, v = (np.zeros(n, np.float32) for _ in range(3))
        prim = np.zeros(n, np.uint32)
        cn = np.zeros(n, np.uint32) if counts else None
        ct = np.zeros(n, np.uint32) if counts else None
        ms = C.c_double()
        self.check(self.lib.rt3_trace_rays(self.h, rays.ctypes.data, n, int(any_hit), t.ctypes.data, u.ctypes.data, v.ctypes.data, prim.ctypes.data,
                                           cn.ctypes.data if counts else None, ct.ctypes.data if counts else None, repeat, C.byref(ms)))
        return (t, u, v, prim, cn, ct, ms.value) if counts else (t, u, v, prim, ms.value)

    def selftest(self, op, inp, out_words, out_dtype=np.uint32):
        inp = np.ascontiguousarray(inp)
        assert inp.dtype.itemsize == 4
        n = inp.shape[0]
        out = np.zeros((n, out_words), out_dtype)
        self.check(self.lib.rt3_selftest_eval(self.h, op, inp.ctypes.data, n, out.ctypes.data))
        return out

    def set_denoise_params(self, params=None, **kw):
        if params is None and kw:
            params = L.DenoiseParams(**kw)
        self.check(self.lib.rt3_denoise_set_params(self.h, C.byref(params) if params is not None else None))

    def set_denoise_variance_input(self, moments_image=0):
        self.check(self.lib.rt3_denoise_set_variance_input(self.h, int(moments_image)))

    def set_temporal_params(self, params=None, **kw):
        if params is None and kw:
            params = L.TemporalParams(**kw)
        self.check(self.lib.rt3_temporal_set_params(self.h, C.byref(params) if params is not None else None))

    def set_prev_view(self, gconst=None):
        if gconst is None:
            self.check(self.lib.rt3_temporal_set_prev_view(self.h, None, 0))
        else:
            self.check(self.lib.rt3_temporal_set_prev_view(self.h, C.byref(gconst), C.sizeof(gconst)))

    def set_temporal_motion_input(self, motion_image=0):
        self.check(self.lib.rt3_temporal_set_motion_input(self.h, int(motion_image)))

    def stats_reset(self):
        self.check(self.lib.rt3_stats_reset(self.h))

    def stats(self) -> L.Stats:
        s = L.Stats()
        self.check(self.lib.rt3_stats_get(self.h, C.byref(s)))
        return s

    def wait(self):
        self.check(self.lib.rt3_frame_wait(self.h))

    def set_tile_partition(self, w, h, rank, n_ranks):
        self.check(self.lib.rt3_set_tile_partition(self.h, w, h, rank, n_ranks))

    def tile_pixel_count(self, rank, n_ranks):
        out = C.c_uint32()
        self.check(self.lib.rt3_tile_pixel_count(self.h, rank, n_ranks, C.byref(out)))
        return out.value

    def comm_unique_id(self) -> bytes:
        buf = C.create_string_buffer(L.COMM_ID_BYTES)
        rc = self.lib.rt3_comm_unique_id(buf)
        if rc != 0:
            raise L.Rt3Error(rc, self.lib.rt3_last_error(None).decode())
        return buf.raw

    def comm_init(self, uid: bytes, rank: int, n_ranks: int):
        assert len(uid) == L.COMM_ID_BYTES
        self.check(self.lib.rt3_comm_init(self.h, C.c_char_p(uid), rank, n_ranks))

    def comm_destroy(self):
        self.check(self.lib.rt3_comm_destroy(self.h))

    def gather_tiles(self, image, root=0):
        self.check(self.lib.rt3_gather_tiles(self.h, image, root))

    def gather_layout(self, image, root, n_ranks):
        off = (C.c_uint64 * (n_ranks + 1))()
        self.check(self.lib.rt3_gather_layout(self.h, image, root, n_ranks, off))
        return [int(x) for x in off]

    def gather_unpack(self, image, root, n_ranks, recv_device_ptr):
        self.check(self.lib.rt3_gather_unpack(self.h, image, root, n_ranks, C.c_void_p(recv_device_ptr)))


class NodeBuilder:

    def __init__(self, rg, name, kind):
        if any(n.name == name for n in rg.nodes):
            raise ValueError(f"Node name {name} allready used")
        self.rg = rg
        self.node = Node(name, kind, "", "main", WorkSize2D.FullScreen if kind == "raytracing" else DispatchSize.FullScreen, None)

    def shader(self, path):
        self.node.path = path
        return self

    def entry(self, entry):
        self.node.entry = entry
        return self

    def constants(self, c):
        self.node.constants = c
        return self

    def _edge(self, origin, handle, typ):
        if typ == "ShaderRead" and origin != IMPORTED:
            prev = [e for e in self.rg.nodes[origin].edges if e.resource == handle]
            if not prev:
                raise ValueError("Origin doesnt write to handle")
            if prev[0].edge_type == "ShaderRead":
                raise ValueError("Origin contains handle but does not write to it")
        self.node.edges.append(NodeEdge(None if origin == IMPORTED else origin, typ, handle))
        return self

    def read(self, origin, handle):
        return self._edge(origin, handle, "ShaderRead")

    def write(self, last_read, handle):
        return self._edge(last_read, handle, "ShaderWrite")

    def read_write(self, origin, handle):
        return self._edge(origin, handle, "ShaderReadWrite")

    def _build(self):
        seen = set()
        for e in self.node.edges:
            if e.resource in seen:
                raise ValueError(f"resource: {e.resource} is duplicate")
            seen.add(e.resource)
        self.rg.nodes.append(self.node)
        return len(self.rg.nodes) - 1

    def launch(self, size=None):
        assert self.node.kind == "raytracing"
        self.node.size = size or WorkSize2D.FullScreen
        return self._build()

    def dispatch(self, size=None):
# ... 96 lines not shown
```

Before: 7551.

## Add shadow-ray exit table that starts traversal at the likely occluder leaf

Builds a 6×R×R table over the scene bounding box by tracing inward probe rays from each face cell and recording the BVH leaf each probe hits. A new shadow kernel maps each shadow ray's exit point on the root box to a cell, tests that cached leaf first, and only then falls back to a root traversal. The goal is early occlusion for shadow rays without walking the tree from the top. It adds a build-time pass, device counters and an adaptive on/off heuristic based on the observed occlusion rate. Rays whose cached leaf does not occlude pay for an extra leaf fetch.

```diff
diff --git a/include/rt3.h b/include/rt3.h
--- a/include/rt3.h
+++ b/include/rt3.h
@@ -113,6 +113,7 @@
 #define RT3_OPT_SAH_TOP 11
 #define RT3_OPT_TRACE_BLOCKS 12
 #define RT3_OPT_INSTANCE_MODE 14
+#define RT3_OPT_SHADOW_EXIT_TABLE 15
 int rt3_set_option(rt3_ctx *ctx, int option, int64_t value);
 
 int rt3_scene_set_vertices(rt3_ctx *ctx, const float *interleaved_p_n_t, uint32_t n_vertices);
@@ -140,6 +141,7 @@
 int rt3_accel_info(rt3_ctx *ctx, uint32_t *n_nodes, uint32_t *n_tris, uint32_t *max_depth, uint32_t *node_bytes);
 int rt3_accel_download(rt3_ctx *ctx, void *nodes, size_t nodes_bytes, void *tris, size_t tris_bytes);
 int rt3_accel_levels(rt3_ctx *ctx, uint32_t *n_meshes, uint32_t *n_meshes_built, uint32_t *n_top_nodes, uint64_t *accel_bytes);
+int rt3_accel_exit_table_info(rt3_ctx *ctx, uint32_t *cells, uint64_t *tried, uint64_t *occluded, uint32_t *in_use);
 int rt3_accel_import(rt3_ctx *ctx, const void *nodes, size_t nodes_bytes, const void *tris, size_t tris_bytes);
 int rt3_scene_update_vertices(rt3_ctx *ctx, const float *interleaved_p_n_t, uint32_t first, uint32_t n);
 int rt3_accel_refit(rt3_ctx *ctx, uint32_t *out_handle);
diff --git a/raytracer3_amd/_lib.py b/raytracer3_amd/_lib.py
--- a/raytracer3_amd/_lib.py
+++ b/raytracer3_amd/_lib.py
@@ -20,6 +20,7 @@
 OPT_WIDE_COLLAPSE, OPT_POOL_CHUNK, OPT_SAH_TOP, OPT_TRACE_BLOCKS = 8, 9, 11, 12
 OPT_FUSED_TRACE = 10
 OPT_INSTANCE_MODE = 14
+OPT_SHADOW_EXIT_TABLE = 15
 DENOISE_NO_DEMODULATION = 1
 TEMPORAL_NO_DEMODULATION = 1
 SELFTEST_EXPN = 28
@@ -31,7 +32,7 @@
     "rt3_scene_set_alpha_cutoffs",
     "rt3_scene_set_material_textures",
     "rt3_scene_set_instances",
-    "rt3_accel_build", "rt3_accel_info", "rt3_accel_levels", "rt3_accel_download", "rt3_accel_import", "rt3_sky_download",
+    "rt3_accel_build", "rt3_accel_info", "rt3_accel_levels", "rt3_accel_exit_table_info", "rt3_accel_download", "rt3_accel_import", "rt3_sky_download",
     "rt3_scene_update_vertices", "rt3_accel_refit", "rt3_light_info", "rt3_light_download",
     "rt3_buffer_create", "rt3_image_create", "rt3_image_import", "rt3_resource_upload", "rt3_resource_download", "rt3_resource_device_ptr",
     "rt3_set_tile_partition", "rt3_tile_pixel_count", "rt3_image_pack_tiles", "rt3_image_unpack_tiles",
@@ -136,6 +137,7 @@
         "rt3_accel_build": (i32, [vp, pu32]),
         "rt3_accel_info": (i32, [vp, pu32, pu32, pu32, pu32]),
         "rt3_accel_levels": (i32, [vp, pu32, pu32, pu32, C.POINTER(C.c_uint64)]),
+        "rt3_accel_exit_table_info": (i32, [vp, pu32, C.POINTER(C.c_uint64), C.POINTER(C.c_uint64), pu32]),
         "rt3_accel_download": (i32, [vp, vp, sz, vp, sz]),
         "rt3_accel_import": (i32, [vp, vp, sz, vp, sz]),
         "rt3_sky_download": (i32, [vp, vp, vp, vp, vp]),
diff --git a/raytracer3_amd/csrc/rt3_accel.hip b/raytracer3_amd/csrc/rt3_accel.hip
--- a/raytracer3_amd/csrc/rt3_accel.hip
+++ b/raytracer3_amd/csrc/rt3_accel.hip
@@ -568,9 +568,59 @@
     HIPC(c, hipMemcpy(c->accel.d_alpha.get(), table.data(), table.size() * sizeof(uint2), hipMemcpyHostToDevice));
     return RT3_OK;
 }
+static uint32_t exit_R(const rt3_ctx* c) {
+    if (c->opt.instance_mode == 1 || c->opt.node_width != 4 || c->opt.node_quant != 1) return 0u;
+    return kExitDefaultR;
+}
+static int make_exit_table(rt3_ctx* c) {
+    LbvhResult& b = c->accel.bvh;
+    b.exit.on = false;
+    if (!b.exit.off || !b.exit.R || b.layout != kLayoutWide64Q || !b.n_nodes || !b.nodes || !c->accel.n_flat_prims) return RT3_OK;
+    if (!c->accel.exit_counters) HIPC(c, c->accel.exit_counters.alloc_bytes(2 * sizeof(unsigned long long)));
+    b.exit.counters = c->accel.exit_counters.get();
+    HIPC(c, hipMemsetAsync(b.exit.counters, 0, 2 * sizeof(unsigned long long), c->stream));
+    if (c->opt.exit_table == 0) return RT3_OK;
+    uint32_t root[16];
+    double box[6];
+    HIPC(c, hipMemcpyAsync(root, b.nodes.get(), 64, hipMemcpyDeviceToHost, c->stream));
+    HIPC(c, hipStreamSynchronize(c->stream));
+    quantised_node_box(root, box);
+    for (int k = 0; k < 3; k++) {
+        if (!(box[k] <= box[3 + k])) return RT3_OK;
+        b.exit.lo[k] = round_down(box[k]);
+        b.exit.hi[k] = round_up(box[3 + k]);
+        const float ext = b.exit.hi[k] - b.exit.lo[k], s = (float)b.exit.R / ext;
+        b.exit.scale[k] = (ext > 0.0f && std::isfinite(s)) ? s : 0.0f;
+    }
+    ExitScratch s;
+    BufLayout plan;
+    exit_table_plan(6u * b.exit.R * b.exit.R, c->accel.n_flat_prims, plan, &s);
+    HIPC(c, c->accel.exit_scratch.grow_bytes(plan.bytes()));
+    HIPC(c, plan.carve(c->accel.exit_scratch));
+    const hipError_t e = exit_table_fill(c->stream, b, c->accel.n_flat_prims, s, c->opt.exit_table == 2);
+    if (e != hipSuccess) return fail(c, RT3_E_HIP, std::string("exit table: ") + hipGetErrorString(e));
+    b.exit.on = true;
+    return RT3_OK;
+}
+extern "C++" {
+namespace rt3 {
+int exit_table_update(rt3_ctx* c) {
+    if (!c->accel.built || c->accel.stale) return RT3_OK;
+    HIPC(c, hipSetDevice(c->device));
+    HIPC(c, hipStreamSynchronize(c->stream));
+    if (int r = make_exit_table(c)) return r;
+    HIPC(c, hipStreamSynchronize(c->stream));
+    return RT3_OK;
+}
+void exit_counters_reset(rt3_ctx* c) {
+    if (c->accel.exit_counters) (void)hipMemsetAsync(c->accel.exit_counters.get(), 0, 2 * sizeof(unsigned long long), c->stream);
+}
+}
+}
 static void bump_stamp(rt3_ctx* c) { c->accel.stamp++; }
 static int accel_finish(rt3_ctx* c, uint32_t* out_handle) {
     if (int r = make_shade_records(c)) return r;
+    if (int r = make_exit_table(c)) return r;
     HIPC(c, hipStreamSynchronize(c->stream));
     c->prof.stats.accel_bulk_copies += c->accel.bulk_copies;
     c->accel.bulk_copies = 0;
@@ -597,7 +647,7 @@
     } else {
         free_accel(c);
         hipError_t e = lbvh_build(c->stream, world_tables(c), c->accel.n_flat_prims, c->opt.leaf_size, c->opt.node_width, c->opt.node_quant, c->opt.collapse,
-                                  c->opt.sah_top, c->accel.build_scratch, &c->accel.bvh, c->accel.masked ? c->accel.d_geom_mask.get() : nullptr);
+                                  c->opt.sah_top, c->accel.build_scratch, &c->accel.bvh, c->accel.masked ? c->accel.d_geom_mask.get() : nullptr, exit_R(c));
         if (c->accel.build_scratch.capacity_bytes() > ((size_t)1 << 30)) c->accel.build_scratch.reset();
         if (e != hipSuccess) {
             const uint64_t need = c->accel.bvh.arena_need;
@@ -689,7 +739,7 @@
     HIPC(c, hipSetDevice(c->device));
     HIPC(c, hipStreamSynchronize(c->stream));
     LbvhResult fresh;
-    hipError_t e = fresh.alloc_arena(nodes_bytes, nt, c->stream);
+    hipError_t e = fresh.alloc_arena(nodes_bytes, nt, c->stream, exit_R(c));
     if (fresh.arena_need > kArenaMaxBytes) return fail_arena(c, "accel_import", fresh.arena_need);
     if (e == hipSuccess) e = hipStreamSynchronize(c->stream);
     if (e == hipSuccess) e = hipMemcpy(fresh.nodes.get(), nodes, nodes_bytes, hipMemcpyHostToDevice);
@@ -706,6 +756,26 @@
         invalidate_accel(c);
         return fail(c, RT3_E_HIP, std::string("accel_import: top-of-tree copy: ") + hipGetErrorString(e));
     }
+    if (int r = make_exit_table(c)) {
+        invalidate_accel(c);
+        return r;
+    }
+    HIPC(c, hipStreamSynchronize(c->stream));
+    return RT3_OK;
+}
+int rt3_accel_exit_table_info(rt3_ctx* c, uint32_t* cells, uint64_t* tried, uint64_t* occluded, uint32_t* in_use) {
+    if (int r = check_accel_current(c, "no acceleration structure built")) return r;
+    const ExitTable& t = c->accel.bvh.exit;
+    unsigned long long cnt[2] = {0, 0};
+    if (t.on) {
+        HIPC(c, hipSetDevice(c->device));
+        HIPC(c, hipStreamSynchronize(c->stream));
+        HIPC(c, hipMemcpy(cnt, t.counters, sizeof(cnt), hipMemcpyDeviceToHost));
+    }
+    if (cells) *cells = t.on ? 6u * t.R * t.R : 0u;
+    if (tried) *tried = cnt[0];
+    if (occluded) *occluded = cnt[1];
+    if (in_use) *in_use = (t.on && (cnt[0] < kExitWarmupTries || 4ull * cnt[1] >= cnt[0])) ? 1u : 0u;
     return RT3_OK;
 }
 
diff --git a/raytracer3_amd/csrc/rt3_api.hip b/raytracer3_amd/csrc/rt3_api.hip
--- a/raytracer3_amd/csrc/rt3_api.hip
+++ b/raytracer3_amd/csrc/rt3_api.hip
@@ -181,6 +181,10 @@
             c->opt.instance_mode = (int)value;
             invalidate_accel(c);
             return RT3_OK;
+        case RT3_OPT_SHADOW_EXIT_TABLE:
+            if (value < 0 || value > 2) return fail(c, RT3_E_INVALID, "shadow exit table must be 0 (off), 1 (on) or 2 (on, scrambled entries)");
+            c->opt.exit_table = (int)value;
+            return exit_table_update(c);
         default: return fail(c, RT3_E_INVALID, "unknown option");
     }
 }
diff --git a/raytracer3_amd/csrc/rt3_ctx.hpp b/raytracer3_amd/csrc/rt3_ctx.hpp
--- a/raytracer3_amd/csrc/rt3_ctx.hpp
+++ b/raytracer3_amd/csrc/rt3_ctx.hpp
@@ -156,6 +156,8 @@
         std::vector<rt3::MeshTables> refit_tables;
         rt3::DevBuf<char> refit_scratch;
         rt3::TwoLevelState tl;
+        rt3::DevBuf<unsigned long long> exit_counters;
+        rt3::DevBuf<char> exit_scratch;
     } accel;
 
     struct Work {
@@ -212,6 +214,7 @@
         int variant = 0;
         uint32_t leaf_size = 2, node_width = 4, node_quant = 1, collapse = 2, sah_top = 1;
         int instance_mode = 0;
+        int exit_table = 1;
     } opt;
     struct Prof {
         rt3_stats stats;
@@ -275,6 +278,8 @@
 GeomTables world_tables(const rt3_ctx* c);
 AlphaDev alpha_dev(const rt3_ctx* c);
 int ensure_lights(rt3_ctx* c);
+int exit_table_update(rt3_ctx* c);
+void exit_counters_reset(rt3_ctx* c);
 
 void motion_tables_stale(rt3_ctx* c);
 
diff --git a/raytracer3_amd/csrc/rt3_exit_table.hip b/raytracer3_amd/csrc/rt3_exit_table.hip
--- /dev/null
+++ b/raytracer3_amd/csrc/rt3_exit_table.hip
@@ -0,0 +1,101 @@
+#include <hip/hip_runtime.h>
+
+#include "rt3_hit.hpp"
+#include "rt3_internal.hpp"
+
+namespace rt3 {
+
+constexpr uint32_t kExitEmpty = 0xFFFFFFFFu;
+
+__global__ void k_exit_probes(ExitTable t, uint32_t n, float pad, float4* __restrict__ rays) {
+    const uint32_t i = blockIdx.x * blockDim.x + threadIdx.x;
+    if (i >= n) return;
+    const uint32_t iu = i % t.R, iv = (i / t.R) % t.R, face = i / (t.R * t.R), axis = face >> 1, high = face & 1u;
+    const uint32_t au = (axis + 1u) % 3u, av = (axis + 2u) % 3u;
+    float o[3], d[3] = {0.0f, 0.0f, 0.0f};
+    o[au] = t.lo[au] + ((float)iu + 0.5f) * ((t.hi[au] - t.lo[au]) / (float)t.R);
+    o[av] = t.lo[av] + ((float)iv + 0.5f) * ((t.hi[av] - t.lo[av]) / (float)t.R);
+    o[axis] = high ? t.hi[axis] + pad : t.lo[axis] - pad;
+    d[axis] = high ? -1.0f : 1.0f;
+    rays[i] = make_float4(o[0], o[1], o[2], 0.0f);
+    rays[n + i] = make_float4(d[0], d[1], d[2], kBackgroundDepth);
+}
+
+__global__ void k_exit_header(ExitHeader h, ExitHeader* out) { *out = h; }
+
+__global__ void k_exit_scatter(const float4* __restrict__ nodes, uint32_t n_nodes, const float4* __restrict__ tris, uint32_t n_tris, uint32_t n_prims,
+                               uint32_t* __restrict__ prim_leaf) {
+    const uint32_t i = blockIdx.x * blockDim.x + threadIdx.x;
+    if (i >= n_nodes) return;
+    const float4 a = nodes[4 * (size_t)i + 2], b = nodes[4 * (size_t)i + 3];
+    const uint32_t ref[4] = {__float_as_uint(a.z), __float_as_uint(a.w), __float_as_uint(b.x), __float_as_uint(b.y)};
+    for (int k = 0; k < 4; k++) {
+        if (ref[k] == kExitEmpty || (ref[k] & 0x80000000u) == 0u) continue;
+        const uint32_t first = ref[k] & 0x0FFFFFFFu, cnt = ((ref[k] >> 28) & 7u) + 1u;
+        if ((uint64_t)first + cnt > n_tris) continue;
+        for (uint32_t j = 0; j < cnt; j++) {
+            const uint32_t prim = __float_as_uint(tris[3 * (size_t)(first + j) + 2].y);
+            if (prim < n_prims) prim_leaf[prim] = ref[k];
+        }
+    }
+}
+
+__global__ void k_exit_entries(const float4* __restrict__ hits, const uint32_t* __restrict__ prim_leaf, uint32_t n_prims, uint32_t n, uint32_t scramble,
+                               uint32_t* __restrict__ table) {
+    const uint32_t i = blockIdx.x * blockDim.x + threadIdx.x;
+    if (i >= n) return;
+    uint32_t prim = __float_as_uint(hits[i].w);
+    if (scramble) {
+        uint32_t h = i * 0x9E3779B1u + 0x7F4A7C15u;
+        h ^= h >> 16;
+        h *= 0x85EBCA6Bu;
+        h ^= h >> 13;
+        prim = h % n_prims;
+    }
+    table[i] = prim < n_prims ? prim_leaf[prim] : kExitEmpty;
+}
+
+void exit_table_plan(uint32_t cells, uint32_t n_prims, BufLayout& plan, ExitScratch* s) {
+    plan.add(&s->rays, (size_t)cells * 8).add(&s->hits, (size_t)cells * 4).add(&s->prim_leaf, (size_t)n_prims).add(&s->cursor, 1);
+}
+
+hipError_t exit_table_fill(hipStream_t st, const LbvhResult& bvh, uint32_t n_prims, const ExitScratch& s, bool scramble) {
+    const ExitTable& t = bvh.exit;
+    const uint32_t n = 6u * t.R * t.R;
+    if (!t.off || !t.R || !n_prims || !bvh.n_nodes || bvh.layout != kLayoutWide64Q) return hipErrorInvalidValue;
+    float ext = 0.0f, mag = 0.0f;
+    for (int k = 0; k < 3; k++) {
+        ext = fmaxf(ext, t.hi[k] - t.lo[k]);
+        mag = fmaxf(mag, fmaxf(fabsf(t.lo[k]), fabsf(t.hi[k])));
+    }
+    const float pad = fmaxf(fmaxf(ext * 1.0e-3f, mag * 1.0e-5f), 1.0e-6f);
+    uint32_t* table = reinterpret_cast<uint32_t*>(reinterpret_cast<char*>(bvh.arena.get()) + t.off + sizeof(ExitHeader));
+    ExitHeader h = {};
+    for (int k = 0; k < 3; k++) {
+        h.lo[k] = t.lo[k];
+        h.hi[k] = t.hi[k];
+        h.scale[k] = t.scale[k];
+    }
+    h.R = t.R;
+    h.last = n - 1u;
+    hipLaunchKernelGGL(k_exit_header, dim3(1), dim3(1), 0, st, h, reinterpret_cast<ExitHeader*>(reinterpret_cast<char*>(bvh.arena.get()) + t.off));
+    hipLaunchKernelGGL(k_exit_probes, dim3((n + 255) / 256), dim3(256), 0, st, t, n, pad, reinterpret_cast<float4*>(s.rays));
+    RT3_TRY(hipMemsetAsync(s.cursor, 0, 4, st));
+    RT3_TRY(hipMemsetAsync(s.prim_leaf, 0xFF, (size_t)n_prims * 4, st));
+    hipLaunchKernelGGL(k_exit_scatter, dim3((bvh.n_nodes + 255) / 256), dim3(256), 0, st, bvh.nodes.get(), bvh.n_nodes, bvh.tris.get(), bvh.n_tris, n_prims,
+                       s.prim_leaf);
+    if (!scramble) {
+        TraceLaunch L;
+        L.rays = s.rays;
+        L.stride = n;
+        L.n = n;
+        L.work_counter = s.cursor;
+        L.hits = s.hits;
+        launch_extend(st, bvh, L);
+    }
+    hipLaunchKernelGGL(k_exit_entries, dim3((n + 255) / 256), dim3(256), 0, st, reinterpret_cast<const float4*>(s.hits), s.prim_leaf, n_prims, n,
+                       scramble ? 1u : 0u, table);
+    return hipGetLastError();
+}
+
+}
diff --git a/raytracer3_amd/csrc/rt3_internal.hpp b/raytracer3_amd/csrc/rt3_internal.hpp
--- a/raytracer3_amd/csrc/rt3_internal.hpp
+++ b/raytracer3_amd/csrc/rt3_internal.hpp
@@ -207,6 +207,24 @@
 uint64_t next_arena_serial();
 constexpr size_t kArenaSlack = 128;
 
+constexpr uint32_t kExitDefaultR = 256, kExitMaxR = 1024;
+constexpr size_t kExitTableSlack = 64;
+struct ExitHeader {
+    float lo[3], hi[3], scale[3];
+    uint32_t R, last;
+    uint32_t pad[5];
+};
+static_assert(sizeof(ExitHeader) == 64, "the entries start 64 bytes behind the header");
+constexpr uint64_t kExitWarmupTries = 1ull << 16;
+struct ExitTable {
+    uint32_t off = 0;
+    uint32_t R = 0;
+    float lo[3] = {0, 0, 0}, hi[3] = {0, 0, 0};
+    float scale[3] = {0, 0, 0};
+    unsigned long long* counters = nullptr;
+    bool on = false;
+};
+
 struct LbvhResult {
     DevBuf<float4> arena;
     DevView<float4> nodes;
@@ -219,24 +237,32 @@
     DevBuf<float4> top;
     uint32_t n_top = 0;
     uint32_t n_nodes = 0, n_tris = 0, max_depth = 0;
-
-    hipError_t alloc_arena(size_t nodes_bytes, size_t n_records, hipStream_t st) {
+    ExitTable exit;
+
+    hipError_t alloc_arena(size_t nodes_bytes, size_t n_records, hipStream_t st, uint32_t exit_R = 0) {
+        const uint32_t exit_cells = 6u * exit_R * exit_R;
         free_arena();
         const size_t off = (nodes_bytes + 127) & ~(size_t)127, rec_end = off + n_records * 48;
-        arena_need = rec_end + kArenaSlack;
+        const size_t table = exit_cells ? sizeof(ExitHeader) + (size_t)exit_cells * 4 + kExitTableSlack : 0;
+        arena_need = rec_end + kArenaSlack + table;
         if (arena_need > kArenaMaxBytes) return hipErrorInvalidValue;
-        RT3_TRY(arena.alloc_bytes(rec_end + kArenaSlack));
+        RT3_TRY(arena.alloc_bytes(rec_end + kArenaSlack + table));
         arena_serial = next_arena_serial();
         tri_off = (uint32_t)off;
         nodes = DevView<float4>(arena.get());
         tris = DevView<float4>(reinterpret_cast<float4*>(reinterpret_cast<char*>(arena.get()) + off));
-        return hipMemsetAsync(reinterpret_cast<char*>(arena.get()) + rec_end, 0, kArenaSlack, st);
+        RT3_TRY(hipMemsetAsync(reinterpret_cast<char*>(arena.get()) + rec_end, 0, kArenaSlack, st));
+        if (!table) return hipSuccess;
+        exit.R = exit_R;
+        exit.off = (uint32_t)(rec_end + kArenaSlack);
+        return hipMemsetAsync(reinterpret_cast<char*>(arena.get()) + exit.off, 0xFF, table, st);
     }
     void free_arena() {
         arena.reset();
         nodes = tris = DevView<float4>();
         tri_off = 0;
         arena_serial = 0;
+        exit = ExitTable{};
     }
     void take_arena(LbvhResult& from) {
         arena = std::move(from.arena);
@@ -244,6 +270,8 @@
         tris = from.tris;
         tri_off = from.tri_off;
         arena_serial = from.arena_serial;
+        exit = from.exit;
+        from.exit = ExitTable{};
         from.nodes = from.tris = DevView<float4>();
         from.tri_off = 0;
         from.arena_serial = 0;
@@ -269,7 +297,14 @@
 void launch_extend(hipStream_t st, const LbvhResult& bvh, const TraceLaunch& L);
 void launch_shadow(hipStream_t st, const LbvhResult& bvh, const TraceLaunch& L);
 hipError_t lbvh_build(hipStream_t st, GeomTables t, uint32_t n_prims, uint32_t leaf_max, uint32_t node_width, uint32_t node_quant, uint32_t collapse_mode,
-                      uint32_t sah_top, DevBuf<char>& scratch, LbvhResult* out, const uint2* geom_mask = nullptr);
+                      uint32_t sah_top, DevBuf<char>& scratch, LbvhResult* out, const uint2* geom_mask = nullptr, uint32_t exit_R = 0);
+
+struct ExitScratch {
+    float *rays, *hits;
+    uint32_t *prim_leaf, *cursor;
+};
+void exit_table_plan(uint32_t cells, uint32_t n_prims, BufLayout& plan, ExitScratch* s);
+hipError_t exit_table_fill(hipStream_t st, const LbvhResult& bvh, uint32_t n_prims, const ExitScratch& s, bool scramble);
 struct SahTopScratch {
     uint32_t *top, *ncl, *pool_pos, *cl_pos, *pool, *cl_ref, *cl_cnt, *idx, *tmp, *counters, *tile_left, *tile_woff, *tile_roff;
     float *cl_mn, *cl_mx;
diff --git a/raytracer3_amd/csrc/rt3_lbvh.hip b/raytracer3_amd/csrc/rt3_lbvh.hip
--- a/raytracer3_amd/csrc/rt3_lbvh.hip
+++ b/raytracer3_amd/csrc/rt3_lbvh.hip
@@ -724,7 +724,7 @@
 }
 
 hipError_t lbvh_build(hipStream_t st, GeomTables t, uint32_t n, uint32_t leaf_max, uint32_t node_width, uint32_t node_quant, uint32_t collapse_mode,
-                      uint32_t sah_top, DevBuf<char>& scratch, LbvhResult* out, const uint2* geom_mask) {
+                      uint32_t sah_top, DevBuf<char>& scratch, LbvhResult* out, const uint2* geom_mask, uint32_t exit_R) {
     *out = LbvhResult{};
     out->n_tris = n;
     const int wide = node_width == 4, quant = wide ? (node_quant > 2 ? 2 : (int)node_quant) : 0, collapse = wide ? (collapse_mode > 2 ? 2 : (int)collapse_mode) : 0;
@@ -732,6 +732,7 @@
     out->node_bytes = (wide && !quant) ? 128u : (quant == 2 ? 16u * kC48Stride : 64u);
     out->layout = !wide ? kLayoutBinary64 : (quant == 2 ? kLayoutWide48Q : (quant ? kLayoutWide64Q : kLayoutWide128));
     if (n == 0) return hipSuccess;
+    if (out->layout != kLayoutWide64Q) exit_R = 0;
     const uint32_t nn = n > 1 ? n - 1 : 1;
     LbvhScratch s = {};
     {
@@ -760,7 +761,7 @@
     hipLaunchKernelGGL(k_leaves, dim3(grid), dim3(256), 0, st, t.verts, t.indices, t.geoms, t.prim_geom, t.first_prim, s.vals_out, s.bmin, s.bmax, s.bounds, n,
                        s.tris_dp ? s.tris_dp : (s.tris_morton ? s.tris_morton : s.tris_stage), s.lmin, s.lmax, geom_mask);
     if (n == 1) {
-        RT3_TRY(out->alloc_arena(out->node_bytes, 1, st));
+        RT3_TRY(out->alloc_arena(out->node_bytes, 1, st, exit_R));
         hipLaunchKernelGGL(k_single, dim3(1), dim3(1), 0, st, s.lmin, s.lmax, wide, quant, out->nodes.get());
         RT3_TRY(hipMemcpyAsync(out->tris.get(), s.tris_stage, 48, hipMemcpyDeviceToDevice, st));
         out->n_nodes = 1;
@@ -835,7 +836,7 @@
         RT3_TRY(hipMemcpyAsync(&out->max_depth, s.levels, 4, hipMemcpyDeviceToHost, st));
         RT3_TRY(hipStreamSynchronize(st));
         out->n_nodes = tail[0] + tail[1];
-        RT3_TRY(out->alloc_arena((size_t)out->n_nodes * out->node_bytes, n, st));
+        RT3_TRY(out->alloc_arena((size_t)out->n_nodes * out->node_bytes, n, st, exit_R));
         if (quant != 2) RT3_TRY(hipMemcpyAsync(out->tris.get(), s.tris_stage, (size_t)n * 48, hipMemcpyDeviceToDevice, st));
         if (quant == 2) {
             hipLaunchKernelGGL(k_child_counts, dim3(grid), dim3(256), 0, st, s.left, s.right, s.rcnt, s.nbox, s.keep, nn, s.live, s.dk, collapse, s.n_int, s.n_ltri);
diff --git a/raytracer3_amd/csrc/rt3_scene.hip b/raytracer3_amd/csrc/rt3_scene.hip
--- a/raytracer3_amd/csrc/rt3_scene.hip
+++ b/raytracer3_amd/csrc/rt3_scene.hip
@@ -380,6 +380,7 @@
     c->scene.sky_w = w;
     c->scene.sky_h = h;
     c->scene.sky_wt = wt;
+    exit_counters_reset(c);
     return RT3_OK;
 }
 int rt3_scene_set_bluenoise(rt3_ctx* c, const uint8_t* rgba, uint32_t w, uint32_t h) {
diff --git a/raytracer3_amd/csrc/rt3_trace.hip b/raytracer3_amd/csrc/rt3_trace.hip
--- a/raytracer3_amd/csrc/rt3_trace.hip
+++ b/raytracer3_amd/csrc/rt3_trace.hip
@@ -55,6 +55,9 @@
 
 __constant__ uint32_t g_pool_chunk = 256;
 __constant__ uint32_t g_refill_lanes = 12;
+__device__ __forceinline__ uint32_t pool_chunk_for(uint32_t n, uint32_t n_waves) {
+    return (n < 2u * n_waves * g_pool_chunk && g_pool_chunk >= 128u) ? ((g_pool_chunk >> 1) & ~63u) : g_pool_chunk;
+}
 void set_refill_lanes(uint32_t v) { (void)hipMemcpyToSymbol(HIP_SYMBOL(g_refill_lanes), &v, 4); }
 void set_pool_chunk(uint32_t v) { (void)hipMemcpyToSymbol(HIP_SYMBOL(g_pool_chunk), &v, 4); }
 static unsigned g_trace_max_blocks = kExtendMaxBlocks;
@@ -87,6 +90,19 @@
     const float tf = __builtin_fminf(__builtin_fminf(fx, fy), __builtin_fminf(fz, tbest));
     tn_out = tn;
     return tn <= tf;
+}
+
+constexpr uint32_t kExitFlag = 0x20000000u;
+struct ExitWalk {
+    uint32_t off = 0;
+    uint32_t mode = 0;
+    uint32_t occluded = 0;
+};
+__device__ __forceinline__ unsigned long long exit_sampled_rays(uint32_t n, uint32_t chunk) {
+    if (n == 0u) return 0ull;
+    const uint32_t n_chunks = (n - 1u) / chunk + 1u, m = (n_chunks + 31u) / 32u;
+    const unsigned long long last_first = 32ull * (m - 1u) * chunk, rest = n - last_first;
+    return (unsigned long long)(m - 1u) * chunk + (rest < chunk ? rest : chunk);
 }
 
 struct LaneRay {
@@ -100,12 +116,13 @@
     uint32_t sel_p0, sel_q0, sel_p1, sel_q1;
 };
 
-template <int MODE, bool COUNT, int LAYOUT, bool TWO = false, bool RANGE = false, bool MASK = false, typename Finish>
+template <int MODE, bool COUNT, int LAYOUT, bool TWO = false, bool RANGE = false, bool MASK = false, bool EXIT = false, typename Finish>
 __device__ __forceinline__ void trace_stream(const float4* __restrict__ nodes, uint32_t tri_off,
                                              const float* __restrict__ rays, size_t stride, uint32_t n, uint32_t* __restrict__ work_counter,
                                              uint32_t* __restrict__ lds, Finish finish, bool any_payload = false, bool ext_payload = false, const float4* top_lds = nullptr, bool use_top = false,
                                              const float2* __restrict__ any_contrib = nullptr, const float* __restrict__ any_tmax = nullptr,
-                                             const AlphaDev& alpha = AlphaDev{}) {
+                                             const AlphaDev& alpha = AlphaDev{}, ExitWalk* xw = nullptr) {
+    static_assert(!EXIT || (MODE == 1 && !COUNT && !TWO && !RANGE && LAYOUT == kLayoutWide64Q), "the exit table serves the plain any-hit walk only");
     constexpr bool ANY = MODE == 1;
     constexpr bool WIDE = LAYOUT == kLayoutWide128;
     constexpr bool WIDEQ = LAYOUT == kLayoutWide64Q || LAYOUT == kLayoutWide48Q;
@@ -116,9 +133,10 @@
     const unsigned long long lanes_below = (1ull << lane) - 1ull;
     const uint32_t n_waves = gridDim.x * (blockDim.x >> 6);
     const uint32_t kRefillLanes = g_refill_lanes,
-                   kPoolChunk = (n < 2u * n_waves * g_pool_chunk && g_pool_chunk >= 128u) ? ((g_pool_chunk >> 1) & ~63u) : g_pool_chunk;
+                   kPoolChunk = pool_chunk_for(n, n_waves);
     const uint32_t wave_id = blockIdx.x * (blockDim.x >> 6) + (uint32_t)__builtin_amdgcn_readfirstlane((int)(threadIdx.x >> 6));
     bool first_chunk = true;
+    bool chunk_exit = false;
     uint32_t spill[kSpill];
     LaneRay r;
     r.o = r.d = r.inv = v3(0.0f, 0.0f, 0.0f);
@@ -164,6 +182,7 @@
             queue_empty = base >= n;
             pool_next = base < n ? base : n;
             pool_end = (n - pool_next) > kPoolChunk ? pool_next + kPoolChunk : n;
+            if constexpr (EXIT) chunk_exit = xw->mode == 2u || (xw->mode == 1u && ((base / kPoolChunk) & 31u) == 0u);
         }
         if (m_idle != 0ull && pool_next < pool_end && ((uint32_t)__popcll(m_idle) >= kRefillLanes || m_idle == ~0ull)) {
             const uint32_t idx = pool_next + (uint32_t)__popcll(m_idle & lanes_below);
@@ -193,6 +212,27 @@
                     r.sel_q1 = r.sel_q0 + 0x00000202u;
                 }
                 r.cur = (LAYOUT == kLayoutWide64Q && use_top) ? kTopFlag : 0u;
+                if constexpr (EXIT) {
+                    if (chunk_exit) {
+                        uint32_t hoff = xw->off;
+                        asm volatile("" : "+s"(hoff));
+                        const ExitHeader e = *reinterpret_cast<const ExitHeader*>(reinterpret_cast<const char*>(nodes) + hoff);
+                        const float tx = ((r.inv.x < 0.0f ? e.lo[0] : e.hi[0]) - r.o.x) * r.inv.x, ty = ((r.inv.y < 0.0f ? e.lo[1] : e.hi[1]) - r.o.y) * r.inv.y,
+                                    tz = ((r.inv.z < 0.0f ? e.lo[2] : e.hi[2]) - r.o.z) * r.inv.z;
+                        const bool ax0 = (tx <= ty) & (tx <= tz), ax1 = !ax0 & (ty <= tz);
+                        const float te = ax0 ? tx : (ax1 ? ty : tz);
+                        const float cx = (__builtin_fmaf(te, r.d.x, r.o.x) - e.lo[0]) * e.scale[0], cy = (__builtin_fmaf(te, r.d.y, r.o.y) - e.lo[1]) * e.scale[1],
+                                    cz = (__builtin_fmaf(te, r.d.z, r.o.z) - e.lo[2]) * e.scale[2];
+                        const float cu = ax0 ? cy : (ax1 ? cz : cx), cv = ax0 ? cz : (ax1 ? cx : cy);
+                        const float ia = ax0 ? r.inv.x : (ax1 ? r.inv.y : r.inv.z);
+                        const uint32_t face = (ax0 ? 0u : (ax1 ? 2u : 4u)) + (ia < 0.0f ? 0u : 1u);
+                        const float top = (float)(e.R - 1u);
+                        const uint32_t iu = (uint32_t)__builtin_fminf(__builtin_fmaxf(cu, 0.0f), top), iv = (uint32_t)__builtin_fminf(__builtin_fmaxf(cv, 0.0f), top);
+                        uint32_t cell = (face * e.R + iv) * e.R + iu;
+                        cell = cell < e.last ? cell : e.last;
+                        r.cur = kExitFlag | cell;
+                    }
+                }
                 if (TWO) tl_world();
                 r.leaf_k = 0u;
                 r.sp = 0;
@@ -211,6 +251,7 @@
             pool_next = pool_next + taken < pool_end ? pool_next + taken : pool_end;
         }
         if (__ballot(busy) == 0ull && pool_next >= pool_end && queue_empty) break;
+        bool by_entry = false;
         if (busy) {
         const bool is_leaf = (r.cur & 0x80000000u) != 0u;
         const uint32_t first = r.cur & 0x0FFFFFFFu, cnt = ((r.cur >> 28) & 7u) + 1u;
@@ -220,7 +261,14 @@
         constexpr uint32_t kNodeBytes = 16u * (WIDE ? 8 : (C48 ? kC48Stride : 4));
         uint32_t off_tri = tri_off + 48u * (first + r.leaf_k), off_node = kNodeBytes * (cached ? 0u : (is_inst ? first : r.cur));
         asm volatile("" : "+v"(off_tri), "+v"(off_node));
-        const uint32_t off = is_tri ? off_tri : off_node;
+        uint32_t off = is_tri ? off_tri : off_node;
+        bool is_exit = false;
+        if constexpr (EXIT) {
+            is_exit = !is_leaf && (r.cur & kExitFlag) != 0u;
+            uint32_t off_exit = xw->off + (uint32_t)sizeof(ExitHeader) + ((r.cur & 0x00FFFFFCu) << 2);
+            asm volatile("" : "+v"(off_exit));
+            off = is_exit ? off_exit : off;
+        }
         const float4* p = reinterpret_cast<const float4*>(reinterpret_cast<const char*>(nodes) + off);
         float4 q0, q1, q2, q3, q4, q5, q6, q7;
         if (TWO && is_tri) {
@@ -254,7 +302,16 @@
         bool pop = false, done = false;
         const V3 o = r.o, d = r.d, inv = r.inv;
         const float tmin = r.tmin;
-        if (TWO && is_inst) {
+        if (EXIT && is_exit) {
+            const uint32_t k = r.cur & 3u;
+            const uint32_t e = __float_as_uint(k == 0u ? q0.x : (k == 1u ? q0.y : (k == 2u ? q0.z : q0.w)));
+            const uint32_t root = use_top ? kTopFlag : 0u;
+            if (e != kEmptySlot) {
+                lds[0] = root;
+                r.sp = 1;
+            }
+            r.cur = e != kEmptySlot ? e : root;
+        } else if (TWO && is_inst) {
             if (COUNT) r.cn++;
             const float mi[12] = {q0.x, q0.y, q0.z, q0.w, q1.x, q1.y, q1.z, q1.w, q2.x, q2.y, q2.z, q2.w};
             const V3 oo = transform_point(mi, o), dd = transform_vector(mi, d);
@@ -431,10 +488,14 @@
         }
         if (++r.steps >= kMaxSteps) done = true;
         if (done) {
+            if constexpr (EXIT) {
+                by_entry = r.best.prim != kMiss && r.sp == 1 && lds[0] == (use_top ? kTopFlag : 0u);
+            }
             finish(r.index, r.best, r.cn, r.ct, r.cl, r.pay0, r.pay1, r.pay2, r.pay3);
             busy = false;
         }
         }
+        if constexpr (EXIT) xw->occluded += (uint32_t)__popcll(__ballot(by_entry));
     }
 }
 
@@ -521,6 +582,51 @@
     counts.add_totals(totals, lds_total);
 }
 
+template <bool MASK>
+__global__ __launch_bounds__(kExtendBlock) __attribute__((amdgpu_waves_per_eu(8, 8))) void k_shadow_exit(const float4* __restrict__ nodes, uint32_t tri_off, const float4* __restrict__ top, uint32_t n_top,
+                                                              const float* __restrict__ rays, size_t stride,
+                                                              const uint32_t* __restrict__ count_ptr, uint32_t count_imm, AlphaArg<MASK> alpha,
+                                                              const float* __restrict__ contrib, float* __restrict__ lacc,
+                                                              uint32_t* __restrict__ occluded_out, uint32_t* __restrict__ work_counter, uint32_t exit_off,
+                                                              unsigned long long* __restrict__ counters) {
+    __shared__ uint32_t stack[kLdsStack * kExtendBlock];
+    __shared__ float4 s_top[4 * kTopNodes];
+    const bool use_top = load_top(s_top, top, n_top);
+    const uint32_t n = count_ptr ? *count_ptr : count_imm;
+    ExitWalk xw;
+    xw.off = exit_off;
+    {
+        const unsigned long long tried = counters[0], occluded = counters[1];
+        xw.mode = (tried < kExitWarmupTries || 4ull * occluded >= tried) ? 2u : 1u;
+    }
+    trace_stream<1, false, kLayoutWide64Q, false, false, MASK, true>(
+        nodes, tri_off, rays, stride, n, work_counter, stack + threadIdx.x,
+        [&](uint32_t i, const Hit& h, uint32_t, uint32_t, uint32_t, float c_r, float c_g, float c_b, float c_pid) {
+            if (occluded_out) {
+                occluded_out[i] = h.prim != kMiss ? 1u : 0u;
+            } else if (h.prim == kMiss) {
+                float4* L = reinterpret_cast<float4*>(lacc) + __float_as_uint(c_pid);
+                float4 v = *L;
+                *L = make_float4(v.x + c_r, v.y + c_g, v.z + c_b, 0.0f);
+            }
+        },
+        occluded_out == nullptr, false, s_top, use_top, occluded_out == nullptr ? reinterpret_cast<const float2*>(contrib) : nullptr, nullptr, alpha.get(), &xw);
+    {
+        __syncthreads();
+        if ((threadIdx.x & 63u) == 0u) stack[threadIdx.x >> 6] = xw.occluded;
+        __syncthreads();
+        if (threadIdx.x == 0u) {
+            unsigned long long o = 0;
+            for (uint32_t w = 0; w < kExtendBlock / 64u; w++) o += stack[w];
+            if (o) atomicAdd(&counters[1], o);
+            if (blockIdx.x == 0u) {
+                const unsigned long long t = xw.mode == 2u ? n : exit_sampled_rays(n, pool_chunk_for(n, gridDim.x * (kExtendBlock / 64u)));
+                if (t) atomicAdd(&counters[0], t);
+            }
+        }
+    }
+}
+
 template <typename Launch>
 static void dispatch_traversal(bool count, int layout, bool masked, Launch launch) {
     auto by_mask = [&](auto c, auto l) {
@@ -554,6 +660,15 @@
 }
 void launch_shadow(hipStream_t st, const LbvhResult& bvh, const TraceLaunch& L) {
     const unsigned grid = grid_for(L.n, kExtendBlock, g_trace_max_blocks);
+    if (bvh.exit.on && bvh.exit.off && bvh.exit.counters && bvh.layout == kLayoutWide64Q && bvh.nodes && !L.count && !L.tmax) {
+        auto launch = [&](auto m) {
+            hipLaunchKernelGGL((k_shadow_exit<decltype(m)::value>), dim3(grid), dim3(kExtendBlock), 0, st, bvh.nodes.get(), bvh.tri_off, bvh.top.get(), bvh.n_top, L.rays,
+                               L.stride, L.count_ptr, L.n, alpha_arg<decltype(m)::value>(L), L.contrib, L.lacc, L.occluded, L.work_counter, bvh.exit.off, bvh.exit.counters);
+        };
+        if (L.alpha.table != nullptr) launch(std::true_type{});
+        else launch(std::false_type{});
+        return;
+    }
     unsigned long long* const tot = L.totals ? L.totals + kTotShadowNodes : nullptr;
     unsigned long long* const lds_tot = L.totals ? L.totals + kTotShadowLds : nullptr;
     dispatch_traversal(L.count, bvh.layout, L.alpha.table != nullptr, [&](auto c, auto l, auto m) {
diff --git a/raytracer3_amd/render_graph.py b/raytracer3_amd/render_graph.py
--- a/raytracer3_amd/render_graph.py
+++ b/raytracer3_amd/render_graph.py
@@ -244,6 +244,11 @@
         self.check(self.lib.rt3_accel_levels(self.h, C.byref(a), C.byref(b), C.byref(c), C.byref(d)))
         return a.value, b.value, c.value, d.value
 
+    def exit_table_info(self):
+        a, b, c, d = C.c_uint32(), C.c_uint64(), C.c_uint64(), C.c_uint32()
+        self.check(self.lib.rt3_accel_exit_table_info(self.h, C.byref(a), C.byref(b), C.byref(c), C.byref(d)))
+        return a.value, b.value, c.value, d.value
+
     def accel_download(self):
         nn, nt, _, nb = self.accel_info()
         nodes = np.empty((nn, nb // 4), np.uint32)
```

Result: faster. 7717, median of 6 (+2.2%).
